# lyuchenyang/Macaw-LLM

Measured on NVIDIA H100. Metric: multimodal prefill tokens/sec (img+audio+text->LLaMA), higher is better.
Workload: dtype fp16

## Files before the change

include/macaw_b200.h:

```cpp
#ifndef MACAW_B200_H_
#define MACAW_B200_H_

#include <stdint.h>

#ifdef __cplusplus
extern "C" {
#endif

const char* mm_last_error(void);
int32_t mm_abi_version(void);
const char* mm_build_hash(void);
int64_t mm_launch_count(void);
void mm_launch_count_reset(void);
void mm_set_act_format(int32_t f16);
int32_t mm_get_act_format(void);

enum {
  MM_ACT_NONE = 0,
  MM_ACT_GELU = 1,
  MM_ACT_QUICK_GELU = 2,
  MM_ACT_SILU = 3
};
enum {
  MM_EPI_STD = 0,
  MM_EPI_SWIGLU = 1,
  MM_EPI_ROPE = 2
};

typedef struct mm_gemm_args {
  int32_t M, N, K, batch, batch2;
  const void* A;
  int64_t lda, a_bs, a_bs2;
  const void* B;
  int64_t ldb, b_bs, b_bs2;
  int32_t b_mn_major;
  void* C;
  int64_t ldc, c_bs, c_bs2;
  int32_t c_fp32;
  int32_t epi;
  int32_t act;
  float alpha;
  const void* bias;
  int64_t bias_bs;
  const float* row_scale;
  const void* residual;
  int64_t ldr, r_bs, r_bs2;
  int32_t res_row_mod;
  const float* rope_cos;
  const float* rope_sin;
  int32_t rope_T, rope_cols;
  const int32_t* rope_pos;
  int32_t c_trans;
  int32_t a_fp16, b_fp16;
  int32_t c_fp16;
  const float* bias_rs;
  const void* bias2;
  const float* bias2_rs;
  int32_t a_mn_major;
  float* sumsq_out;
  const float* rs_sumsq;
  int32_t rs_parts;
  float rs_eps;
  void* sk_workspace;
  int64_t sk_workspace_bytes;
} mm_gemm_args;

int32_t mm_gemm_fwd(const mm_gemm_args* args, void* stream);
enum {
  MM_GEMM_KERNEL_CONSUMER_EPILOGUE = 0,
  MM_GEMM_KERNEL_EPILOGUE_WARPGROUP = 1,
  MM_GEMM_KERNEL_TILE_PAIRS = 2
};
typedef struct mm_gemm_schedule {
  int32_t block_n;
  int32_t kernel;
  int32_t m_tiles, n_tiles, k_blocks;
  int64_t units;
  int32_t workers;
  int32_t grid;
  int32_t threads;
  int32_t waves;
  int32_t group_m;
  int32_t streamk_tiles;
  int32_t smem_bytes;
  int32_t vectorised_epilogue;
} mm_gemm_schedule;
int32_t mm_gemm_plan(const mm_gemm_args* args, mm_gemm_schedule* plan);
int32_t mm_gemm_streamk_mode(int32_t mode);
int32_t mm_gemm_overlap_mode(int32_t mode);
int64_t mm_gemm_streamk_workspace_bytes(void);

int32_t mm_splitk_reduce(const float* partial, int32_t splits, int32_t M, int32_t N, const void* bias, void* out,
                         int64_t ldo, int32_t out_fp16, void* stream);

typedef struct mm_attn_args {
  const void *q, *k, *v;
  void* out;
  int32_t B, H, Tq, Tk, head_dim;
  int64_t q_bs, q_ts, q_hs;
  int64_t k_bs, k_ts, k_hs;
  int64_t v_bs, v_ts, v_hs;
  int64_t o_bs, o_ts, o_hs;
  const int32_t* key_mask;
  int32_t causal;
  float scale;
  const int32_t* tk_dev;
} mm_attn_args;
int32_t mm_attn_fwd(const mm_attn_args* args, void* stream);

int32_t mm_rmsnorm_fwd(const void* x, const void* w, void* y, int32_t rows, int32_t cols, float eps, void* stream);
int32_t mm_rms_rstd(const void* x, float* rstd, int32_t rows, int32_t cols, float eps, void* stream);
int32_t mm_layernorm_fwd(const void* x, int64_t ldx, const void* w, const void* b, void* y, int64_t ldy, int32_t rows,
                         int32_t cols, float eps, void* stream);

int32_t mm_embed_gather(const void* table, int32_t vocab, int32_t dim, const int64_t* ids, int64_t n_ids, void* out,
                        int64_t ldo, void* stream);
int32_t mm_splice_prefix(const void* text, const void* prefix, void* dst, int32_t B, int32_t L, int32_t n_prefix,
                         int32_t E, const int64_t* mask_in, int64_t* mask_out, const int64_t* labels_in,
                         int64_t* labels_out, void* stream);
int32_t mm_patchify(const void* images, int32_t B, int32_t C, int32_t H, int32_t W, int32_t patch, void* out,
                    int64_t ldo, void* stream);
int32_t mm_transpose_pad(const void* x, int32_t B, int32_t C, int32_t T, int32_t pad, void* out, void* stream);
int32_t mm_add_rows(const void* x, int64_t ldx, const void* add, int64_t lda, int32_t add_rows, void* y, int64_t ldy,
                    int32_t rows, int32_t cols, void* stream);
int32_t mm_cast_bf16_f16(const void* x, int64_t ldx, void* y, int64_t ldy, int32_t rows, int32_t cols, void* stream);
int32_t mm_copy_rows(const void* x, int64_t ldx, void* y, int64_t ldy, int32_t rows, int32_t cols, void* stream);

typedef struct mm_align_args {
  const void* table;
  int32_t V, E;
  int64_t ldt;
  const void* qt;
  int32_t R;
  int64_t ldq;
  const float* row_bias;
  const float* extra;
  int64_t stat_stride;
  void* out;
  int64_t ldo;
  float* p_sum_real;
  float* p_extra;
  void* P;
  int64_t ldp;
  void* workspace;
  int32_t mode;
  float* inv_l;
} mm_align_args;
int32_t mm_align_fwd(const mm_align_args* args, void* stream);
int64_t mm_align_workspace_bytes(int32_t R, int32_t V);

int32_t mm_kv_append(const void* qkv, int64_t ld_qkv, int32_t B, int32_t T_new, int32_t E, void* cache, int32_t Tmax,
                     int32_t t0, const int32_t* t0_dev, void* stream);
int32_t mm_argmax_rows(const void* logits, int64_t ld, int32_t rows, int32_t V, int64_t* out, void* stream);
int32_t mm_sample_rows(const void* logits, int64_t ld, int32_t rows, int32_t V, uint32_t* seen, float repetition_penalty,
                       float temperature, int32_t top_k, float top_p, int32_t do_sample, const uint64_t* seed_dev,
                       const int32_t* step_dev, int64_t* out, void* stream);
enum { MM_THIN_RES = 0, MM_THIN_SWIGLU = 1, MM_THIN_QKV = 2 };
typedef struct mm_thin_args {
  const float* part;
  int32_t splits, N, M, ldp, mode;
  const float* row_scale;
  const float* rs_sumsq;
  int32_t rs_parts, rs_K;
  float rs_eps;
  const void* residual;
  int64_t ldr;
  void* out;
  int64_t ldo;
  float* sumsq_out;
  const float* rope_cos;
  const float* rope_sin;
  const int32_t* pos_dev;
  int32_t E;
  void* cache;
  int32_t Tmax, t0;
  const int32_t* t0_dev;
} mm_thin_args;
int32_t mm_thin_fused(const mm_thin_args* args, void* stream);
int32_t mm_rope_rows(void* x, int64_t ld, int32_t rows, int32_t rot_cols, const float* cos_t, const float* sin_t,
                     int32_t rope_T, const int32_t* pos_dev, void* stream);

int32_t mm_ce_loss(const void* logits, const int64_t* labels, int32_t B, int32_t T, int32_t V, float* loss_sum,
                   int32_t* n_valid, void* stream);

int32_t mm_rmsnorm_bwd_parts(int32_t rows);
int32_t mm_rmsnorm_bwd(const void* dy, const void* x, const float* rstd, const void* g, const void* dres, void* dx,
                       float* dg, float* dg_partials, int32_t rows, int32_t cols, void* stream);
int32_t mm_swiglu_fwd(const void* gate, const void* up, void* h, int64_t n, void* stream);
int32_t mm_swiglu_bwd(const void* dh, const void* gate, const void* up, void* dgate, void* dup, int64_t n, void* stream);
int32_t mm_attn_softmax_bwd(const float* S, const float* dP, void* P, void* dS, int32_t B, int32_t H, int32_t Tq,
                            int32_t Tk, int64_t ld, float scale, int32_t causal, const int32_t* key_mask, float p_drop,
                            const uint64_t* seed_dev, uint32_t sid, void* stream);
int32_t mm_attn_softmax_fwd(const float* S, void* P, int32_t B, int32_t H, int32_t Tq, int32_t Tk, int64_t ld, float scale,
                            int32_t causal, const int32_t* key_mask, float p_drop, const uint64_t* seed_dev, uint32_t sid,
                            void* stream);
int32_t mm_align_dropout_fwd(const void* P_unnorm_f16, void* Pm_f16, int64_t ldp, const float* inv_l, const float* p_extra,
                             float* rs, float* p_sum_real_d, float* p_extra_d, int32_t R, int32_t V, float p_drop,
                             const uint64_t* seed_dev, uint32_t sid, void* stream);
int32_t mm_dropout_mask(float* out, int64_t ld, int32_t rows, int32_t cols, float p_drop, const uint64_t* seed_dev,
                        uint32_t sid, void* stream);
int32_t mm_ce_bwd(const void* logits, const int64_t* labels, void* dlogits, int32_t B, int32_t T, int32_t V,
                  const int32_t* n_valid, float grad_scale, const float* grad_scale_dev, void* stream);
int32_t mm_embed_scatter_add(const void* dx, int64_t ldx, const int64_t* ids, int64_t n, int32_t dim, int32_t vocab,
                             void* dtable, void* stream);
int32_t mm_colsum(const void* x, int64_t ldx, int32_t rows, int32_t cols, float* out, void* stream);
int32_t mm_adamw(void* p, const void* g, float* master, float* m, float* v, int64_t n, float lr, float beta1, float beta2,
                 float eps, float weight_decay, int32_t step, const int32_t* step_dev, float grad_scale,
                 const float* grad_mult_dev, const int32_t* skip_dev, const float* lr_dev, void* stream);
int32_t mm_adamw_host(void* p, const void* g, float* master, float* m, float* v, int64_t n, float lr, float beta1,
                      float beta2, float eps, float weight_decay, int32_t step, const int32_t* step_dev, float grad_scale,
                      const float* grad_mult_dev, const int32_t* skip_dev, const float* lr_dev, void* stream);
int32_t mm_host_alloc(int64_t bytes, void** host_ptr, void** dev_ptr);
int32_t mm_host_free(void* host_ptr);

int32_t mm_grad_sumsq_parts(int64_t n);
int32_t mm_grad_sumsq(const void* g, int64_t n, int32_t fp16, float* out, float* partials, void* stream);
typedef struct mm_loss_scale_state {
  float scale;
  float inv_scale;
  int32_t cur_iter;
  int32_t last_overflow_iter;
  int32_t cur_hysteresis;
  int32_t skip;
  float grad_mult;
  int32_t skipped;
  int32_t step;
  float grad_norm;
  int32_t reserved[2];
} mm_loss_scale_state;
int32_t mm_loss_scale_update(mm_loss_scale_state* state, float* sumsq, float max_norm, int32_t dynamic, int32_t window,
                             int32_t hysteresis, float min_scale, void* stream);

int32_t mm_lr_schedule(const int32_t* step_dev, double base_lr, int32_t kind, int32_t warmup_steps, int32_t training_steps,
                       float* lr_out, void* stream);

int32_t mm_align_softmax_bwd(const float* G, int64_t ldg, const void* P_unnorm_f16, int64_t ldp, const float* inv_l,
                             const float* d_p_sum_real, const float* p_extra, const float* d_p_extra, float gscale,
                             void* P_bf16, void* dS_bf16, int64_t ldo, float* dstats, int32_t R, int32_t V, float p_drop,
                             const uint64_t* seed_dev, uint32_t sid, void* stream);
int32_t mm_head_weighted_colsum(const void* x, int64_t ldx, int32_t x_fp16, const float* w, int64_t w_stride, int32_t Nq,
                                int32_t E, int32_t head_dim, float* out, void* stream);
int32_t mm_window_gather_add(const void* dwin, int32_t B, int32_t N, int32_t C, int32_t Lq, int32_t kk, int32_t ss,
                             void* dfeats, void* stream);
int32_t mm_cast_f16_bf16(const void* x, int64_t ldx, void* y, int64_t ldy, int32_t rows, int32_t cols, void* stream);

#define MM_LORA_MAX 3
typedef struct mm_lora_args {
  int32_t n, M, K, N, r;
  float scaling, p_drop;
  const uint64_t* seed_dev;
  uint32_t sid[MM_LORA_MAX];
  const void* x;
  int64_t ldx;
  const void* A[MM_LORA_MAX];
  const void* B[MM_LORA_MAX];
  float* u[MM_LORA_MAX];
  void* y[MM_LORA_MAX];
  int64_t ldy;
  const float* rope_cos;
  const float* rope_sin;
  int32_t rope_T;
  float* g[MM_LORA_MAX];
  void* dA[MM_LORA_MAX];
  void* dB[MM_LORA_MAX];
  int32_t accumulate[MM_LORA_MAX];
  void* dx;
  int64_t lddx;
  float* workspace;
  int64_t workspace_bytes;
} mm_lora_args;
int32_t mm_lora_down(const mm_lora_args* args, void* stream);
int32_t mm_lora_up(const mm_lora_args* args, void* stream);
int32_t mm_lora_bwd_dy(const mm_lora_args* args, void* stream);
int32_t mm_lora_bwd_x(const mm_lora_args* args, void* stream);
int64_t mm_lora_workspace_bytes(const mm_lora_args* args, int32_t entry);

#define MM_W8_MAX_SRC 3
#define MM_W8_XS_BYTES 49152
typedef struct mm_w8_matrix {
  const int8_t* q[MM_W8_MAX_SRC];
  const float* scale[MM_W8_MAX_SRC];
  int32_t rows[MM_W8_MAX_SRC];
  const int32_t* chunks;
  int32_t N, K;
  const void* gain;
} mm_w8_matrix;
int32_t mm_quantize_rows_int8(const void* w, int64_t ldw, int32_t w_format, int32_t rows, int32_t K, int8_t* q, float* scale,
                              void* stream);
int32_t mm_dequant_rows(const mm_w8_matrix* w, void* out, int64_t ldo, void* stream);
int32_t mm_gemm_w8_thin(const mm_w8_matrix* w, const void* x, int64_t ldx, int32_t M, float* part, int32_t splits,
                        int32_t ldp, void* xs_work, void* stream);

typedef struct mm_gemm_e4m3_args {
  const float* a_scale;
  mm_w8_matrix w;
  int32_t unpromoted;
} mm_gemm_e4m3_args;
int32_t mm_quantize_rows_e4m3(const void* x, int64_t ldx, int32_t x_format, int32_t rows, int32_t K, const void* gain,
                              uint8_t* q, int64_t ldq, float* scale, void* stream);
int32_t mm_gemm_e4m3_fwd(const mm_gemm_args* args, const mm_gemm_e4m3_args* e, void* stream);
int32_t mm_gemm_e4m3_plan(const mm_gemm_args* args, const mm_gemm_e4m3_args* e, mm_gemm_schedule* plan);
int32_t mm_gemm_e4m3_thin(const mm_w8_matrix* w, const void* x, int64_t ldx, int32_t M, float* part, int32_t splits,
                          int32_t ldp, void* xs_work, void* stream);

int32_t mm_nccl_unique_id(void* out128);
int32_t mm_nccl_init(const void* id128, int32_t world, int32_t rank);
int32_t mm_nccl_allreduce(void* buf, int64_t count, int32_t dtype, int32_t average, void* stream);
int32_t mm_nccl_destroy(void);

typedef struct mm_image_args {
  const void* src;
  int64_t ld;
  int32_t row0, n_rows;
  int32_t out_h, out_w;
  const int32_t* bounds_h;
  const int32_t* kk_h;
  int32_t ksize_h;
  const int32_t* bounds_v;
  const int32_t* kk_v;
  int32_t ksize_v;
  float mean[3], std[3];
  void* tmp;
  void* out;
  int32_t out_fp32;
  void* out_u8;
} mm_image_args;
int32_t mm_image_preprocess(const mm_image_args* args, void* stream);
int32_t mm_log_mel(const float* pcm, int32_t n_samples, const float* basisT, const float* mel, float* logspec,
                   void* max_scratch, void* out, int32_t out_fp32, void* stream);

typedef struct mm_jpeg_image {
  int32_t width, height;
  int32_t n_comp;
  int32_t hmax, vmax;
  int32_t mcus_x, mcus_y;
  int32_t seg0, n_seg;
  int32_t bw[3], bh[3];
  int32_t huff_dc[3], huff_ac[3];
  int32_t quant[3];
  int64_t coef_off[3];
  int64_t plane_off[3];
  int64_t out_off, out_ld;
} mm_jpeg_image;
typedef struct mm_jpeg_segment {
  int64_t offset;
  int32_t n_bytes;
  int32_t image;
  int32_t mcu0, n_mcu;
} mm_jpeg_segment;
typedef struct mm_jpeg_huff {
  int32_t maxcode[18];
  int32_t valoffset[18];
  uint16_t look[256];
  uint8_t huffval[256];
} mm_jpeg_huff;
typedef struct mm_jpeg_args {
  int32_t n_images, n_segments, n_huff, n_quant;
  const uint8_t* data;
  int64_t data_bytes;
  const mm_jpeg_image* images;
  const mm_jpeg_segment* segments;
  const mm_jpeg_huff* huff;
  const uint16_t* quant;
  int16_t* coef;
  int64_t coef_elems;
  uint8_t* planes;
  int64_t plane_bytes;
  uint8_t* out;
  int64_t out_bytes;
  int32_t* status;
  int32_t max_blocks, max_pixels;
} mm_jpeg_args;
int32_t mm_jpeg_decode(const mm_jpeg_args* args, void* stream);

#ifdef __cplusplus
}
#endif
#endif
```

macaw-llm_b200/_lib.py:

```python
from __future__ import annotations

import ctypes as C
import os

HERE = os.path.dirname(os.path.abspath(__file__))
LIB_PATH = os.path.join(HERE, "libmacaw_b200.so")

c_i32, c_i64, c_f32, c_vp, c_u32 = C.c_int32, C.c_int64, C.c_float, C.c_void_p, C.c_uint32


class GemmArgs(C.Structure):

    _fields_ = [
        ("M", c_i32), ("N", c_i32), ("K", c_i32), ("batch", c_i32), ("batch2", c_i32),
        ("A", c_vp), ("lda", c_i64), ("a_bs", c_i64), ("a_bs2", c_i64),
        ("B", c_vp), ("ldb", c_i64), ("b_bs", c_i64), ("b_bs2", c_i64), ("b_mn_major", c_i32),
        ("C", c_vp), ("ldc", c_i64), ("c_bs", c_i64), ("c_bs2", c_i64), ("c_fp32", c_i32),
        ("epi", c_i32), ("act", c_i32), ("alpha", c_f32),
        ("bias", c_vp), ("bias_bs", c_i64),
        ("row_scale", c_vp),
        ("residual", c_vp), ("ldr", c_i64), ("r_bs", c_i64), ("r_bs2", c_i64), ("res_row_mod", c_i32),
        ("rope_cos", c_vp), ("rope_sin", c_vp), ("rope_T", c_i32), ("rope_cols", c_i32), ("rope_pos", c_vp), ("c_trans", c_i32),
        ("a_fp16", c_i32), ("b_fp16", c_i32), ("c_fp16", c_i32),
        ("bias_rs", c_vp), ("bias2", c_vp), ("bias2_rs", c_vp), ("a_mn_major", c_i32),
        ("sumsq_out", c_vp), ("rs_sumsq", c_vp), ("rs_parts", c_i32), ("rs_eps", c_f32),
        ("sk_workspace", c_vp), ("sk_workspace_bytes", c_i64),
    ]


class GemmPlan(C.Structure):

    _fields_ = [("block_n", c_i32), ("kernel", c_i32), ("m_tiles", c_i32), ("n_tiles", c_i32), ("k_blocks", c_i32),
                ("units", c_i64), ("workers", c_i32), ("grid", c_i32), ("threads", c_i32), ("waves", c_i32),
                ("group_m", c_i32), ("streamk_tiles", c_i32), ("smem_bytes", c_i32), ("vectorised_epilogue", c_i32)]


class ThinArgs(C.Structure):
    _fields_ = [("part", c_vp), ("splits", c_i32), ("N", c_i32), ("M", c_i32), ("ldp", c_i32), ("mode", c_i32),
                ("row_scale", c_vp), ("rs_sumsq", c_vp), ("rs_parts", c_i32), ("rs_K", c_i32), ("rs_eps", c_f32),
                ("residual", c_vp), ("ldr", c_i64), ("out", c_vp), ("ldo", c_i64), ("sumsq_out", c_vp),
                ("rope_cos", c_vp), ("rope_sin", c_vp), ("pos_dev", c_vp), ("E", c_i32), ("cache", c_vp),
                ("Tmax", c_i32), ("t0", c_i32), ("t0_dev", c_vp)]


class AttnArgs(C.Structure):

    _fields_ = [
        ("q", c_vp), ("k", c_vp), ("v", c_vp), ("out", c_vp),
        ("B", c_i32), ("H", c_i32), ("Tq", c_i32), ("Tk", c_i32), ("head_dim", c_i32),
        ("q_bs", c_i64), ("q_ts", c_i64), ("q_hs", c_i64),
        ("k_bs", c_i64), ("k_ts", c_i64), ("k_hs", c_i64),
        ("v_bs", c_i64), ("v_ts", c_i64), ("v_hs", c_i64),
        ("o_bs", c_i64), ("o_ts", c_i64), ("o_hs", c_i64),
        ("key_mask", c_vp), ("causal", c_i32), ("scale", c_f32), ("tk_dev", c_vp),
    ]


class AlignArgs(C.Structure):

    _fields_ = [
        ("table", c_vp), ("V", c_i32), ("E", c_i32), ("ldt", c_i64),
        ("qt", c_vp), ("R", c_i32), ("ldq", c_i64),
        ("row_bias", c_vp), ("extra", c_vp), ("stat_stride", c_i64),
        ("out", c_vp), ("ldo", c_i64), ("p_sum_real", c_vp), ("p_extra", c_vp),
        ("P", c_vp), ("ldp", c_i64), ("workspace", c_vp), ("mode", c_i32), ("inv_l", c_vp),
    ]


LORA_MAX = 3


class LoraArgs(C.Structure):

    _fields_ = [
        ("n", c_i32), ("M", c_i32), ("K", c_i32), ("N", c_i32), ("r", c_i32), ("scaling", c_f32), ("p_drop", c_f32),
        ("seed_dev", c_vp), ("sid", c_u32 * LORA_MAX), ("x", c_vp), ("ldx", c_i64), ("A", c_vp * LORA_MAX),
        ("B", c_vp * LORA_MAX), ("u", c_vp * LORA_MAX), ("y", c_vp * LORA_MAX), ("ldy", c_i64), ("rope_cos", c_vp),
        ("rope_sin", c_vp), ("rope_T", c_i32), ("g", c_vp * LORA_MAX), ("dA", c_vp * LORA_MAX), ("dB", c_vp * LORA_MAX),
        ("accumulate", c_i32 * LORA_MAX), ("dx", c_vp), ("lddx", c_i64), ("workspace", c_vp), ("workspace_bytes", c_i64),
    ]


W8_MAX_SRC = 3
W8_XS_BYTES = 49152


class W8Matrix(C.Structure):

    _fields_ = [("q", c_vp * W8_MAX_SRC), ("scale", c_vp * W8_MAX_SRC), ("rows", c_i32 * W8_MAX_SRC), ("chunks", c_vp), ("N", c_i32), ("K", c_i32),
                ("gain", c_vp)]


class GemmE4m3Args(C.Structure):

    _fields_ = [("a_scale", c_vp), ("w", W8Matrix), ("unpromoted", c_i32)]


class LossScaleState(C.Structure):

    _fields_ = [("scale", c_f32), ("inv_scale", c_f32), ("cur_iter", c_i32), ("last_overflow_iter", c_i32),
                ("cur_hysteresis", c_i32), ("skip", c_i32), ("grad_mult", c_f32), ("skipped", c_i32), ("step", c_i32),
                ("grad_norm", c_f32), ("reserved", c_i32 * 2)]


class ImageArgs(C.Structure):

    _fields_ = [
        ("src", c_vp), ("ld", c_i64), ("row0", c_i32), ("n_rows", c_i32), ("out_h", c_i32), ("out_w", c_i32),
        ("bounds_h", c_vp), ("kk_h", c_vp), ("ksize_h", c_i32), ("bounds_v", c_vp), ("kk_v", c_vp), ("ksize_v", c_i32),
        ("mean", c_f32 * 3), ("std", c_f32 * 3), ("tmp", c_vp), ("out", c_vp), ("out_fp32", c_i32), ("out_u8", c_vp),
    ]


class JpegImage(C.Structure):

    _fields_ = [
        ("width", c_i32), ("height", c_i32), ("n_comp", c_i32), ("hmax", c_i32), ("vmax", c_i32),
        ("mcus_x", c_i32), ("mcus_y", c_i32), ("seg0", c_i32), ("n_seg", c_i32),
        ("bw", c_i32 * 3), ("bh", c_i32 * 3), ("huff_dc", c_i32 * 3), ("huff_ac", c_i32 * 3), ("quant", c_i32 * 3),
        ("coef_off", c_i64 * 3), ("plane_off", c_i64 * 3), ("out_off", c_i64), ("out_ld", c_i64),
    ]


class JpegSegment(C.Structure):

    _fields_ = [("offset", c_i64), ("n_bytes", c_i32), ("image", c_i32), ("mcu0", c_i32), ("n_mcu", c_i32)]


class JpegHuff(C.Structure):

    _fields_ = [("maxcode", c_i32 * 18), ("valoffset", c_i32 * 18), ("look", C.c_uint16 * 256), ("huffval", C.c_uint8 * 256)]


class JpegArgs(C.Structure):

    _fields_ = [
        ("n_images", c_i32), ("n_segments", c_i32), ("n_huff", c_i32), ("n_quant", c_i32),
        ("data", c_vp), ("data_bytes", c_i64), ("images", c_vp), ("segments", c_vp), ("huff", c_vp), ("quant", c_vp),
        ("coef", c_vp), ("coef_elems", c_i64), ("planes", c_vp), ("plane_bytes", c_i64), ("out", c_vp),
        ("out_bytes", c_i64), ("status", c_vp), ("max_blocks", c_i32), ("max_pixels", c_i32),
    ]


SIGNATURES = {
    "mm_last_error": (C.c_char_p, []),
    "mm_abi_version": (c_i32, []),
    "mm_build_hash": (C.c_char_p, []),
    "mm_launch_count": (c_i64, []),
    "mm_launch_count_reset": (None, []),
    "mm_set_act_format": (None, [c_i32]),
    "mm_get_act_format": (c_i32, []),
    "mm_gemm_fwd": (c_i32, [C.POINTER(GemmArgs), c_vp]),
    "mm_gemm_plan": (c_i32, [C.POINTER(GemmArgs), C.POINTER(GemmPlan)]),
    "mm_splitk_reduce": (c_i32, [c_vp, c_i32, c_i32, c_i32, c_vp, c_vp, c_i64, c_i32, c_vp]),
    "mm_attn_fwd": (c_i32, [C.POINTER(AttnArgs), c_vp]),
    "mm_rmsnorm_fwd": (c_i32, [c_vp, c_vp, c_vp, c_i32, c_i32, c_f32, c_vp]),
    "mm_rms_rstd": (c_i32, [c_vp, c_vp, c_i32, c_i32, c_f32, c_vp]),
    "mm_layernorm_fwd": (c_i32, [c_vp, c_i64, c_vp, c_vp, c_vp, c_i64, c_i32, c_i32, c_f32, c_vp]),
    "mm_embed_gather": (c_i32, [c_vp, c_i32, c_i32, c_vp, c_i64, c_vp, c_i64, c_vp]),
    "mm_splice_prefix": (c_i32, [c_vp, c_vp, c_vp, c_i32, c_i32, c_i32, c_i32, c_vp, c_vp, c_vp, c_vp, c_vp]),
    "mm_patchify": (c_i32, [c_vp, c_i32, c_i32, c_i32, c_i32, c_i32, c_vp, c_i64, c_vp]),
    "mm_transpose_pad": (c_i32, [c_vp, c_i32, c_i32, c_i32, c_i32, c_vp, c_vp]),
    "mm_add_rows": (c_i32, [c_vp, c_i64, c_vp, c_i64, c_i32, c_vp, c_i64, c_i32, c_i32, c_vp]),
    "mm_cast_bf16_f16": (c_i32, [c_vp, c_i64, c_vp, c_i64, c_i32, c_i32, c_vp]),
    "mm_copy_rows": (c_i32, [c_vp, c_i64, c_vp, c_i64, c_i32, c_i32, c_vp]),
    "mm_align_fwd": (c_i32, [C.POINTER(AlignArgs), c_vp]),
    "mm_align_workspace_bytes": (c_i64, [c_i32, c_i32]),
    "mm_kv_append": (c_i32, [c_vp, c_i64, c_i32, c_i32, c_i32, c_vp, c_i32, c_i32, c_vp, c_vp]),
    "mm_gemm_streamk_workspace_bytes": (c_i64, []),
    "mm_gemm_streamk_mode": (c_i32, [c_i32]),
    "mm_gemm_overlap_mode": (c_i32, [c_i32]),
    "mm_thin_fused": (c_i32, [C.POINTER(ThinArgs), c_vp]),
    "mm_argmax_rows": (c_i32, [c_vp, c_i64, c_i32, c_i32, c_vp, c_vp]),
    "mm_sample_rows": (c_i32, [c_vp, c_i64, c_i32, c_i32, c_vp, c_f32, c_f32, c_i32, c_f32, c_i32, c_vp, c_vp, c_vp, c_vp]),
    "mm_rope_rows": (c_i32, [c_vp, c_i64, c_i32, c_i32, c_vp, c_vp, c_i32, c_vp, c_vp]),
    "mm_rmsnorm_bwd": (c_i32, [c_vp, c_vp, c_vp, c_vp, c_vp, c_vp, c_vp, c_vp, c_i32, c_i32, c_vp]),
    "mm_rmsnorm_bwd_parts": (c_i32, [c_i32]),
    "mm_swiglu_fwd": (c_i32, [c_vp, c_vp, c_vp, c_i64, c_vp]),
    "mm_swiglu_bwd": (c_i32, [c_vp, c_vp, c_vp, c_vp, c_vp, c_i64, c_vp]),
    "mm_attn_softmax_bwd": (c_i32, [c_vp, c_vp, c_vp, c_vp, c_i32, c_i32, c_i32, c_i32, c_i64, c_f32, c_i32, c_vp, c_f32, c_vp,
                                    c_u32, c_vp]),
    "mm_attn_softmax_fwd": (c_i32, [c_vp, c_vp, c_i32, c_i32, c_i32, c_i32, c_i64, c_f32, c_i32, c_vp, c_f32, c_vp, c_u32, c_vp]),
    "mm_align_dropout_fwd": (c_i32, [c_vp, c_vp, c_i64, c_vp, c_vp, c_vp, c_vp, c_vp, c_i32, c_i32, c_f32, c_vp, c_u32, c_vp]),
    "mm_dropout_mask": (c_i32, [c_vp, c_i64, c_i32, c_i32, c_f32, c_vp, c_u32, c_vp]),
    "mm_ce_bwd": (c_i32, [c_vp, c_vp, c_vp, c_i32, c_i32, c_i32, c_vp, c_f32, c_vp, c_vp]),
    "mm_embed_scatter_add": (c_i32, [c_vp, c_i64, c_vp, c_i64, c_i32, c_i32, c_vp, c_vp]),
    "mm_colsum": (c_i32, [c_vp, c_i64, c_i32, c_i32, c_vp, c_vp]),
    "mm_adamw": (c_i32, [c_vp, c_vp, c_vp, c_vp, c_vp, c_i64, c_f32, c_f32, c_f32, c_f32, c_f32, c_i32, c_vp, c_f32, c_vp,
                         c_vp, c_vp, c_vp]),
    "mm_adamw_host": (c_i32, [c_vp, c_vp, c_vp, c_vp, c_vp, c_i64, c_f32, c_f32, c_f32, c_f32, c_f32, c_i32, c_vp, c_f32,
                              c_vp, c_vp, c_vp, c_vp]),
    "mm_lr_schedule": (c_i32, [c_vp, C.c_double, c_i32, c_i32, c_i32, c_vp, c_vp]),
    "mm_host_alloc": (c_i32, [c_i64, C.POINTER(c_vp), C.POINTER(c_vp)]),
    "mm_host_free": (c_i32, [c_vp]),
    "mm_grad_sumsq_parts": (c_i32, [c_i64]),
    "mm_grad_sumsq": (c_i32, [c_vp, c_i64, c_i32, c_vp, c_vp, c_vp]),
    "mm_loss_scale_update": (c_i32, [c_vp, c_vp, c_f32, c_i32, c_i32, c_i32, c_f32, c_vp]),
    "mm_image_preprocess": (c_i32, [C.POINTER(ImageArgs), c_vp]),
    "mm_log_mel": (c_i32, [c_vp, c_i32, c_vp, c_vp, c_vp, c_vp, c_vp, c_i32, c_vp]),
    "mm_align_softmax_bwd": (c_i32, [c_vp, c_i64, c_vp, c_i64, c_vp, c_vp, c_vp, c_vp, c_f32, c_vp, c_vp, c_i64, c_vp, c_i32,
                                     c_i32, c_f32, c_vp, c_u32, c_vp]),
    "mm_head_weighted_colsum": (c_i32, [c_vp, c_i64, c_i32, c_vp, c_i64, c_i32, c_i32, c_i32, c_vp, c_vp]),
    "mm_window_gather_add": (c_i32, [c_vp, c_i32, c_i32, c_i32, c_i32, c_i32, c_i32, c_vp, c_vp]),
    "mm_cast_f16_bf16": (c_i32, [c_vp, c_i64, c_vp, c_i64, c_i32, c_i32, c_vp]),
    "mm_nccl_unique_id": (c_i32, [c_vp]),
    "mm_nccl_init": (c_i32, [c_vp, c_i32, c_i32]),
    "mm_nccl_allreduce": (c_i32, [c_vp, c_i64, c_i32, c_i32, c_vp]),
    "mm_nccl_destroy": (c_i32, []),
    "mm_ce_loss": (c_i32, [c_vp, c_vp, c_i32, c_i32, c_i32, c_vp, c_vp, c_vp]),
    "mm_lora_down": (c_i32, [C.POINTER(LoraArgs), c_vp]),
    "mm_lora_up": (c_i32, [C.POINTER(LoraArgs), c_vp]),
    "mm_lora_bwd_dy": (c_i32, [C.POINTER(LoraArgs), c_vp]),
    "mm_lora_bwd_x": (c_i32, [C.POINTER(LoraArgs), c_vp]),
    "mm_lora_workspace_bytes": (c_i64, [C.POINTER(LoraArgs), c_i32]),
    "mm_jpeg_decode": (c_i32, [C.POINTER(JpegArgs), c_vp]),
    "mm_quantize_rows_int8": (c_i32, [c_vp, c_i64, c_i32, c_i32, c_i32, c_vp, c_vp, c_vp]),
    "mm_dequant_rows": (c_i32, [C.POINTER(W8Matrix), c_vp, c_i64, c_vp]),
    "mm_gemm_w8_thin": (c_i32, [C.POINTER(W8Matrix), c_vp, c_i64, c_i32, c_vp, c_i32, c_i32, c_vp, c_vp]),
    "mm_quantize_rows_e4m3": (c_i32, [c_vp, c_i64, c_i32, c_i32, c_i32, c_vp, c_vp, c_i64, c_vp, c_vp]),
    "mm_gemm_e4m3_fwd": (c_i32, [C.POINTER(GemmArgs), C.POINTER(GemmE4m3Args), c_vp]),
    "mm_gemm_e4m3_plan": (c_i32, [C.POINTER(GemmArgs), C.POINTER(GemmE4m3Args), C.POINTER(GemmPlan)]),
    "mm_gemm_e4m3_thin": (c_i32, [C.POINTER(W8Matrix), c_vp, c_i64, c_i32, c_vp, c_i32, c_i32, c_vp, c_vp]),
}

NULLABLE_BEFORE_STREAM = {"mm_adamw": 1, "mm_adamw_host": 1}

_lib = None
ABI_VERSION = 8


class _NullableBeforeStream:

    def __init__(self, fn, n_opt: int):
        self._fn, self._n_opt = fn, n_opt

    def __call__(self, *args):
        n = len(self._fn.argtypes)
        if n - self._n_opt <= len(args) < n:
            args = args[:-1] + (None,) * (n - len(args)) + args[-1:]
        return self._fn(*args)

    def __getattr__(self, name):
        return getattr(self._fn, name)


def load(build_if_missing: bool = True) -> C.CDLL:
    global _lib
    if _lib is not None:
        return _lib
    import importlib.util

    spec = importlib.util.spec_from_file_location("_macaw_b200_build", os.path.join(HERE, "build.py"))
    mod = importlib.util.module_from_spec(spec)
    spec.loader.exec_module(mod)
    want = mod.source_hash()
    if not os.path.exists(LIB_PATH) or mod.built_hash() != want:
        if not build_if_missing:
            raise RuntimeError(f"{LIB_PATH} is missing or older than csrc/; run `python macaw-llm_b200/build.py`")
        mod.build()
    lib = C.CDLL(LIB_PATH)
    for name, (res, args) in SIGNATURES.items():
        fn = getattr(lib, name)
        fn.restype = res
        fn.argtypes = args
        if name in NULLABLE_BEFORE_STREAM:
            setattr(lib, name, _NullableBeforeStream(fn, NULLABLE_BEFORE_STREAM[name]))
    got = lib.mm_build_hash().decode()
    if got != want or lib.mm_abi_version() != ABI_VERSION:
        raise RuntimeError(f"libmacaw_b200.so was built from other sources (library {got}, csrc {want}; ABI "
                           f"{lib.mm_abi_version()} vs {ABI_VERSION}): rebuild with `python macaw-llm_b200/build.py --force`")
    _lib = lib
    return lib


def last_error() -> str:
    return load().mm_last_error().decode("utf-8", "replace")
```

macaw-llm_b200/csrc/gemm_wgmma.cu:

```cuda
#include "common.cuh"
#include "ptx.cuh"
#include "../../include/macaw_b200.h"
#include <stdlib.h>

namespace mm {

struct GemmKParams {
  int M, N, K, batch, batch2;
  int m_tiles, n_tiles, num_k;
  int b_shared, b2_shared;
  void* C;
  long long ldc, c_bs, c_bs2;
  int c_fp32;
  int act;
  float alpha;
  const bf16* bias;
  long long bias_bs;
  const float* row_scale;
  const bf16* residual;
  long long ldr, r_bs, r_bs2;
  int res_row_mod;
  const float* rope_cos;
  const float* rope_sin;
  int rope_T, rope_cols;
  const int* rope_pos;
  int c_trans;
  int c_fp16;
  int aux_f16;
  const float* bias_rs;
  const bf16* bias2;
  const float* bias2_rs;
  float* sumsq_out;
  const float* rs_sumsq;
  int sumsq_parts, rs_parts;
  float rs_eps;
  int vec_ok;
  int group_m;
  int sk_tiles, sk_first;
  float* sk_ws;
  int* sk_flags;
};

constexpr int kBlockM = 128;
constexpr int kBlockK = 64;
constexpr uint32_t kABytes = kBlockM * kBlockK * 2;
constexpr int kMaxBN = 128;
constexpr int kGemmThreads = 288;
constexpr int kProducerWarp = 8;
constexpr int kGemmThreadsEwg = 512;
constexpr int kProducerWarpEwg = 12;
constexpr int kEwgMinKBlocks = 32;

__host__ __device__ constexpr int gemm_stages(int BN) {
  return BN >= 128 ? 4 : (BN >= 64 ? 6 : 8);
}
__host__ __device__ constexpr int gemm_stage_ld(int BN) { return BN + 4; }
__host__ __device__ constexpr size_t gemm_smem_bytes(int stages, uint32_t b_bytes, int BN) {
  return 1024  + (size_t)stages * (kABytes + b_bytes) + (size_t)kBlockM * gemm_stage_ld(BN) * 4 +
         256 ;
}

struct GemmSmem {
  uint8_t *sA, *sB;
  float* sC;
  uint64_t *full_bar, *empty_bar, *staging_full, *staging_empty;
};
template <int STAGES, uint32_t B_BYTES, int BN>
__device__ __forceinline__ GemmSmem gemm_smem(uint8_t* smem_raw) {
  uint8_t* smem = reinterpret_cast<uint8_t*>((reinterpret_cast<uintptr_t>(smem_raw) + 1023) & ~uintptr_t(1023));
  uint8_t* sB = smem + STAGES * kABytes;
  float* sC = reinterpret_cast<float*>(sB + STAGES * B_BYTES);
  uint64_t* bar = reinterpret_cast<uint64_t*>(sC + kBlockM * gemm_stage_ld(BN));
  return {smem, sB, sC, bar, bar + STAGES, bar + 2 * STAGES, bar + 2 * STAGES + 1};
}
template <int STAGES, bool STAGING>
__device__ __forceinline__ void gemm_prologue(const GemmSmem& s, const CUtensorMap* tmA, const CUtensorMap* tmB) {
  tma_prefetch_desc(tmA);
  tma_prefetch_desc(tmB);
  for (int i = 0; i < STAGES; ++i) {
    mbar_init(&s.full_bar[i], 1);
    mbar_init(&s.empty_bar[i], 8);
  }
  if constexpr (STAGING) {
    mbar_init(s.staging_full, 256);
    mbar_init(s.staging_empty, 128);
  }
  fence_mbar_init();
}

struct TileCoord {
  int b, b_lo, b_hi, m_blk, n_blk;
};
__device__ __forceinline__ TileCoord tile_coord(int idx, const GemmKParams& p, int m_units) {
  const int per_batch = m_units * p.n_tiles;
  TileCoord t;
  t.b = idx / per_batch;
  t.b_hi = t.b / p.batch;
  t.b_lo = t.b - t.b_hi * p.batch;
  int r = idx - t.b * per_batch;
  const int in_group = p.group_m * p.n_tiles;
  const int g = r / in_group;
  const int first_m = g * p.group_m;
  const int gsz = min(m_units - first_m, p.group_m);
  const int rr = r - g * in_group;
  t.m_blk = first_m + rr % gsz;
  t.n_blk = rr / gsz;
  return t;
}

struct GemmWork {
  int tile, kb0, kb1, role, c0, nc;
};
__device__ __forceinline__ bool gemm_work(const GemmKParams& p, int worker, int n_workers, int total_tiles, int it,
                                          GemmWork& w) {
  const int first = p.sk_tiles > 0 ? p.sk_first : total_tiles;
  const int n_full = first > worker ? (first - worker + n_workers - 1) / n_workers : 0;
  w.c0 = 0;
  w.nc = 0;
  int n_sk = 0;
  unsigned nk = 1, U = 0, u0 = 0, u1 = 0, ta = 0, end_a = 0;
  bool has_b = false;
  if (p.sk_tiles > 0) {
    nk = p.num_k;
    U = static_cast<unsigned>(p.sk_tiles) * nk;
    u0 = static_cast<unsigned>(worker) * U / n_workers;
    u1 = static_cast<unsigned>(worker + 1) * U / n_workers;
    if (u0 < u1) {
      ta = u0 / nk;
      end_a = u1 < (ta + 1) * nk ? u1 : (ta + 1) * nk;
      has_b = u1 > end_a;
      n_sk = has_b ? 2 : 1;
    }
  }
  if (it >= n_sk) {
    const int f = it - n_sk;
    if (f >= n_full) return false;
    w.tile = worker + f * n_workers;
    w.kb0 = 0;
    w.kb1 = p.num_k;
    w.role = 0;
    return true;
  }
  if (has_b && it == 0) {
    w.tile = first + static_cast<int>(ta) + 1;
    w.kb0 = 0;
    w.kb1 = static_cast<int>(u1 - end_a);
    w.role = 1;
    return true;
  }
  w.tile = first + static_cast<int>(ta);
  w.kb0 = static_cast<int>(u0 - ta * nk);
  w.kb1 = static_cast<int>(end_a - ta * nk);
  w.role = (w.kb1 == p.num_k) ? 2 : 1;
  if (w.role == 2) {
    int c0 = worker;
    while (c0 > 0 && static_cast<unsigned>(c0) * U / n_workers > ta * nk) --c0;
    w.c0 = c0;
    w.nc = worker - c0;
  }
  return true;
}

__device__ __forceinline__ void st_release_gpu(int* p, int v) {
  asm volatile("st.release.gpu.global.s32 [%0], %1;" ::"l"(p), "r"(v) : "memory");
}
__device__ __forceinline__ int ld_acquire_gpu(const int* p) {
  int v;
  asm volatile("ld.acquire.gpu.global.s32 %0, [%1];" : "=r"(v) : "l"(p) : "memory");
  return v;
}

__device__ __forceinline__ float rcp_approx(float x) {
  float y;
  asm("rcp.approx.ftz.f32 %0, %1;" : "=f"(y) : "f"(x));
  return y;
}
__device__ __forceinline__ float sigmoid_fast(float x) { return rcp_approx(1.0f + __expf(-x)); }
__device__ __forceinline__ float gelu_erf(float x) {
  const float z = fabsf(x) * 0.70710678118654752f;
  const float t = __frcp_rn(fmaf(0.5f, z, 1.0f));
  float p = fmaf(0.17087277f, t, -0.82215223f);
  p = fmaf(p, t, 1.48851587f);
  p = fmaf(p, t, -1.13520398f);
  p = fmaf(p, t, 0.27886807f);
  p = fmaf(p, t, -0.18628806f);
  p = fmaf(p, t, 0.09678418f);
  p = fmaf(p, t, 0.37409196f);
  p = fmaf(p, t, 1.00002368f);
  p = fmaf(p, t, -1.26551223f);
  const float q = t * exp2f(1.4426950408889634f * fmaf(-z, z, p));
  return 0.5f * x * (x >= 0.0f ? 2.0f - q : q);
}

__device__ __forceinline__ float aux_ld(const bf16* p, long long i, int f16) {
  const uint16_t raw = reinterpret_cast<const uint16_t*>(p)[i];
  return f16 ? __half2float(__ushort_as_half(raw)) : __uint_as_float(static_cast<uint32_t>(raw) << 16);
}
__device__ __forceinline__ void aux_add8(float* v, const uint4& u, int f16) {
  if (f16) {
    const __half2* h = reinterpret_cast<const __half2*>(&u);
#pragma unroll
    for (int k = 0; k < 4; ++k) {
      const float2 f = __half22float2(h[k]);
      v[2 * k] += f.x;
      v[2 * k + 1] += f.y;
    }
  } else {
    v[0] += bf16lo(u.x); v[1] += bf16hi(u.x); v[2] += bf16lo(u.y); v[3] += bf16hi(u.y);
    v[4] += bf16lo(u.z); v[5] += bf16hi(u.z); v[6] += bf16lo(u.w); v[7] += bf16hi(u.w);
  }
}

__device__ __forceinline__ void apply_act32(float (&v)[32], int act) {
  if (act == MM_ACT_QUICK_GELU) {
#pragma unroll
    for (int i = 0; i < 32; ++i) v[i] *= sigmoid_fast(1.702f * v[i]);
  } else if (act == MM_ACT_GELU) {
#pragma unroll
    for (int i = 0; i < 32; ++i) v[i] = gelu_erf(v[i]);
  } else if (act == MM_ACT_SILU) {
#pragma unroll
    for (int i = 0; i < 32; ++i) v[i] *= sigmoid_fast(v[i]);
  }
}

__device__ __forceinline__ void store_row32(const GemmKParams& p, void* crow, int col0, int ncols_total,
                                            const float (&v)[32]) {
  if (p.c_fp32) {
    float* c = reinterpret_cast<float*>(crow) + col0;
    if (p.vec_ok && col0 + 32 <= ncols_total) {
#pragma unroll
      for (int i = 0; i < 8; ++i)
        reinterpret_cast<float4*>(c)[i] = make_float4(v[4 * i], v[4 * i + 1], v[4 * i + 2], v[4 * i + 3]);
    } else {
#pragma unroll
      for (int i = 0; i < 32; ++i)
        if (col0 + i < ncols_total) c[i] = v[i];
    }
  } else {
    bf16* c = reinterpret_cast<bf16*>(crow) + col0;
    if (p.vec_ok && col0 + 32 <= ncols_total) {
      if (p.c_fp16) {
#pragma unroll
        for (int i = 0; i < 4; ++i) {
          uint4 u;
          u.x = pack_f16x2(v[8 * i + 0], v[8 * i + 1]);
          u.y = pack_f16x2(v[8 * i + 2], v[8 * i + 3]);
          u.z = pack_f16x2(v[8 * i + 4], v[8 * i + 5]);
          u.w = pack_f16x2(v[8 * i + 6], v[8 * i + 7]);
          reinterpret_cast<uint4*>(c)[i] = u;
        }
      } else {
#pragma unroll
        for (int i = 0; i < 4; ++i) {
          uint4 u;
          u.x = pack_bf16x2(v[8 * i + 0], v[8 * i + 1]);
          u.y = pack_bf16x2(v[8 * i + 2], v[8 * i + 3]);
          u.z = pack_bf16x2(v[8 * i + 4], v[8 * i + 5]);
          u.w = pack_bf16x2(v[8 * i + 6], v[8 * i + 7]);
          reinterpret_cast<uint4*>(c)[i] = u;
        }
      }
    } else if (p.c_fp16) {
      __half* ch = reinterpret_cast<__half*>(c);
#pragma unroll
      for (int i = 0; i < 32; ++i)
        if (col0 + i < ncols_total) ch[i] = __float2half_rn(v[i]);
    } else {
#pragma unroll
      for (int i = 0; i < 32; ++i)
        if (col0 + i < ncols_total) c[i] = __float2bfloat16(v[i]);
    }
  }
}

template <int BN, bool F16, int TA, int TB>
__device__ __forceinline__ void wgmma_tile(float (&d)[BN / 2], uint64_t a, uint64_t b) {
  if constexpr (BN == 128) wgmma_ss_n128<F16, TA, TB>(d, a, b, 1u);
  else if constexpr (BN == 64) wgmma_ss_n64<F16, TA, TB>(d, a, b, 1u);
  else wgmma_ss_n32<F16, TA, TB>(d, a, b, 1u);
}

template <int BN, int EPI>
__host__ __device__ constexpr int epi_chunk_count() {
  return EPI == MM_EPI_STD ? (BN >= 64 ? BN / 64 : 1) : 2 * (BN / 128);
}
template <int BN, int EPI>
__host__ __device__ constexpr int epi_chunk(int half, int j) {
  if constexpr (EPI == MM_EPI_STD) {
    const int c = half * epi_chunk_count<BN, EPI>() + j;
    return c < BN / 32 ? c : -1;
  } else {
    const int u = half * (BN / 128) + j / 2;
    if constexpr (EPI == MM_EPI_SWIGLU) return 2 * u + (j & 1);
    else return 4 * (u >> 1) + (u & 1) + 2 * (j & 1);
  }
}
template <int BN, int EPI>
constexpr bool epi_chunks_partition_tile() {
  int seen[BN / 32] = {};
  for (int half = 0; half < 2; ++half)
    for (int j = 0; j < epi_chunk_count<BN, EPI>(); ++j) {
      const int c = epi_chunk<BN, EPI>(half, j);
      if (c >= BN / 32) return false;
      if (c >= 0) ++seen[c];
    }
  for (int c = 0; c < BN / 32; ++c)
    if (seen[c] != 1) return false;
  return true;
}

__device__ __forceinline__ void consumer_sync() { asm volatile("bar.sync 1, 256;" ::: "memory"); }

__device__ __forceinline__ float epi_row_scale(const GemmKParams& p, const TileCoord& t, int row) {
  const bool row_ok = row < p.M;
  float rs = 1.0f;
  if (p.row_scale != nullptr && row_ok && !p.c_trans) rs = p.row_scale[static_cast<long long>(t.b) * p.M + row];
  if (p.rs_sumsq != nullptr && row_ok) {
    const float4* sp = reinterpret_cast<const float4*>(p.rs_sumsq + static_cast<long long>(row) * p.rs_parts);
    float ssum = 0.f;
    for (int j = 0; j < p.rs_parts / 4; ++j) {
      const float4 f = __ldg(sp + j);
      ssum += (f.x + f.y) + (f.z + f.w);
    }
    rs = rsqrtf(ssum / static_cast<float>(p.K) + p.rs_eps);
  }
  return rs * p.alpha;
}

template <int BN, int EPI>
__device__ __forceinline__ void gemm_epilogue(const GemmKParams& p, const TileCoord& t, const GemmWork& wk, const float* srow,
                                              float rs, int q, int lane, int half, int wi, int worker, int n_workers) {
  const int n_out_total = (EPI == MM_EPI_SWIGLU) ? p.N / 2 : p.N;
  const int row = t.m_blk * kBlockM + q * 32 + lane;
  const bool row_ok = row < p.M;
  if (wk.role == 1) {
    float* slot = p.sk_ws + static_cast<long long>(worker) * (kBlockM * BN);
#pragma unroll 1
    for (int j = 0; j < epi_chunk_count<BN, EPI>(); ++j) {
      const int c = epi_chunk<BN, EPI>(half, j);
      if (c < 0) continue;
      uint32_t r[32];
      stage_ld32(srow + c * 32, r);
      float4* dst = reinterpret_cast<float4*>(slot) + static_cast<long long>(c) * 8 * kBlockM + q * 32 + lane;
#pragma unroll
      for (int i = 0; i < 8; ++i)
        dst[i * kBlockM] = make_float4(__uint_as_float(r[4 * i]), __uint_as_float(r[4 * i + 1]), __uint_as_float(r[4 * i + 2]),
                             __uint_as_float(r[4 * i + 3]));
    }
    __threadfence();
    __syncwarp();
    if (lane == 0) st_release_gpu(p.sk_flags + worker * 8 + wi, 1);
    return;
  }
  const unsigned sk_units = static_cast<unsigned>(p.sk_tiles) * p.num_k;
  auto sk_has = [&](int sidx) {
    return static_cast<unsigned>(sidx) * sk_units / n_workers < static_cast<unsigned>(sidx + 1) * sk_units / n_workers;
  };
  auto sk_add = [&](uint32_t (&r)[32], int col_off) {
    if (wk.nc == 0) return;
    const int c = col_off >> 5;
    for (int sidx = wk.c0; sidx < wk.c0 + wk.nc; ++sidx) {
      if (!sk_has(sidx)) continue;
      const float4* src = reinterpret_cast<const float4*>(p.sk_ws + static_cast<long long>(sidx) * (kBlockM * BN)) +
                          static_cast<long long>(c) * 8 * kBlockM + q * 32 + lane;
      float4 fv[8];
#pragma unroll
      for (int i = 0; i < 8; ++i) fv[i] = __ldcg(src + i * kBlockM);
#pragma unroll
      for (int i = 0; i < 8; ++i) {
        const float4 f = fv[i];
        r[4 * i] = __float_as_uint(__uint_as_float(r[4 * i]) + f.x);
        r[4 * i + 1] = __float_as_uint(__uint_as_float(r[4 * i + 1]) + f.y);
        r[4 * i + 2] = __float_as_uint(__uint_as_float(r[4 * i + 2]) + f.z);
        r[4 * i + 3] = __float_as_uint(__uint_as_float(r[4 * i + 3]) + f.w);
      }
    }
  };
  if (wk.nc > 0) {
    if (lane == 0)
      for (int sidx = wk.c0; sidx < wk.c0 + wk.nc; ++sidx)
        if (sk_has(sidx)) {
          unsigned spins = 0;
          while (ld_acquire_gpu(p.sk_flags + sidx * 8 + wi) == 0) {
            __nanosleep(64);
            if (++spins > (1u << 25)) asm volatile("trap;");
          }
        }
    __syncwarp();
  }
  char* crow = reinterpret_cast<char*>(p.C) +
               (static_cast<long long>(t.b_lo) * p.c_bs + static_cast<long long>(t.b_hi) * p.c_bs2 +
                static_cast<long long>(row) * p.ldc) * (p.c_fp32 ? 4 : 2);
  if constexpr (EPI == MM_EPI_STD) {
    if (p.c_trans) {
      const float bias_r = (p.bias != nullptr && row_ok) ? aux_ld(p.bias, row, p.aux_f16) : 0.f;
#pragma unroll 1
      for (int j = 0; j < epi_chunk_count<BN, EPI>(); ++j) {
        const int c = epi_chunk<BN, EPI>(half, j);
        if (c < 0) continue;
        uint32_t r[32];
        stage_ld32(srow + c * 32, r);
        sk_add(r, c * 32);
        const int col0 = t.n_blk * BN + c * 32;
        if (col0 >= p.N || !row_ok) continue;
        float v[32];
#pragma unroll
        for (int i = 0; i < 32; ++i) {
          const int col = col0 + i;
          float cs = p.alpha;
          if (p.row_scale != nullptr && col < p.N) cs *= p.row_scale[col];
          v[i] = __uint_as_float(r[i]) * cs + bias_r;
        }
        if (p.act != MM_ACT_NONE) apply_act32(v, p.act);
#pragma unroll
        for (int i = 0; i < 32; ++i) {
          const int col = col0 + i;
          if (col < p.N) {
            float o = v[i];
            if (p.residual != nullptr) o += aux_ld(p.residual, static_cast<long long>(col) * p.ldr + row, p.aux_f16);
            if (p.c_fp32)
              reinterpret_cast<float*>(p.C)[static_cast<long long>(col) * p.ldc + row] = o;
            else if (p.c_fp16)
              reinterpret_cast<__half*>(p.C)[static_cast<long long>(col) * p.ldc + row] = __float2half_rn(o);
            else
              reinterpret_cast<bf16*>(p.C)[static_cast<long long>(col) * p.ldc + row] = __float2bfloat16(o);
          }
        }
      }
    } else {
    const bf16* bias = p.bias ? p.bias + static_cast<long long>(t.b_lo) * p.bias_bs : nullptr;
    const bf16* rrow = nullptr;
    if (p.residual != nullptr && row_ok) {
      const int rr = p.res_row_mod > 0 ? row % p.res_row_mod : row;
      rrow = p.residual + static_cast<long long>(t.b_lo) * p.r_bs + static_cast<long long>(t.b_hi) * p.r_bs2 +
             static_cast<long long>(rr) * p.ldr;
    }
#pragma unroll 1
    for (int j = 0; j < epi_chunk_count<BN, EPI>(); ++j) {
      const int c = epi_chunk<BN, EPI>(half, j);
      if (c < 0) continue;
      uint32_t r[32];
      stage_ld32(srow + c * 32, r);
      sk_add(r, c * 32);
      const int col0 = t.n_blk * BN + c * 32;
      if (col0 >= p.N) continue;
      float v[32];
#pragma unroll
      for (int i = 0; i < 32; ++i) v[i] = __uint_as_float(r[i]) * rs;
      const bool full = p.vec_ok && (col0 + 32 <= p.N);
      if (p.bias_rs != nullptr || p.bias2 != nullptr) {
        const long long ri = static_cast<long long>(t.b) * p.M + row;
        const float s1 = (p.bias_rs != nullptr && row_ok) ? p.bias_rs[ri] : 1.0f;
        const float s2 = (p.bias2_rs != nullptr && row_ok) ? p.bias2_rs[ri] : 1.0f;
        const bf16* b2 = p.bias2 ? p.bias2 + static_cast<long long>(t.b_lo) * p.bias_bs : nullptr;
#pragma unroll
        for (int i = 0; i < 32; ++i)
          if (col0 + i < p.N) {
            if (bias != nullptr) v[i] = fmaf(s1, aux_ld(bias, col0 + i, p.aux_f16), v[i]);
            if (b2 != nullptr) v[i] = fmaf(s2, aux_ld(b2, col0 + i, p.aux_f16), v[i]);
          }
      } else if (bias != nullptr) {
        if (full) {
#pragma unroll
          for (int i = 0; i < 4; ++i)
            aux_add8(v + 8 * i, __ldg(reinterpret_cast<const uint4*>(bias + col0) + i), p.aux_f16);
        } else {
#pragma unroll
          for (int i = 0; i < 32; ++i)
            if (col0 + i < p.N) v[i] += aux_ld(bias, col0 + i, p.aux_f16);
        }
      }
      if (p.act != MM_ACT_NONE) apply_act32(v, p.act);
      if (rrow != nullptr) {
        if (full) {
#pragma unroll
          for (int i = 0; i < 4; ++i) aux_add8(v + 8 * i, *(reinterpret_cast<const uint4*>(rrow + col0) + i), p.aux_f16);
        } else {
#pragma unroll
          for (int i = 0; i < 32; ++i)
            if (col0 + i < p.N) v[i] += aux_ld(rrow, col0 + i, p.aux_f16);
        }
      }
      if (row_ok) store_row32(p, crow, col0, n_out_total, v);
      if (p.sumsq_out != nullptr && row_ok) {
        float ss = 0.f;
#pragma unroll
        for (int i = 0; i < 32; ++i) {
          const float r = p.c_fp16 ? __half2float(__float2half_rn(v[i])) : __bfloat162float(__float2bfloat16(v[i]));
          ss = fmaf(r, r, ss);
        }
        p.sumsq_out[static_cast<long long>(row) * p.sumsq_parts + (col0 >> 5)] = ss;
      }
    }
    }
  } else if constexpr (EPI == MM_EPI_SWIGLU) {
#pragma unroll 1
    for (int j = 0; j < epi_chunk_count<BN, EPI>(); j += 2) {
      const int cg = epi_chunk<BN, EPI>(half, j), cu = epi_chunk<BN, EPI>(half, j + 1);
      uint32_t g[32], u[32];
      stage_ld32(srow + cg * 32, g);
      stage_ld32(srow + cu * 32, u);
      sk_add(g, cg * 32);
      sk_add(u, cu * 32);
      const int col_in = t.n_blk * BN + cg * 32;
      if (col_in >= p.N) continue;
      float v[32];
#pragma unroll
      for (int i = 0; i < 32; ++i) {
        const float gg = __uint_as_float(g[i]) * rs;
        const float uu = __uint_as_float(u[i]) * rs;
        v[i] = gg * sigmoid_fast(gg) * uu;
      }
      if (row_ok) store_row32(p, crow, col_in / 2, n_out_total, v);
    }
  } else {
    const int pos = (row_ok ? (row % p.rope_T) : 0) + (p.rope_pos != nullptr ? __ldg(p.rope_pos) : 0);
    const float* cs = p.rope_cos + static_cast<long long>(pos) * 64;
    const float* sn = p.rope_sin + static_cast<long long>(pos) * 64;
#pragma unroll 1
    for (int j = 0; j < epi_chunk_count<BN, EPI>(); j += 2) {
      {
        const int c1 = epi_chunk<BN, EPI>(half, j), c2 = epi_chunk<BN, EPI>(half, j + 1);
        const int hc = c1 & 1;
        uint32_t x1[32], x2[32];
        stage_ld32(srow + c1 * 32, x1);
        stage_ld32(srow + c2 * 32, x2);
        sk_add(x1, c1 * 32);
        sk_add(x2, c2 * 32);
        const int col1 = t.n_blk * BN + c1 * 32;
        if (col1 >= p.N) continue;
        float o1[32], o2[32];
        if (col1 < p.rope_cols) {
#pragma unroll
          for (int i = 0; i < 8; ++i) {
            const float4 c4 = __ldg(reinterpret_cast<const float4*>(cs + hc * 32) + i);
            const float4 s4 = __ldg(reinterpret_cast<const float4*>(sn + hc * 32) + i);
            const float cc[4] = {c4.x, c4.y, c4.z, c4.w};
            const float ss[4] = {s4.x, s4.y, s4.z, s4.w};
#pragma unroll
            for (int j = 0; j < 4; ++j) {
              const float a = __uint_as_float(x1[4 * i + j]) * rs;
              const float b = __uint_as_float(x2[4 * i + j]) * rs;
              o1[4 * i + j] = a * cc[j] - b * ss[j];
              o2[4 * i + j] = b * cc[j] + a * ss[j];
            }
          }
        } else {
#pragma unroll
          for (int i = 0; i < 32; ++i) {
            o1[i] = __uint_as_float(x1[i]) * rs;
            o2[i] = __uint_as_float(x2[i]) * rs;
          }
        }
        if (row_ok) {
          store_row32(p, crow, col1, n_out_total, o1);
          store_row32(p, crow, col1 + 64, n_out_total, o2);
        }
      }
    }
  }
  if (wk.nc > 0) {
    __syncwarp();
    if (lane == 0)
      for (int sidx = wk.c0; sidx < wk.c0 + wk.nc; ++sidx)
        if (sk_has(sidx)) p.sk_flags[sidx * 8 + wi] = 0;
  }
}

template <int BN, int N>
__device__ __forceinline__ void stage_acc(float* sC, const float (&acc)[N], int off, int wg, int q, int lane) {
  constexpr int LDS = gemm_stage_ld(BN);
  const int r0 = wg * 64 + q * 16 + (lane >> 2);
  const int c0 = 2 * (lane & 3);
#pragma unroll
  for (int j = 0; j < BN / 8; ++j) {
    const int i = off + 4 * j;
    *reinterpret_cast<float2*>(sC + r0 * LDS + 8 * j + c0) = make_float2(acc[i], acc[i + 1]);
    *reinterpret_cast<float2*>(sC + (r0 + 8) * LDS + 8 * j + c0) = make_float2(acc[i + 2], acc[i + 3]);
  }
}

template <int BN, int EPI>
__device__ __forceinline__ void ewg_tile(const GemmKParams& p, const GemmSmem& s, const TileCoord& t, const GemmWork& wk,
                                         const float* srow, float rs, uint32_t parity, int q, int lane, int worker,
                                         int n_workers) {
  mbar_wait(s.staging_full, parity);
  for (int half = 0; half < 2; ++half)
    gemm_epilogue<BN, EPI>(p, t, wk, srow, rs, q, lane, half, q + 4 * half, worker, n_workers);
  mbar_arrive(s.staging_empty);
}

template <int BN, int EPI, bool B_MN, bool A_MN, bool F16, bool EWG>
__global__ void __launch_bounds__(EWG ? kGemmThreadsEwg : kGemmThreads, 1)
gemm_bf16_kernel(const __grid_constant__ CUtensorMap tmA, const __grid_constant__ CUtensorMap tmB,
                 const GemmKParams p) {
  static_assert(BN == 32 || BN == 64 || BN == 128, "wgmma tile width");
  static_assert(epi_chunks_partition_tile<BN, EPI>(), "epilogue chunk ownership must partition the tile");
  constexpr int STAGES = gemm_stages(BN);
  constexpr uint32_t B_BYTES = BN * kBlockK * 2;
  constexpr int LDS = gemm_stage_ld(BN);

  extern __shared__ uint8_t smem_raw[];
  const GemmSmem sm = gemm_smem<STAGES, B_BYTES, BN>(smem_raw);

  constexpr int kProducer = EWG ? kProducerWarpEwg : kProducerWarp;
  const int warp = threadIdx.x >> 5;
  const int lane = threadIdx.x & 31;
  const int worker = static_cast<int>(blockIdx.x);
  const int n_workers = static_cast<int>(gridDim.x);
  const int m_units = p.m_tiles;
  const int total_tiles = p.batch * p.batch2 * m_units * p.n_tiles;

  if (warp == kProducer && elect_one()) gemm_prologue<STAGES, EWG>(sm, &tmA, &tmB);
  __syncthreads();
  griddep_launch();
  griddep_wait();

  if (warp >= kProducer) {
    if constexpr (EWG) setmaxnreg_dec<40>();
    if (warp == kProducer && elect_one()) {
      int stage = 0;
      uint32_t phase = 0;
      GemmWork wk;
      for (int it = 0; gemm_work(p, worker, n_workers, total_tiles, it, wk); ++it) {
        const TileCoord t = tile_coord(wk.tile, p, m_units);
        const int bb = p.b_shared ? 0 : t.b_lo;
        const int bh = p.b2_shared ? 0 : t.b_hi;
        for (int kb = wk.kb0; kb < wk.kb1; ++kb) {
          mbar_wait(&sm.empty_bar[stage], phase ^ 1);
          mbar_arrive_expect_tx(&sm.full_bar[stage], kABytes + B_BYTES);
          if constexpr (A_MN) {
#pragma unroll
            for (int j = 0; j < kBlockM / 64; ++j)
              tma_load_4d(&tmA, &sm.full_bar[stage], sm.sA + stage * kABytes + j * 8192, t.m_blk * kBlockM + j * 64,
                          kb * kBlockK, t.b_lo, t.b_hi);
          } else {
            tma_load_4d(&tmA, &sm.full_bar[stage], sm.sA + stage * kABytes, kb * kBlockK, t.m_blk * kBlockM, t.b_lo,
                        t.b_hi);
          }
          if constexpr (!B_MN) {
            tma_load_4d(&tmB, &sm.full_bar[stage], sm.sB + stage * B_BYTES, kb * kBlockK, t.n_blk * BN, bb, bh);
          } else {
#pragma unroll
            for (int j = 0; j < BN / 64; ++j)
              tma_load_4d(&tmB, &sm.full_bar[stage], sm.sB + stage * B_BYTES + j * 8192, t.n_blk * BN + j * 64,
                          kb * kBlockK, bb, bh);
          }
          if (++stage == STAGES) {
            stage = 0;
            phase ^= 1;
          }
        }
      }
    }
    return;
  }

  const int q = warp & 3;
  const float* srow = sm.sC + (q * 32 + lane) * LDS;
  if (EWG && warp >= 8) {
    if constexpr (EWG) setmaxnreg_inc<168>();
    GemmWork wk;
    for (int it = 0; gemm_work(p, worker, n_workers, total_tiles, it, wk); ++it) {
      const TileCoord t = tile_coord(wk.tile, p, m_units);
      const float rs = epi_row_scale(p, t, t.m_blk * kBlockM + q * 32 + lane);
      ewg_tile<BN, EPI>(p, sm, t, wk, srow, rs, it & 1, q, lane, worker, n_workers);
    }
    return;
  }

  if constexpr (EWG) setmaxnreg_inc<152>();
  const int wg = warp >> 2;
  int stage = 0;
  uint32_t phase = 0;
  GemmWork wk;
  for (int it = 0; gemm_work(p, worker, n_workers, total_tiles, it, wk); ++it) {
    const TileCoord t = tile_coord(wk.tile, p, m_units);
    {
      float acc[BN / 2];
#pragma unroll
      for (int i = 0; i < BN / 2; ++i) acc[i] = 0.f;
      int prev = -1;
      for (int kb = wk.kb0; kb < wk.kb1; ++kb) {
        mbar_wait(&sm.full_bar[stage], phase);
        const uint32_t a_addr = smem_u32(sm.sA + stage * kABytes) + wg * 8192;
        const uint32_t b_addr = smem_u32(sm.sB + stage * B_BYTES);
        const uint64_t a_desc = make_sdesc_sw128(a_addr, A_MN ? 8192 : 16, 1024);
        const uint64_t b_desc = make_sdesc_sw128(b_addr, B_MN ? 8192 : 16, 1024);
        wgmma_fence();
#pragma unroll
        for (int kk = 0; kk < kBlockK / 16; ++kk)
          wgmma_tile<BN, F16, A_MN ? 1 : 0, B_MN ? 1 : 0>(acc, a_desc + static_cast<uint64_t>(A_MN ? kk * 128 : kk * 2),
                                                         b_desc + static_cast<uint64_t>(B_MN ? kk * 128 : kk * 2));
        wgmma_commit();
        wgmma_wait<1>();
        if (prev >= 0) {
          __syncwarp();
          if (lane == 0) mbar_arrive(&sm.empty_bar[prev]);
        }
        prev = stage;
        if (++stage == STAGES) {
          stage = 0;
          phase ^= 1;
        }
      }
      wgmma_wait<0>();
      fence_regs(acc);
      __syncwarp();
      if (lane == 0) mbar_arrive(&sm.empty_bar[prev]);
      if constexpr (EWG) mbar_wait(sm.staging_empty, (it & 1) ^ 1);
      else consumer_sync();
      stage_acc<BN>(sm.sC, acc, 0, wg, q, lane);
      if constexpr (EWG) {
        mbar_arrive(sm.staging_full);
        continue;
      }
      consumer_sync();
    }
    const int half = warp >> 2;
    const float rs = wk.role == 1 ? 1.0f : epi_row_scale(p, t, t.m_blk * kBlockM + q * 32 + lane);
    gemm_epilogue<BN, EPI>(p, t, wk, srow, rs, q, lane, half, warp, worker, n_workers);
  }
}

constexpr int kWideThreads = 384;
constexpr int kWideStages = 3;
constexpr uint32_t kWideBBytes = 2 * kMaxBN * kBlockK * 2;
constexpr size_t kWideSmemBytes = gemm_smem_bytes(kWideStages, kWideBBytes, kMaxBN);
static_assert(kWideSmemBytes <= 227 * 1024, "wide GEMM: ring + staging tile exceed an sm_90 block's shared memory");
constexpr int kWideRegsConsumer = 184, kWideRegsEpilogue = 136;
static_assert(2 * kWideRegsConsumer + kWideRegsEpilogue <= 3 * 168, "wide GEMM: register budget");

__device__ __forceinline__ TileCoord pair_coord(int idx, const GemmKParams& p) {
  const int n_pairs = p.n_tiles / 2;
  const int in_group = p.group_m * n_pairs;
  const int g = idx / in_group;
  const int first_m = g * p.group_m;
  const int gsz = min(p.m_tiles - first_m, p.group_m);
  const int rr = idx - g * in_group;
  TileCoord t;
  t.b = t.b_lo = t.b_hi = 0;
  t.m_blk = first_m + rr % gsz;
  t.n_blk = 2 * (rr / gsz);
  return t;
}

template <int EPI, bool F16>
__global__ void __launch_bounds__(kWideThreads, 1)
gemm_wide_kernel(const __grid_constant__ CUtensorMap tmA, const __grid_constant__ CUtensorMap tmB, const GemmKParams p) {
  constexpr int BN = kMaxBN;
  extern __shared__ uint8_t smem_raw[];
  const GemmSmem sm = gemm_smem<kWideStages, kWideBBytes, BN>(smem_raw);

  const int warp = threadIdx.x >> 5;
  const int lane = threadIdx.x & 31;
  const int worker = static_cast<int>(blockIdx.x);
  const int n_workers = static_cast<int>(gridDim.x);
  const int total_pairs = p.m_tiles * (p.n_tiles / 2);

  if (warp == 0 && elect_one()) gemm_prologue<kWideStages, true>(sm, &tmA, &tmB);
  __syncthreads();
  griddep_launch();
  griddep_wait();

  const int q = warp & 3;
  if (warp >= 8) {
    setmaxnreg_dec<kWideRegsEpilogue>();
    const float* srow = sm.sC + (q * 32 + lane) * gemm_stage_ld(BN);
    GemmWork wk;
    wk.tile = 0; wk.kb0 = 0; wk.kb1 = p.num_k; wk.role = 0; wk.c0 = 0; wk.nc = 0;
    for (int u = worker; u < total_pairs; u += n_workers) {
      TileCoord t = pair_coord(u, p);
      const float rs = epi_row_scale(p, t, t.m_blk * kBlockM + q * 32 + lane);
#pragma unroll 1
      for (int side = 0; side < 2; ++side) {
        ewg_tile<BN, EPI>(p, sm, t, wk, srow, rs, side, q, lane, worker, n_workers);
        ++t.n_blk;
      }
    }
    return;
  }

  setmaxnreg_inc<kWideRegsConsumer>();
  const int wg = warp >> 2;
  int stage = 0;
  uint32_t phase = 0;
  const bool loader = threadIdx.x == 0;
  int ld_u = worker, ld_kb = 0, ld_stage = 0;
  uint32_t ld_phase = 0;
  TileCoord ld_t = pair_coord(worker, p);
  auto load_next = [&]() {
    if (ld_u >= total_pairs) return;
    mbar_wait(&sm.empty_bar[ld_stage], ld_phase ^ 1);
    mbar_arrive_expect_tx(&sm.full_bar[ld_stage], kABytes + kWideBBytes);
    tma_load_4d(&tmA, &sm.full_bar[ld_stage], sm.sA + ld_stage * kABytes, ld_kb * kBlockK, ld_t.m_blk * kBlockM, 0, 0);
    uint8_t* b = sm.sB + ld_stage * kWideBBytes;
    tma_load_4d(&tmB, &sm.full_bar[ld_stage], b, ld_kb * kBlockK, ld_t.n_blk * BN, 0, 0);
    tma_load_4d(&tmB, &sm.full_bar[ld_stage], b + kWideBBytes / 2, ld_kb * kBlockK, (ld_t.n_blk + 1) * BN, 0, 0);
    if (++ld_stage == kWideStages) {
      ld_stage = 0;
      ld_phase ^= 1;
    }
    if (++ld_kb == p.num_k) {
      ld_kb = 0;
      ld_u += n_workers;
      if (ld_u < total_pairs) ld_t = pair_coord(ld_u, p);
    }
  };
  if (loader)
    for (int s = 0; s < kWideStages; ++s) load_next();
  __syncwarp();
  for (int u = worker; u < total_pairs; u += n_workers) {
    float acc[2 * BN / 2];
#pragma unroll
    for (int i = 0; i < BN; ++i) acc[i] = 0.f;
    int prev = -1;
    for (int kb = 0; kb < p.num_k; ++kb) {
      mbar_wait(&sm.full_bar[stage], phase);
      const uint64_t a_desc = make_sdesc_sw128(smem_u32(sm.sA + stage * kABytes) + wg * 8192, 16, 1024);
      const uint64_t b_desc = make_sdesc_sw128(smem_u32(sm.sB + stage * kWideBBytes), 16, 1024);
      wgmma_fence();
#pragma unroll
      for (int kk = 0; kk < kBlockK / 16; ++kk)
        wgmma_ss_n256<F16, 0, 0>(acc, a_desc + static_cast<uint64_t>(kk * 2), b_desc + static_cast<uint64_t>(kk * 2), 1u);
      wgmma_commit();
      wgmma_wait<1>();
      if (prev >= 0) {
        __syncwarp();
        if (lane == 0) mbar_arrive(&sm.empty_bar[prev]);
        if (loader) load_next();
        __syncwarp();
      }
      prev = stage;
      if (++stage == kWideStages) {
        stage = 0;
        phase ^= 1;
      }
    }
    wgmma_wait<0>();
    fence_regs(acc);
    __syncwarp();
    if (lane == 0) mbar_arrive(&sm.empty_bar[prev]);
    if (loader) load_next();
    __syncwarp();
#pragma unroll
    for (int side = 0; side < 2; ++side) {
      mbar_wait(sm.staging_empty, side ^ 1);
      stage_acc<BN>(sm.sC, acc, side * (BN / 2), wg, q, lane);
      mbar_arrive(sm.staging_full);
    }
  }
}

struct E4m3P {
  const float* a_scale;
  const float* w_scale[MM_W8_MAX_SRC];
  int w_rows[MM_W8_MAX_SRC];
  const int32_t* chunks;
};

__device__ __forceinline__ void tma_load_2d(const CUtensorMap* m, uint64_t* bar, void* dst, int c0, int c1) {
  asm volatile("cp.async.bulk.tensor.2d.shared::cluster.global.mbarrier::complete_tx::bytes [%0], [%1, {%3, %4}], [%2];"
               ::"r"(smem_u32(dst)), "l"(reinterpret_cast<uint64_t>(m)), "r"(smem_u32(bar)), "r"(c0), "r"(c1)
               : "memory");
}

__device__ __forceinline__ float e4m3_w_scale(const E4m3P& e, int n) {
  const int2 c = reinterpret_cast<const int2*>(e.chunks)[n >> 5];
  const int rows = c.x == 0 ? e.w_rows[0] : c.x == 1 ? e.w_rows[1] : e.w_rows[2];
  const float* s = c.x == 0 ? e.w_scale[0] : c.x == 1 ? e.w_scale[1] : e.w_scale[2];
  if (c.x < 0 || c.x >= MM_W8_MAX_SRC || s == nullptr || c.y < 0 || c.y + 32 > rows) return 0.f;
  return __ldg(s + c.y + (n & 31));
}

constexpr int kE4m3BlockK = 128;

template <int EPI, bool PROMOTE>
__global__ void __launch_bounds__(kGemmThreads, 1)
gemm_e4m3_kernel(const __grid_constant__ CUtensorMap tmA, const __grid_constant__ CUtensorMap tmB0,
                 const __grid_constant__ CUtensorMap tmB1, const __grid_constant__ CUtensorMap tmB2, const GemmKParams p,
                 const E4m3P e) {
  constexpr int BN = kMaxBN;
  constexpr int STAGES = gemm_stages(BN);
  constexpr uint32_t B_BYTES = BN * kE4m3BlockK;
  static_assert(B_BYTES == BN * kBlockK * 2 && kABytes == kBlockM * kE4m3BlockK, "e4m3 stage = the 16-bit stage");
  constexpr int LDS = gemm_stage_ld(BN);
  extern __shared__ uint8_t smem_raw[];
  const GemmSmem sm = gemm_smem<STAGES, B_BYTES, BN>(smem_raw);

  const int warp = threadIdx.x >> 5;
  const int lane = threadIdx.x & 31;
  const int worker = static_cast<int>(blockIdx.x);
  const int n_workers = static_cast<int>(gridDim.x);
  const int m_units = p.m_tiles;
  const int total_tiles = m_units * p.n_tiles;

  if (warp == kProducerWarp && elect_one()) {
    gemm_prologue<STAGES, false>(sm, &tmA, &tmB0);
    tma_prefetch_desc(&tmB1);
    tma_prefetch_desc(&tmB2);
  }
  __syncthreads();
  griddep_launch();
  griddep_wait();

  if (warp == kProducerWarp) {
    if (elect_one()) {
      int stage = 0;
      uint32_t phase = 0;
      GemmWork wk;
      for (int it = 0; gemm_work(p, worker, n_workers, total_tiles, it, wk); ++it) {
        const TileCoord t = tile_coord(wk.tile, p, m_units);
        const CUtensorMap* bm[4];
        int brow[4];
#pragma unroll
        for (int c = 0; c < 4; ++c) {
          const int2 ch = reinterpret_cast<const int2*>(e.chunks)[t.n_blk * 4 + c];
          bm[c] = ch.x == 0 ? &tmB0 : ch.x == 1 ? &tmB1 : &tmB2;
          brow[c] = ch.y;
        }
        for (int kb = wk.kb0; kb < wk.kb1; ++kb) {
          mbar_wait(&sm.empty_bar[stage], phase ^ 1);
          mbar_arrive_expect_tx(&sm.full_bar[stage], kABytes + B_BYTES);
          tma_load_2d(&tmA, &sm.full_bar[stage], sm.sA + stage * kABytes, kb * kE4m3BlockK, t.m_blk * kBlockM);
#pragma unroll
          for (int c = 0; c < 4; ++c)
            tma_load_2d(bm[c], &sm.full_bar[stage], sm.sB + stage * B_BYTES + c * (32 * kE4m3BlockK), kb * kE4m3BlockK,
                        brow[c]);
          if (++stage == STAGES) {
            stage = 0;
            phase ^= 1;
          }
        }
      }
    }
    return;
  }

  const int q = warp & 3;
  const float* srow = sm.sC + (q * 32 + lane) * LDS;
  const int wg = warp >> 2;
  int stage = 0;
  uint32_t phase = 0;
  GemmWork wk;
  for (int it = 0; gemm_work(p, worker, n_workers, total_tiles, it, wk); ++it) {
    const TileCoord t = tile_coord(wk.tile, p, m_units);
    {
      float acc[BN / 2];
#pragma unroll
      for (int i = 0; i < BN / 2; ++i) acc[i] = 0.f;
      int prev = -1;
      for (int kb = wk.kb0; kb < wk.kb1; ++kb) {
        mbar_wait(&sm.full_bar[stage], phase);
        const uint64_t a_desc = make_sdesc_sw128(smem_u32(sm.sA + stage * kABytes) + wg * 8192, 16, 1024);
        const uint64_t b_desc = make_sdesc_sw128(smem_u32(sm.sB + stage * B_BYTES), 16, 1024);
        if constexpr (PROMOTE) {
          float part[BN / 2];
          wgmma_fence();
#pragma unroll
          for (int kk = 0; kk < kE4m3BlockK / 32; ++kk)
            wgmma_e4m3_n128(part, a_desc + static_cast<uint64_t>(kk * 2), b_desc + static_cast<uint64_t>(kk * 2),
                            kk > 0 ? 1u : 0u);
          wgmma_commit();
          wgmma_wait<0>();
          fence_regs(part);
          __syncwarp();
          if (lane == 0) mbar_arrive(&sm.empty_bar[stage]);
#pragma unroll
          for (int i = 0; i < BN / 2; ++i) acc[i] += part[i];
        } else {
          wgmma_fence();
#pragma unroll
          for (int kk = 0; kk < kE4m3BlockK / 32; ++kk)
            wgmma_e4m3_n128(acc, a_desc + static_cast<uint64_t>(kk * 2), b_desc + static_cast<uint64_t>(kk * 2), 1u);
          wgmma_commit();
          wgmma_wait<1>();
          if (prev >= 0) {
            __syncwarp();
            if (lane == 0) mbar_arrive(&sm.empty_bar[prev]);
          }
          prev = stage;
        }
        if (++stage == STAGES) {
          stage = 0;
          phase ^= 1;
        }
      }
      if constexpr (!PROMOTE) {
        wgmma_wait<0>();
        fence_regs(acc);
        __syncwarp();
        if (lane == 0 && prev >= 0) mbar_arrive(&sm.empty_bar[prev]);
      }
      const int r0 = t.m_blk * kBlockM + wg * 64 + q * 16 + (lane >> 2);
      const float sx0 = r0 < p.M ? __ldg(e.a_scale + r0) : 0.f;
      const float sx1 = r0 + 8 < p.M ? __ldg(e.a_scale + r0 + 8) : 0.f;
      const int n0 = t.n_blk * BN + 2 * (lane & 3);
#pragma unroll
      for (int j = 0; j < BN / 8; ++j) {
        const float sw0 = e4m3_w_scale(e, n0 + 8 * j), sw1 = e4m3_w_scale(e, n0 + 8 * j + 1);
        acc[4 * j] = acc[4 * j] * sx0 * sw0;
        acc[4 * j + 1] = acc[4 * j + 1] * sx0 * sw1;
        acc[4 * j + 2] = acc[4 * j + 2] * sx1 * sw0;
        acc[4 * j + 3] = acc[4 * j + 3] * sx1 * sw1;
      }
      consumer_sync();
      stage_acc<BN>(sm.sC, acc, 0, wg, q, lane);
      consumer_sync();
    }
    const int half = warp >> 2;
    const float rs = epi_row_scale(p, t, t.m_blk * kBlockM + q * 32 + lane);
    gemm_epilogue<BN, EPI>(p, t, wk, srow, rs, q, lane, half, warp, worker, n_workers);
  }
}

typedef CUresult (*EncodeTiledFn)(CUtensorMap*, CUtensorMapDataType, cuuint32_t, void*, const cuuint64_t*,
                                  const cuuint64_t*, const cuuint32_t*, const cuuint32_t*, CUtensorMapInterleave,
                                  CUtensorMapSwizzle, CUtensorMapL2promotion, CUtensorMapFloatOOBfill);

static EncodeTiledFn get_encode_fn() {
  static EncodeTiledFn fn = nullptr;
  if (fn == nullptr) {
    void* p = nullptr;
    cudaDriverEntryPointQueryResult q;
    if (cudaGetDriverEntryPoint("cuTensorMapEncodeTiled", &p, cudaEnableDefault, &q) == cudaSuccess &&
        q == cudaDriverEntryPointSuccess)
      fn = reinterpret_cast<EncodeTiledFn>(p);
  }
  return fn;
}

int make_map(CUtensorMap* m, const void* ptr, uint64_t inner, uint64_t rows, uint64_t batch, uint64_t batch2,
             int64_t ld, int64_t bs, int64_t bs2, uint32_t box_rows) {
  EncodeTiledFn fn = get_encode_fn();
  if (fn == nullptr) {
    set_error("cuTensorMapEncodeTiled entry point unavailable (no CUDA driver?)");
    return 1;
  }
  cuuint64_t dims[4] = {inner, rows, batch, batch2};
  if (bs <= 0) bs = static_cast<int64_t>(rows) * ld;
  if (bs2 <= 0) bs2 = static_cast<int64_t>(batch) * bs;
  cuuint64_t strides[3] = {static_cast<cuuint64_t>(ld) * 2, static_cast<cuuint64_t>(bs) * 2,
                           static_cast<cuuint64_t>(bs2) * 2};
  cuuint32_t box[4] = {64, box_rows, 1, 1};
  cuuint32_t estr[4] = {1, 1, 1, 1};
  CUresult r = fn(m, CU_TENSOR_MAP_DATA_TYPE_BFLOAT16, 4, const_cast<void*>(ptr), dims, strides, box, estr,
                  CU_TENSOR_MAP_INTERLEAVE_NONE, CU_TENSOR_MAP_SWIZZLE_128B, CU_TENSOR_MAP_L2_PROMOTION_L2_256B,
                  CU_TENSOR_MAP_FLOAT_OOB_FILL_NONE);
  if (r != CUDA_SUCCESS) {
    set_error("cuTensorMapEncodeTiled failed (%d): ptr=%p dims={%llu,%llu,%llu,%llu} ld=%lld bs=%lld bs2=%lld box_rows=%u",
              static_cast<int>(r), ptr, (unsigned long long)inner, (unsigned long long)rows,
              (unsigned long long)batch, (unsigned long long)batch2, (long long)ld, (long long)bs, (long long)bs2,
              box_rows);
    return 1;
  }
  return 0;
}


static int& streamk_mode() {
  static int mode = []() { const char* e = getenv("MACAW_B200_GEMM_STREAMK"); const int v = e ? atoi(e) : 1; return v < 0 || v > 2 ? 1 : v; }();
  return mode;
}

static int& overlap_mode() {
  static int mode = []() { const char* e = getenv("MACAW_B200_GEMM_OVERLAP"); const int v = e ? atoi(e) : 2; return v < 0 || v > 2 ? 2 : v; }();
  return mode;
}

struct GemmLaunch {
  GemmKParams p;
  mm_gemm_schedule s;
  bool f16;
};

static int plan_gemm(const mm_gemm_args* a, GemmLaunch& L) {
  MM_REQUIRE(a != nullptr, "mm_gemm_fwd: null args");
  MM_REQUIRE(a->M > 0 && a->N > 0 && a->K > 0 && a->batch > 0 && a->batch2 >= 0,
             "mm_gemm_fwd: bad shape M=%d N=%d K=%d batch=%d batch2=%d", a->M, a->N, a->K, a->batch, a->batch2);
  const int batch2 = a->batch2 > 0 ? a->batch2 : 1;
  MM_REQUIRE(a->A && a->B && a->C, "mm_gemm_fwd: null operand");
  MM_REQUIRE((reinterpret_cast<uintptr_t>(a->A) & 15) == 0 && (reinterpret_cast<uintptr_t>(a->B) & 15) == 0,
             "mm_gemm_fwd: A/B must be 16-byte aligned");
  MM_REQUIRE(a->lda % 8 == 0 && a->ldb % 8 == 0, "mm_gemm_fwd: lda/ldb must be multiples of 8 elements (lda=%lld ldb=%lld)",
             (long long)a->lda, (long long)a->ldb);
  MM_REQUIRE(a->batch == 1 || (a->a_bs % 8 == 0 && a->b_bs % 8 == 0), "mm_gemm_fwd: batch strides must be multiples of 8");
  MM_REQUIRE(batch2 == 1 || (a->a_bs2 % 8 == 0 && a->b_bs2 % 8 == 0), "mm_gemm_fwd: batch2 strides must be multiples of 8");
  MM_REQUIRE(a->epi >= MM_EPI_STD && a->epi <= MM_EPI_ROPE, "mm_gemm_fwd: bad epilogue %d", a->epi);
  MM_REQUIRE(a->sumsq_out == nullptr || (a->epi == MM_EPI_STD && !a->c_trans && !a->c_fp32 && a->batch == 1 && batch2 == 1 &&
                                         a->N % 32 == 0),
             "mm_gemm_fwd: sumsq_out needs the standard epilogue, 16-bit output, no batching and N %% 32 == 0");
  MM_REQUIRE(a->rs_sumsq == nullptr || (a->rs_parts > 0 && a->rs_parts % 4 == 0 && !a->c_trans && a->batch == 1 && batch2 == 1 &&
                                        (reinterpret_cast<uintptr_t>(a->rs_sumsq) & 15) == 0),
             "mm_gemm_fwd: rs_sumsq needs rs_parts %% 4 == 0, a 16-byte aligned buffer and no batching");
  MM_REQUIRE(!(a->c_fp16 && a->c_fp32), "mm_gemm_fwd: c_fp16 and c_fp32 are exclusive");
  MM_REQUIRE((a->a_fp16 != 0) == (a->b_fp16 != 0),
             "mm_gemm_fwd: A and B must share one 16-bit format (wgmma takes no mixed f16 x bf16 operands)");
  MM_REQUIRE((!a->bias_rs && !a->bias2 && !a->bias2_rs) || (a->epi == MM_EPI_STD && !a->c_trans),
             "mm_gemm_fwd: row-scaled bias terms need the standard, non-transposed epilogue");
  MM_REQUIRE(!a->c_trans || (a->epi == MM_EPI_STD && a->batch == 1 && batch2 == 1),
             "mm_gemm_fwd: c_trans needs the standard epilogue and no batching");
  MM_REQUIRE(!a->a_mn_major || (a->b_mn_major && a->epi == MM_EPI_STD && !a->c_trans),
             "mm_gemm_fwd: MN-major A needs MN-major B and the standard epilogue");
  MM_REQUIRE(!a->b_mn_major || a->epi == MM_EPI_STD, "mm_gemm_fwd: MN-major B only with the standard epilogue");
  const int esz = a->c_fp32 ? 4 : 2;
  bool vec = (reinterpret_cast<uintptr_t>(a->C) % 16 == 0) && ((a->ldc * esz) % 16 == 0) &&
             ((a->c_bs * esz) % 16 == 0) && ((a->c_bs2 * esz) % 16 == 0);
  if (a->bias) vec = vec && (reinterpret_cast<uintptr_t>(a->bias) % 16 == 0) && (a->bias_bs % 8 == 0);
  if (a->residual)
    vec = vec && (reinterpret_cast<uintptr_t>(a->residual) % 16 == 0) && (a->ldr % 8 == 0) && (a->r_bs % 8 == 0) &&
          (a->r_bs2 % 8 == 0);
  MM_REQUIRE(a->epi != MM_EPI_ROPE || (a->N % 128 == 0 && a->rope_cos && a->rope_sin && a->rope_T > 0 && vec &&
                                       a->rope_cols % 128 == 0),
             "mm_gemm_fwd: RoPE epilogue needs N %% 128 == 0, cos/sin tables and vector-aligned C");
  MM_REQUIRE(a->epi != MM_EPI_SWIGLU || a->N % 64 == 0, "mm_gemm_fwd: SwiGLU epilogue needs N %% 64 == 0");
  GemmKParams& p = L.p;
  p.M = a->M; p.N = a->N; p.K = a->K; p.batch = a->batch; p.batch2 = batch2;
  p.num_k = (a->K + kBlockK - 1) / kBlockK;
  p.m_tiles = (a->M + kBlockM - 1) / kBlockM;
  p.b_shared = (a->batch > 1 && a->b_bs == 0) ? 1 : 0;
  p.b2_shared = (batch2 > 1 && a->b_bs2 == 0) ? 1 : 0;
  p.C = a->C; p.ldc = a->ldc; p.c_bs = a->c_bs; p.c_bs2 = a->c_bs2; p.c_fp32 = a->c_fp32;
  p.act = a->act; p.alpha = a->alpha;
  p.bias = reinterpret_cast<const bf16*>(a->bias); p.bias_bs = a->bias_bs;
  p.row_scale = a->row_scale;
  p.residual = reinterpret_cast<const bf16*>(a->residual); p.ldr = a->ldr; p.r_bs = a->r_bs; p.r_bs2 = a->r_bs2;
  p.res_row_mod = a->res_row_mod;
  p.rope_cos = a->rope_cos; p.rope_sin = a->rope_sin; p.rope_T = a->rope_T; p.rope_cols = a->rope_cols;
  p.rope_pos = a->rope_pos;
  p.c_trans = a->c_trans;
  p.c_fp16 = a->c_fp16;
  p.aux_f16 = act_f16() ? 1 : 0;
  p.bias_rs = a->bias_rs; p.bias2 = reinterpret_cast<const bf16*>(a->bias2); p.bias2_rs = a->bias2_rs;
  p.sumsq_out = a->sumsq_out; p.sumsq_parts = (a->N + 31) / 32;
  p.rs_sumsq = a->rs_sumsq; p.rs_parts = a->rs_parts; p.rs_eps = a->rs_eps;
  p.vec_ok = vec ? 1 : 0;

  const int sms = num_sms();
  int BN = kMaxBN;
  if (a->epi == MM_EPI_STD) {
    const int cands[3] = {128, 64, 32};
    const long long kcost[3] = {512, 282, 192};
    long long best = -1;
    BN = 32;
    for (int i = 0; i < 3; ++i) {
      const int bn = cands[i];
      if (a->b_mn_major && bn < 64) continue;
      if (bn > 32 && a->N <= bn / 2) continue;
      const long long tiles = (long long)a->batch * batch2 * p.m_tiles * ((a->N + bn - 1) / bn);
      const long long waves = (tiles + sms - 1) / sms;
      const long long cost = waves * ((long long)p.num_k * kcost[i] + 2 * kcost[i]);
      if (best < 0 || cost < best) {
        best = cost;
        BN = bn;
      }
    }
    if (a->b_mn_major && BN < 64) BN = 64;
  }
  p.n_tiles = (a->N + BN - 1) / BN;
  const long long tiles = (long long)a->batch * batch2 * p.m_tiles * p.n_tiles;
  {
    const long long unit_bytes = (long long)kBlockM * a->K * 2;
    long long g = ((16LL << 20) + unit_bytes / 2) / unit_bytes;
    g = g < 2 ? 2 : (g > 32 ? 32 : g);
    p.group_m = static_cast<int>(g);
  }
  p.sk_tiles = 0; p.sk_first = 0; p.sk_ws = nullptr; p.sk_flags = nullptr;
  const int sk_env = streamk_mode();
  if (sk_env != 0 && a->sk_workspace != nullptr && p.num_k >= 8 && tiles > sms &&
      static_cast<long long>(sms) * p.num_k * (sms + 1) < (1LL << 31)) {
    const int rem = static_cast<int>(tiles % sms);
    const long long need = 8192 + static_cast<long long>(sms) * kBlockM * BN * 4;
    const bool pays = sk_env == 2 || static_cast<long long>(sms - rem) * p.num_k * BN >= 3400LL * 256;
    if (rem > 0 && pays && a->sk_workspace_bytes >= need &&
        (reinterpret_cast<uintptr_t>(a->sk_workspace) & 15) == 0) {
      p.sk_tiles = rem;
      p.sk_first = static_cast<int>(tiles - rem);
      p.sk_flags = reinterpret_cast<int*>(a->sk_workspace);
      p.sk_ws = reinterpret_cast<float*>(reinterpret_cast<char*>(a->sk_workspace) + 8192);
    }
  }
  const int overlap = overlap_mode();
  const bool ewg = overlap >= 1 && p.num_k >= kEwgMinKBlocks && p.sk_tiles == 0;
  const bool wide = overlap == 2 && ewg && BN == kMaxBN && !a->a_mn_major && !a->b_mn_major && !a->c_trans &&
                    a->batch == 1 && batch2 == 1 && p.n_tiles % 2 == 0 && tiles / 2 >= sms;
  L.f16 = a->a_fp16 != 0;
  mm_gemm_schedule& s = L.s;
  s.block_n = BN; s.m_tiles = p.m_tiles; s.n_tiles = p.n_tiles; s.k_blocks = p.num_k; s.group_m = p.group_m;
  s.units = tiles; s.workers = sms; s.waves = static_cast<int>((tiles + sms - 1) / sms);
  s.streamk_tiles = p.sk_tiles; s.vectorised_epilogue = p.vec_ok;
  s.kernel = wide ? MM_GEMM_KERNEL_TILE_PAIRS : ewg ? MM_GEMM_KERNEL_EPILOGUE_WARPGROUP : MM_GEMM_KERNEL_CONSUMER_EPILOGUE;
  s.threads = wide ? kWideThreads : ewg ? kGemmThreadsEwg : kGemmThreads;
  s.smem_bytes = static_cast<int32_t>(wide ? kWideSmemBytes : gemm_smem_bytes(gemm_stages(BN), BN * kBlockK * 2, BN));
  const long long units = wide ? tiles / 2 : tiles;
  s.grid = static_cast<int>((units < sms && p.sk_tiles == 0) ? units : sms);
  MM_REQUIRE(s.kernel == MM_GEMM_KERNEL_CONSUMER_EPILOGUE || p.sk_tiles == 0,
             "mm_gemm_fwd: only the consumer-epilogue kernel takes a stream-K tail");
  return 0;
}

template <auto kern>
static int launch_gemm(const GemmLaunch& L, const CUtensorMap& ta, const CUtensorMap& tb, cudaStream_t st) {
  static bool attr_set[kMaxDevices] = {};
  if (int rc = ensure_smem_attr(kern, L.s.smem_bytes, attr_set, "mm_gemm_fwd")) return rc;
  cudaError_t e = launch_kernel(kern, dim3(L.s.grid), dim3(L.s.threads), L.s.smem_bytes, st, 1, ta, tb, L.p);
  if (e != cudaSuccess) {
    set_error("mm_gemm_fwd: launch failed: %s", cudaGetErrorString(e));
    return 2;
  }
  return check_launch("mm_gemm_fwd");
}

template <int BN, int EPI, bool B_MN = false, bool A_MN = false>
static int launch_variant(const GemmLaunch& L, const CUtensorMap& ta, const CUtensorMap& tb, cudaStream_t st) {
  if constexpr (BN == kMaxBN && !B_MN && !A_MN)
    if (L.s.kernel == MM_GEMM_KERNEL_TILE_PAIRS)
      return L.f16 ? launch_gemm<&gemm_wide_kernel<EPI, true>>(L, ta, tb, st)
                   : launch_gemm<&gemm_wide_kernel<EPI, false>>(L, ta, tb, st);
  if (L.s.kernel == MM_GEMM_KERNEL_EPILOGUE_WARPGROUP)
    return L.f16 ? launch_gemm<&gemm_bf16_kernel<BN, EPI, B_MN, A_MN, true, true>>(L, ta, tb, st)
                 : launch_gemm<&gemm_bf16_kernel<BN, EPI, B_MN, A_MN, false, true>>(L, ta, tb, st);
  return L.f16 ? launch_gemm<&gemm_bf16_kernel<BN, EPI, B_MN, A_MN, true, false>>(L, ta, tb, st)
               : launch_gemm<&gemm_bf16_kernel<BN, EPI, B_MN, A_MN, false, false>>(L, ta, tb, st);
}

}

using namespace mm;

extern "C" int32_t mm_gemm_fwd(const mm_gemm_args* a, void* stream) {
  GemmLaunch L;
  if (int rc = plan_gemm(a, L)) return rc;
  const int BN = L.s.block_n;
  const int batch2 = L.p.batch2;
  CUtensorMap ta, tb;
  if (a->a_mn_major) {
    if (make_map(&ta, a->A, a->M, a->K, a->batch, batch2, a->lda, a->a_bs, a->a_bs2, 64)) return 1;
  } else if (make_map(&ta, a->A, a->K, a->M, a->batch, batch2, a->lda, a->a_bs, a->a_bs2, kBlockM)) {
    return 1;
  }
  const uint64_t b_batch = L.p.b_shared ? 1 : a->batch;
  const uint64_t b_batch2 = L.p.b2_shared ? 1 : batch2;
  if (!a->b_mn_major) {
    if (make_map(&tb, a->B, a->K, a->N, b_batch, b_batch2, a->ldb, a->b_bs, a->b_bs2, BN)) return 1;
  } else {
    if (make_map(&tb, a->B, a->N, a->K, b_batch, b_batch2, a->ldb, a->b_bs, a->b_bs2, 64)) return 1;
  }
  cudaStream_t st = reinterpret_cast<cudaStream_t>(stream);
#define MM_LAUNCH(...) return launch_variant<__VA_ARGS__>(L, ta, tb, st)
  if (a->epi == MM_EPI_ROPE) MM_LAUNCH(128, MM_EPI_ROPE);
  if (a->epi == MM_EPI_SWIGLU) MM_LAUNCH(128, MM_EPI_SWIGLU);
  if (a->a_mn_major) {
    if (BN == 128) MM_LAUNCH(128, MM_EPI_STD, true, true);
    MM_LAUNCH(64, MM_EPI_STD, true, true);
  }
  if (a->b_mn_major) {
    if (BN == 128) MM_LAUNCH(128, MM_EPI_STD, true);
    MM_LAUNCH(64, MM_EPI_STD, true);
  }
  if (BN == 128) MM_LAUNCH(128, MM_EPI_STD);
  if (BN == 64) MM_LAUNCH(64, MM_EPI_STD);
  MM_LAUNCH(32, MM_EPI_STD);
#undef MM_LAUNCH
}

extern "C" int32_t mm_gemm_plan(const mm_gemm_args* a, mm_gemm_schedule* plan) {
  MM_REQUIRE(plan != nullptr, "mm_gemm_plan: null plan");
  GemmLaunch L;
  if (int rc = plan_gemm(a, L)) return rc;
  *plan = L.s;
  return 0;
}

extern "C" int32_t mm_gemm_streamk_mode(int32_t mode) {
  const int prev = streamk_mode();
  if (mode >= 0 && mode <= 2) streamk_mode() = mode;
  return prev;
}

extern "C" int32_t mm_gemm_overlap_mode(int32_t mode) {
  const int prev = overlap_mode();
  if (mode >= 0 && mode <= 2) overlap_mode() = mode;
  return prev;
}

extern "C" int64_t mm_gemm_streamk_workspace_bytes(void) {
  return 8192 + static_cast<int64_t>(num_sms()) * kBlockM * kMaxBN * 4;
}

namespace mm {
static int make_map_e4m3(CUtensorMap* m, const void* ptr, uint64_t inner, uint64_t rows, uint64_t ld, uint32_t box_rows) {
  EncodeTiledFn fn = get_encode_fn();
  if (fn == nullptr) {
    set_error("cuTensorMapEncodeTiled entry point unavailable (no CUDA driver?)");
    return 1;
  }
  cuuint64_t dims[2] = {inner, rows};
  cuuint64_t strides[1] = {ld};
  cuuint32_t box[2] = {static_cast<cuuint32_t>(kE4m3BlockK), box_rows}, estr[2] = {1, 1};
  const CUresult r = fn(m, CU_TENSOR_MAP_DATA_TYPE_UINT8, 2, const_cast<void*>(ptr), dims, strides, box, estr,
                        CU_TENSOR_MAP_INTERLEAVE_NONE, CU_TENSOR_MAP_SWIZZLE_128B, CU_TENSOR_MAP_L2_PROMOTION_L2_256B,
                        CU_TENSOR_MAP_FLOAT_OOB_FILL_NONE);
  if (r != CUDA_SUCCESS) {
    set_error("mm_gemm_e4m3_fwd: cuTensorMapEncodeTiled failed (%d): ptr=%p %llu x %llu ld=%llu", static_cast<int>(r), ptr,
              (unsigned long long)rows, (unsigned long long)inner, (unsigned long long)ld);
    return 1;
  }
  return 0;
}

static int plan_gemm_e4m3(const mm_gemm_args* a, const mm_gemm_e4m3_args* e, GemmLaunch& L) {
  MM_REQUIRE(a != nullptr && e != nullptr, "mm_gemm_e4m3_fwd: null args");
  MM_REQUIRE(a->M > 0 && a->N > 0 && a->K > 0, "mm_gemm_e4m3_fwd: bad shape M=%d N=%d K=%d", a->M, a->N, a->K);
  MM_REQUIRE(a->K % kE4m3BlockK == 0, "mm_gemm_e4m3_fwd: K %% 128 == 0 required (K=%d)", a->K);
  MM_REQUIRE(a->N % kMaxBN == 0, "mm_gemm_e4m3_fwd: N %% 128 == 0 required (N=%d)", a->N);
  MM_REQUIRE(a->batch == 1 && a->batch2 <= 1 && !a->c_trans && !a->a_mn_major && !a->b_mn_major,
             "mm_gemm_e4m3_fwd: no batching, c_trans or MN-major operands");
  MM_REQUIRE(a->A != nullptr && (reinterpret_cast<uintptr_t>(a->A) & 15) == 0 && a->lda >= a->K && a->lda % 16 == 0,
             "mm_gemm_e4m3_fwd: A must be 16-byte aligned with lda >= K and lda %% 16 == 0 (lda=%lld)", (long long)a->lda);
  MM_REQUIRE(e->a_scale != nullptr, "mm_gemm_e4m3_fwd: null A scales");
  MM_REQUIRE(!e->unpromoted || a->epi == MM_EPI_STD,
             "mm_gemm_e4m3_fwd: the unpromoted comparison instance has the standard epilogue only");
  const mm_w8_matrix& w = e->w;
  MM_REQUIRE(w.N == a->N && w.K == a->K, "mm_gemm_e4m3_fwd: weight is %d x %d, the problem needs %d x %d", w.N, w.K, a->N,
             a->K);
  MM_REQUIRE(w.chunks != nullptr && (reinterpret_cast<uintptr_t>(w.chunks) & 15) == 0,
             "mm_gemm_e4m3_fwd: chunk table (16-byte aligned)");
  MM_REQUIRE(w.gain == nullptr, "mm_gemm_e4m3_fwd: the weight's gain must be null (apply it when quantizing A)");
  MM_REQUIRE(w.q[0] != nullptr, "mm_gemm_e4m3_fwd: weight source 0");
  for (int j = 0; j < MM_W8_MAX_SRC; ++j) {
    MM_REQUIRE(w.q[j] == nullptr || (reinterpret_cast<uintptr_t>(w.q[j]) & 15) == 0,
               "mm_gemm_e4m3_fwd: weight source %d must be 16-byte aligned", j);
    MM_REQUIRE(w.q[j] == nullptr || (w.scale[j] != nullptr && w.rows[j] > 0 && w.rows[j] % 32 == 0),
               "mm_gemm_e4m3_fwd: weight source %d needs non-null scales and a positive multiple of 32 rows", j);
  }
  mm_gemm_args v = *a;
  v.B = w.q[0];
  v.lda = v.ldb = a->K;
  v.a_fp16 = v.b_fp16 = 0;
  v.sk_workspace = nullptr;
  v.sk_workspace_bytes = 0;
  if (int rc = plan_gemm(&v, L)) return rc;
  GemmKParams& p = L.p;
  const int sms = num_sms();
  p.n_tiles = a->N / kMaxBN;
  p.num_k = a->K / kE4m3BlockK;
  {
    const long long unit_bytes = (long long)kBlockM * a->K;
    long long g = ((16LL << 20) + unit_bytes / 2) / unit_bytes;
    p.group_m = static_cast<int>(g < 2 ? 2 : (g > 32 ? 32 : g));
  }
  p.sk_tiles = 0; p.sk_first = 0; p.sk_ws = nullptr; p.sk_flags = nullptr;
  const long long tiles = (long long)p.m_tiles * p.n_tiles;
  mm_gemm_schedule& s = L.s;
  s.block_n = kMaxBN; s.m_tiles = p.m_tiles; s.n_tiles = p.n_tiles; s.k_blocks = p.num_k; s.group_m = p.group_m;
  s.units = tiles; s.workers = sms; s.waves = static_cast<int>((tiles + sms - 1) / sms);
  s.streamk_tiles = 0; s.vectorised_epilogue = p.vec_ok;
  s.kernel = MM_GEMM_KERNEL_CONSUMER_EPILOGUE;
  s.threads = kGemmThreads;
  s.smem_bytes = static_cast<int32_t>(gemm_smem_bytes(gemm_stages(kMaxBN), kMaxBN * kE4m3BlockK, kMaxBN));
  s.grid = static_cast<int>(tiles < sms ? tiles : sms);
  return 0;
}

template <int EPI, bool PROMOTE>
static int launch_e4m3(const GemmLaunch& L, const CUtensorMap (&tm)[4], const E4m3P& e, cudaStream_t st) {
  auto kern = &gemm_e4m3_kernel<EPI, PROMOTE>;
  static bool attr_set[kMaxDevices] = {};
  if (int rc = ensure_smem_attr(kern, L.s.smem_bytes, attr_set, "mm_gemm_e4m3_fwd")) return rc;
  cudaError_t err = launch_kernel(kern, dim3(L.s.grid), dim3(L.s.threads), L.s.smem_bytes, st, 1, tm[0], tm[1], tm[2], tm[3],
                                  L.p, e);
  if (err != cudaSuccess) {
    set_error("mm_gemm_e4m3_fwd: launch failed: %s", cudaGetErrorString(err));
    return 2;
  }
  return check_launch("mm_gemm_e4m3_fwd");
}
}

extern "C" int32_t mm_gemm_e4m3_plan(const mm_gemm_args* a, const mm_gemm_e4m3_args* e, mm_gemm_schedule* plan) {
  MM_REQUIRE(plan != nullptr, "mm_gemm_e4m3_plan: null plan");
  GemmLaunch L;
  if (int rc = plan_gemm_e4m3(a, e, L)) return rc;
  *plan = L.s;
  return 0;
}

extern "C" int32_t mm_gemm_e4m3_fwd(const mm_gemm_args* a, const mm_gemm_e4m3_args* e, void* stream) {
  GemmLaunch L;
  if (int rc = plan_gemm_e4m3(a, e, L)) return rc;
  CUtensorMap tm[4];
  if (make_map_e4m3(&tm[0], a->A, a->K, a->M, a->lda, kBlockM)) return 1;
  const mm_w8_matrix& w = e->w;
  for (int j = 0; j < MM_W8_MAX_SRC; ++j) {
    const int src = w.q[j] != nullptr ? j : 0;
    if (make_map_e4m3(&tm[1 + j], w.q[src], w.K, w.rows[src], w.K, 32)) return 1;
  }
  E4m3P ep = {};
  ep.a_scale = e->a_scale;
  for (int j = 0; j < MM_W8_MAX_SRC; ++j) {
    ep.w_scale[j] = w.q[j] != nullptr ? w.scale[j] : nullptr;
    ep.w_rows[j] = w.q[j] != nullptr ? w.rows[j] : 0;
  }
  ep.chunks = w.chunks;
  cudaStream_t st = reinterpret_cast<cudaStream_t>(stream);
  if (e->unpromoted) return launch_e4m3<MM_EPI_STD, false>(L, tm, ep, st);
  if (a->epi == MM_EPI_ROPE) return launch_e4m3<MM_EPI_ROPE, true>(L, tm, ep, st);
  if (a->epi == MM_EPI_SWIGLU) return launch_e4m3<MM_EPI_SWIGLU, true>(L, tm, ep, st);
  return launch_e4m3<MM_EPI_STD, true>(L, tm, ep, st);
}


namespace mm {
__global__ void splitk_reduce_kernel(const float* __restrict__ part, int splits, int M, int N,
                                     const bf16* __restrict__ bias, bf16* __restrict__ out, long long ldo, int out_fp16,
                                     int bias_f16) {
  const long long total = static_cast<long long>(M) * N;
  for (long long i = blockIdx.x * static_cast<long long>(blockDim.x) + threadIdx.x; i < total;
       i += static_cast<long long>(gridDim.x) * blockDim.x) {
    const int m = static_cast<int>(i / N), n = static_cast<int>(i % N);
    float acc = bias ? aux_ld(bias, n, bias_f16) : 0.0f;
    for (int s = 0; s < splits; ++s) acc += part[static_cast<long long>(s) * total + i];
    if (out_fp16)
      reinterpret_cast<__half*>(out)[static_cast<long long>(m) * ldo + n] = __float2half_rn(acc);
    else
      out[static_cast<long long>(m) * ldo + n] = __float2bfloat16(acc);
  }
}
}

extern "C" int32_t mm_splitk_reduce(const float* partial, int32_t splits, int32_t M, int32_t N, const void* bias,
                                    void* out, int64_t ldo, int32_t out_fp16, void* stream) {
  MM_REQUIRE(partial && out && splits > 0 && M > 0 && N > 0, "mm_splitk_reduce: bad arguments");
  const long long total = static_cast<long long>(M) * N;
  int blocks = static_cast<int>((total + 255) / 256);
  if (blocks > num_sms() * 8) blocks = num_sms() * 8;
  splitk_reduce_kernel<<<blocks, 256, 0, reinterpret_cast<cudaStream_t>(stream)>>>(
      partial, splits, M, N, reinterpret_cast<const bf16*>(bias), reinterpret_cast<bf16*>(out), ldo, out_fp16,
      act_f16() ? 1 : 0);
  return check_launch("mm_splitk_reduce");
}
```

macaw-llm_b200/ops.py:

```python
from __future__ import annotations

import ctypes as C
from typing import Optional

import torch

from . import _lib
from ._lib import AlignArgs, AttnArgs, GemmArgs

ACT_NONE, ACT_GELU, ACT_QUICK_GELU, ACT_SILU = 0, 1, 2, 3
EPI_STD, EPI_SWIGLU, EPI_ROPE = 0, 1, 2
GEMM_CONSUMER_EPILOGUE, GEMM_EPILOGUE_WARPGROUP, GEMM_TILE_PAIRS = 0, 1, 2

_BF16 = torch.bfloat16
_F16 = torch.float16
_ACT_DTYPE = torch.bfloat16


def ACT():
    return _ACT_DTYPE


def set_act_format(dtype) -> None:
    global _ACT_DTYPE
    if dtype not in _16BIT:
        raise TypeError(f"macaw_b200: activation format must be bf16 or fp16, got {dtype}")
    if dtype != _ACT_DTYPE or int(_lib.load().mm_get_act_format()) != int(dtype == _F16):
        _lib.load().mm_set_act_format(int(dtype == _F16))
        _ACT_DTYPE = dtype
_16BIT = (torch.bfloat16, torch.float16)


def _stream() -> int:
    return torch.cuda.current_stream().cuda_stream


def _check(rc: int, what: str) -> None:
    if rc != 0:
        raise RuntimeError(f"{what} failed (rc={rc}): {_lib.last_error()}")


def _cuda(t: torch.Tensor, dtype=None, name: str = "tensor") -> torch.Tensor:
    if not isinstance(t, torch.Tensor) or not t.is_cuda:
        raise RuntimeError(f"macaw_b200: {name} must be a CUDA tensor (no CPU fallback exists)")
    if dtype is not None and t.dtype != dtype:
        raise TypeError(f"macaw_b200: {name} must be {dtype}, got {t.dtype}")
    if t.device.index != torch.cuda.current_device():
        raise RuntimeError(f"macaw_b200: {name} lives on {t.device} but the current CUDA device is "
                           f"cuda:{torch.cuda.current_device()}; wrap the call in torch.cuda.device(...)")
    return t


def _ptr(t: Optional[torch.Tensor]) -> Optional[int]:
    return None if t is None else t.data_ptr()


PROFILE = None
TAG = "gemm"


def launch_count() -> int:
    return int(_lib.load().mm_launch_count())


def launch_count_reset() -> None:
    _lib.load().mm_launch_count_reset()


def gemm_raw(*, M, N, K, A, lda, B, ldb, Cout, ldc, batch=1, a_bs=0, b_bs=0, c_bs=0, batch2=1, a_bs2=0, b_bs2=0,
             c_bs2=0, b_mn_major=False, c_fp32=False, epi=EPI_STD, act=ACT_NONE, alpha=1.0, bias=None, bias_bs=0,
             row_scale=None, residual=None, ldr=0, r_bs=0, r_bs2=0, res_row_mod=0, rope_cos=None, rope_sin=None,
             rope_T=0, rope_cols=0, rope_pos=None, c_trans=False, a_fp16=None, b_fp16=None, c_fp16=None,
             bias_rs=None, bias2=None, bias2_rs=None, a_mn_major=False, sumsq_out=None, rs_sumsq=None, rs_parts=0,
             rs_eps=0.0, streamk=None, plan_only: bool = False, e4m3: Optional[_lib.GemmE4m3Args] = None):
    f16 = ACT() == _F16
    a_fp16 = f16 if a_fp16 is None else a_fp16
    b_fp16 = f16 if b_fp16 is None else b_fp16
    c_fp16 = (f16 and not c_fp32) if c_fp16 is None else c_fp16
    if isinstance(streamk, torch.Tensor):
        streamk = (streamk.data_ptr(), streamk.numel() * streamk.element_size())
    a = GemmArgs(M, N, K, batch, batch2, A, lda, a_bs, a_bs2, B, ldb, b_bs, b_bs2, int(b_mn_major), Cout, ldc, c_bs,
                 c_bs2, int(c_fp32), epi, act, float(alpha), bias, bias_bs, row_scale, residual, ldr, r_bs, r_bs2,
                 res_row_mod, rope_cos, rope_sin, rope_T, rope_cols, rope_pos, int(c_trans), int(a_fp16), int(b_fp16), int(c_fp16),
                 bias_rs, bias2, bias2_rs, int(a_mn_major), sumsq_out, rs_sumsq, int(rs_parts), float(rs_eps),
                 None if streamk is None else streamk[0], 0 if streamk is None else streamk[1])
    if plan_only or PLANS is not None:
        plan = _plan_of(a, e4m3)
        if plan_only:
            return plan
        PLANS.append(plan)
    if e4m3 is None:
        fwd, args, what = _lib.load().mm_gemm_fwd, (C.byref(a),), "mm_gemm_fwd"
    else:
        fwd, args, what = _lib.load().mm_gemm_e4m3_fwd, (C.byref(a), C.byref(e4m3)), "mm_gemm_e4m3_fwd"
    if PROFILE is None:
        _check(fwd(*args, _stream()), what)
        return
    e0, e1 = torch.cuda.Event(enable_timing=True), torch.cuda.Event(enable_timing=True)
    e0.record()
    _check(fwd(*args, _stream()), what)
    e1.record()
    PROFILE.append((TAG, 2.0 * M * N * K * batch * max(1, batch2), e0, e1))


def gemm_plan(*, M: int, N: int, K: int, batch: int = 1, batch2: int = 1, epi: int = EPI_STD, b_mn_major: bool = False,
              a_mn_major: bool = False, c_fp32: bool = False, c_trans: bool = False, fp16: bool = False,
              streamk: bool = False) -> dict:
    lib = _lib.load()
    fake = 1 << 20
    lda = M if a_mn_major else K
    ldb = N if b_mn_major else K
    n_out = N // 2 if epi == EPI_SWIGLU else N
    ldc = M if c_trans else n_out
    ws = int(lib.mm_gemm_streamk_workspace_bytes()) if streamk else 0
    rope = dict(rope_cos=fake, rope_sin=fake, rope_T=max(1, M), rope_cols=(N // 128) * 128) if epi == EPI_ROPE else {}
    kw = dict(M=M, N=N, K=K, batch=batch, batch2=batch2, A=fake, lda=lda, a_bs=M * K, a_bs2=M * K * batch, B=fake, ldb=ldb,
              b_bs=N * K, b_bs2=N * K * batch, b_mn_major=int(b_mn_major), C=fake, ldc=ldc, c_bs=M * n_out,
              c_bs2=M * n_out * batch, c_fp32=int(c_fp32), epi=epi, act=ACT_NONE, alpha=1.0, c_trans=int(c_trans),
              a_fp16=int(fp16), b_fp16=int(fp16), c_fp16=int(fp16 and not c_fp32), a_mn_major=int(a_mn_major),
              sk_workspace=fake if streamk else None, sk_workspace_bytes=ws, **rope)
    return _plan_of(GemmArgs(**kw))


PLANS = None


def _plan_of(a: GemmArgs, e4m3=None) -> dict:
    plan = _lib.GemmPlan()
    if e4m3 is None:
        _check(_lib.load().mm_gemm_plan(C.byref(a), C.byref(plan)), "mm_gemm_plan")
    else:
        _check(_lib.load().mm_gemm_e4m3_plan(C.byref(a), C.byref(e4m3), C.byref(plan)), "mm_gemm_e4m3_plan")
    d = {name: int(getattr(plan, name)) for name, _ in _lib.GemmPlan._fields_}
    d["fill"] = d["units"] / float(d["waves"] * d["workers"])
    return d


def linear(x: torch.Tensor, w: torch.Tensor, bias: Optional[torch.Tensor] = None, *, act: int = ACT_NONE,
           residual: Optional[torch.Tensor] = None, res_row_mod: int = 0, out: Optional[torch.Tensor] = None,
           out_fp32: bool = False, alpha: float = 1.0, row_scale: Optional[torch.Tensor] = None, epi: int = EPI_STD,
           rope=None, out_dtype=None, sumsq_out: Optional[torch.Tensor] = None, rms_from=None) -> torch.Tensor:
    _cuda(x, None, "x"); _cuda(w, None, "w")
    assert x.dtype in _16BIT and w.dtype in _16BIT, (x.dtype, w.dtype)
    assert x.dim() == 2 and w.dim() == 2 and x.shape[1] == w.shape[1], (x.shape, w.shape)
    assert x.stride(1) == 1 and w.stride(1) == 1
    M, K = x.shape
    N = w.shape[0]
    n_out = N // 2 if epi == EPI_SWIGLU else N
    if out is None:
        out = torch.empty((M, n_out), device=x.device,
                          dtype=out_dtype if out_dtype is not None else (torch.float32 if out_fp32 else ACT()))
    assert out.shape[0] == M and out.shape[1] == n_out and out.stride(1) == 1
    kw = {}
    if residual is not None:
        _cuda(residual, ACT(), "residual")
        assert residual.stride(-1) == 1
        kw.update(residual=residual.data_ptr(), ldr=residual.stride(0), res_row_mod=res_row_mod)
    if rope is not None:
        cos, sin, T, cols = rope[:4]
        kw.update(rope_cos=cos.data_ptr(), rope_sin=sin.data_ptr(), rope_T=T, rope_cols=cols)
        if len(rope) > 4 and rope[4] is not None:
            kw.update(rope_pos=rope[4].data_ptr())
    if sumsq_out is not None:
        assert sumsq_out.dtype == torch.float32 and sumsq_out.is_contiguous() and sumsq_out.shape == (M, (N + 31) // 32)
        kw.update(sumsq_out=sumsq_out.data_ptr())
    if rms_from is not None:
        parts, eps = rms_from
        assert parts.dtype == torch.float32 and parts.is_contiguous() and parts.shape[0] == M and row_scale is None
        kw.update(rs_sumsq=parts.data_ptr(), rs_parts=parts.shape[1], rs_eps=eps)
    if STREAMK is not None and STREAMK.device == x.device:
        kw.update(streamk=STREAMK)
    gemm_raw(M=M, N=N, K=K, A=x.data_ptr(), lda=x.stride(0), B=w.data_ptr(), ldb=w.stride(0), Cout=out.data_ptr(),
             ldc=out.stride(0), c_fp32=out.dtype == torch.float32, c_fp16=out.dtype == _F16, a_fp16=x.dtype == _F16,
             b_fp16=w.dtype == _F16, epi=epi, act=act, alpha=alpha, bias=_ptr(bias), row_scale=_ptr(row_scale), **kw)
    return out


STREAMK: Optional[torch.Tensor] = None


def streamk_workspace(device) -> torch.Tensor:
    _lib.load()
    with torch.cuda.device(device):
        n = int(_lib.load().mm_gemm_streamk_workspace_bytes())
    return torch.zeros((n + 15) // 16 * 4, device=device, dtype=torch.int32)


def linear_thin(x: torch.Tensor, w: torch.Tensor, bias: Optional[torch.Tensor] = None, *, act: int = ACT_NONE,
                residual: Optional[torch.Tensor] = None, out: Optional[torch.Tensor] = None,
                row_scale: Optional[torch.Tensor] = None) -> torch.Tensor:
    _cuda(x, ACT(), "x"); _cuda(w, ACT(), "w")
    M, K = x.shape
    N = w.shape[0]
    assert x.stride(1) == 1 and w.stride(1) == 1 and w.shape[1] == K
    if out is None:
        out = torch.empty((M, N), device=x.device, dtype=ACT())
    assert out.shape == (M, N) and out.stride(1) == 1
    kw = {}
    if residual is not None:
        assert residual.stride(1) == 1
        kw.update(residual=residual.data_ptr(), ldr=residual.stride(0))
    if STREAMK is not None and STREAMK.device == x.device:
        kw.update(streamk=STREAMK)
    gemm_raw(M=N, N=M, K=K, A=w.data_ptr(), lda=w.stride(0), B=x.data_ptr(), ldb=x.stride(0), Cout=out.data_ptr(),
             ldc=out.stride(0), c_fp32=out.dtype == torch.float32, act=act, bias=_ptr(bias), row_scale=_ptr(row_scale),
             c_trans=True, **kw)
    return out


THIN_SPLITS = 4


THIN_RES, THIN_SWIGLU, THIN_QKV = 0, 1, 2


def linear_thin_fused(x: torch.Tensor, w: torch.Tensor, mode: int, *, row_scale: Optional[torch.Tensor] = None,
                      rms_from=None, residual: Optional[torch.Tensor] = None, out: Optional[torch.Tensor] = None,
                      sumsq_out: Optional[torch.Tensor] = None, rope=None, cache: Optional[torch.Tensor] = None, t0: int = 0,
                      t0_dev: Optional[torch.Tensor] = None, splits: Optional[int] = None) -> torch.Tensor:
    _cuda(x, ACT(), "x"); _cuda(w, ACT(), "w")
    M, K = x.shape
    N = w.shape[0]
    assert x.stride(1) == 1 and w.stride(1) == 1 and w.shape[1] == K and M <= 64
    sk = None
    S = THIN_SPLITS if splits is None else int(splits)
    if S < 1 or K % (S * 64) != 0:
        S = 1
    Kc = K // S
    Mp = (M + 3) // 4 * 4
    dev = x.device
    part = torch.empty((S, N, Mp), device=dev, dtype=torch.float32)
    gemm_raw(M=N, N=M, K=Kc, batch=S, A=w.data_ptr(), lda=w.stride(0), a_bs=Kc, B=x.data_ptr(), ldb=x.stride(0), b_bs=Kc,
             Cout=part.data_ptr(), ldc=Mp, c_bs=N * Mp, c_fp32=True, streamk=sk)
    return _thin_tail(part, M, K, mode, row_scale=row_scale, rms_from=rms_from, residual=residual, out=out,
                      sumsq_out=sumsq_out, rope=rope, cache=cache, t0=t0, t0_dev=t0_dev)


def _thin_tail(part: torch.Tensor, M: int, K: int, mode: int, *, row_scale=None, rms_from=None, residual=None, out=None,
               sumsq_out=None, rope=None, cache=None, t0: int = 0, t0_dev=None) -> torch.Tensor:
    S, N, Mp = part.shape
    dev = part.device
    n_out = N // 2 if mode == THIN_SWIGLU else N
    if out is None:
        out = torch.empty((M, n_out), device=dev, dtype=ACT())
    assert out.shape == (M, n_out) and out.stride(1) == 1
    a = _lib.ThinArgs()
    a.part, a.splits, a.N, a.M, a.ldp, a.mode = part.data_ptr(), S, N, M, Mp, int(mode)
    a.row_scale = _ptr(row_scale)
    if rms_from is not None:
        parts, eps = rms_from
        assert row_scale is None and parts.dtype == torch.float32 and parts.is_contiguous() and parts.shape[0] == M
        a.rs_sumsq, a.rs_parts, a.rs_K, a.rs_eps = parts.data_ptr(), parts.shape[1], K, float(eps)
    if residual is not None:
        _cuda(residual, ACT(), "residual")
        assert mode == THIN_RES and residual.stride(1) == 1
        a.residual, a.ldr = residual.data_ptr(), residual.stride(0)
    a.out, a.ldo = out.data_ptr(), out.stride(0)
    if sumsq_out is not None:
        assert mode == THIN_RES and sumsq_out.dtype == torch.float32 and sumsq_out.is_contiguous() and sumsq_out.shape == (M, N // 32)
        a.sumsq_out = sumsq_out.data_ptr()
    if mode == THIN_QKV:
        cos, sin, pos_dev = rope
        _cuda(cache, ACT(), "cache")
        E = N // 3
        assert cache.is_contiguous() and cache.dim() == 4 and cache.shape[0] == M and cache.shape[2] == 2 and cache.shape[3] == E
        a.rope_cos, a.rope_sin, a.pos_dev, a.E = cos.data_ptr(), sin.data_ptr(), _ptr(pos_dev), E
        a.cache, a.Tmax, a.t0, a.t0_dev = cache.data_ptr(), cache.shape[1], int(t0), _ptr(t0_dev)
    _check(_lib.load().mm_thin_fused(C.byref(a), _stream()), "mm_thin_fused")
    return out


_W8_FORMAT = {torch.bfloat16: 0, torch.float16: 1, torch.float32: 2}


def quantize_rows_int8(w: torch.Tensor):
    if not isinstance(w, torch.Tensor) or w.dim() != 2 or w.dtype not in _W8_FORMAT or w.stride(1) != 1:
        raise TypeError("macaw_b200: quantize_rows_int8 takes a 2-D bf16 / fp16 / fp32 tensor with unit column stride")
    _cuda(w, None, "w")
    rows, K = w.shape
    q = torch.empty((rows, K), device=w.device, dtype=torch.int8)
    s = torch.empty((rows,), device=w.device, dtype=torch.float32)
    _check(_lib.load().mm_quantize_rows_int8(w.data_ptr(), w.stride(0), _W8_FORMAT[w.dtype], rows, K, q.data_ptr(),
                                             s.data_ptr(), _stream()), "mm_quantize_rows_int8")
    return q, s


def w8_chunk_map(rows, interleave: bool = False) -> torch.Tensor:
    rows = [int(r) for r in rows]
    if any(r <= 0 or r % 32 for r in rows):
        raise ValueError(f"macaw_b200: fused sources need a positive multiple of 32 rows, got {rows}")
    if interleave:
        if len(rows) != 2 or rows[0] != rows[1]:
            raise ValueError(f"macaw_b200: an interleaved fused matrix has two sources of equal height, got {rows}")
        c = torch.arange(2 * rows[0] // 32)
        return torch.stack([c % 2, 32 * (c // 2)], 1).to(torch.int32)
    return torch.cat([torch.stack([torch.full((r // 32,), j), 32 * torch.arange(r // 32)], 1)
                      for j, r in enumerate(rows)]).to(torch.int32)


_W8_CHUNKS = {}


class W8Matrix:

    def __init__(self, qs, scales, interleave: bool = False, gain: Optional[torch.Tensor] = None):
        qs, scales = list(qs), list(scales)
        if not 1 <= len(qs) <= _lib.W8_MAX_SRC or len(scales) != len(qs):
            raise ValueError(f"macaw_b200: a fused int8 weight has 1..{_lib.W8_MAX_SRC} sources, each with its scales")
        K = qs[0].shape[1]
        self.fp8 = qs[0].dtype == _E4M3
        for q, s in zip(qs, scales):
            if self.fp8 and (q.dtype != _E4M3 or q.dim() != 2 or not q.is_contiguous() or q.shape[1] != K):
                raise TypeError("macaw_b200: e4m3 sources must be contiguous (rows, K) float8_e4m3fn tensors with one K")
            if not self.fp8 and (q.dtype != torch.int8 or q.dim() != 2 or not q.is_contiguous() or q.shape[1] != K):
                raise TypeError("macaw_b200: int8 sources must be contiguous (rows, K) int8 tensors with one K")
            if s.dtype != torch.float32 or tuple(s.shape) != (q.shape[0],) or not s.is_contiguous():
                raise TypeError("macaw_b200: each source needs a contiguous fp32 scale per row")
        chunks = w8_chunk_map([q.shape[0] for q in qs], interleave)
        N = 32 * chunks.shape[0]
        if N % 64 or K % 16:
            raise ValueError(f"macaw_b200: int8 weights need N % 64 == 0 and K % 16 == 0, got N={N}, K={K}")
        if gain is not None and (gain.dtype != ACT() or tuple(gain.shape) != (K,) or not gain.is_contiguous()):
            raise TypeError(f"macaw_b200: the gain must be a contiguous ({K},) {ACT()} tensor")
        for i, t in enumerate(qs + scales + ([gain] if gain is not None else [])):
            _cuda(t, None, f"int8 weight operand {i}")
        dev = qs[0].device
        key = (tuple(q.shape[0] for q in qs), bool(interleave), str(dev))
        dchunks = _W8_CHUNKS.get(key)
        if dchunks is None:
            dchunks = _W8_CHUNKS[key] = chunks.to(dev)
        self.N, self.K, self.gain = N, K, gain
        self._keep = (qs, scales, dchunks, gain)
        self.args = _lib.W8Matrix()
        for j, (q, s) in enumerate(zip(qs, scales)):
            self.args.q[j], self.args.scale[j], self.args.rows[j] = q.data_ptr(), s.data_ptr(), q.shape[0]
        self.args.chunks, self.args.N, self.args.K, self.args.gain = dchunks.data_ptr(), N, K, _ptr(gain)


def dequant_rows(w: W8Matrix, out: Optional[torch.Tensor] = None) -> torch.Tensor:
    dev = w._keep[0][0].device
    if out is None:
        out = torch.empty((w.N, w.K), device=dev, dtype=ACT())
    _cuda(out, ACT(), "out")
    assert out.shape == (w.N, w.K) and out.stride(1) == 1
    _check(_lib.load().mm_dequant_rows(C.byref(w.args), out.data_ptr(), out.stride(0), _stream()), "mm_dequant_rows")
    return out


def w8_thin_splits(N: int, K: int, n_sms: int) -> int:
    return min((K + 127) // 128, max(2, -(-2 * n_sms // (N // 64))))


def linear_w8_thin_fused(x: torch.Tensor, w: W8Matrix, mode: int, *, splits: Optional[int] = None, **tail) -> torch.Tensor:
    _cuda(x, ACT(), "x")
    M, K = x.shape
    assert x.stride(1) == 1 and K == w.K and 1 <= M <= 64
    dev = x.device
    S = w8_thin_splits(w.N, K, torch.cuda.get_device_properties(dev).multi_processor_count) if splits is None else int(splits)
    Mp = (M + 3) // 4 * 4
    part = torch.empty((S, w.N, Mp), device=dev, dtype=torch.float32)
    xs_work = torch.empty((M, (K + 127) // 128 * 128), device=dev, dtype=ACT())
    fn, what = (_lib.load().mm_gemm_e4m3_thin, "mm_gemm_e4m3_thin") if w.fp8 else (_lib.load().mm_gemm_w8_thin, "mm_gemm_w8_thin")
    _check(fn(C.byref(w.args), x.data_ptr(), x.stride(0), M, part.data_ptr(), S, Mp, xs_work.data_ptr(), _stream()), what)
    return _thin_tail(part, M, K, mode, **tail)


_E4M3 = torch.float8_e4m3fn


def quantize_rows_e4m3(x: torch.Tensor, gain: Optional[torch.Tensor] = None):
    if not isinstance(x, torch.Tensor) or x.dim() != 2 or x.dtype not in _W8_FORMAT or x.stride(1) != 1:
        raise TypeError("macaw_b200: quantize_rows_e4m3 takes a 2-D bf16 / fp16 / fp32 tensor with unit column stride")
    _cuda(x, None, "x")
    rows, K = x.shape
    if gain is not None:
        _cuda(gain, ACT(), "gain")
        assert tuple(gain.shape) == (K,) and gain.is_contiguous()
    q = torch.empty((rows, K), device=x.device, dtype=_E4M3)
    s = torch.empty((rows,), device=x.device, dtype=torch.float32)
    args = (x.data_ptr(), x.stride(0), _W8_FORMAT[x.dtype], rows, K, _ptr(gain), q.data_ptr(), K, s.data_ptr(), _stream())
    if PROFILE is None:
        _check(_lib.load().mm_quantize_rows_e4m3(*args), "mm_quantize_rows_e4m3")
        return q, s
    e0, e1 = torch.cuda.Event(enable_timing=True), torch.cuda.Event(enable_timing=True)
    e0.record()
    _check(_lib.load().mm_quantize_rows_e4m3(*args), "mm_quantize_rows_e4m3")
    e1.record()
    PROFILE.append((TAG + ".quantize", 0.0, e0, e1))
    return q, s


def _e4m3_args(a_scale: int, w: W8Matrix, unpromoted: bool) -> _lib.GemmE4m3Args:
    if not w.fp8:
        raise TypeError("macaw_b200: the e4m3 GEMM needs an e4m3 weight")
    e = _lib.GemmE4m3Args()
    e.a_scale, e.unpromoted = a_scale, int(unpromoted)
    C.memmove(C.byref(e.w), C.byref(w.args), C.sizeof(_lib.W8Matrix))
    e.w.gain = None
    return e


def linear_e4m3(xq: torch.Tensor, xs: torch.Tensor, w: W8Matrix, *, epi: int = EPI_STD, residual=None,
                out: Optional[torch.Tensor] = None, out_dtype=None, row_scale: Optional[torch.Tensor] = None, rope=None,
                sumsq_out: Optional[torch.Tensor] = None, rms_from=None, unpromoted: bool = False,
                plan_only: bool = False):
    _cuda(xq, _E4M3, "xq"); _cuda(xs, torch.float32, "xs")
    M, K = xq.shape
    assert xq.stride(1) == 1 and xs.shape == (M,) and xs.is_contiguous() and K == w.K
    N = w.N
    n_out = N // 2 if epi == EPI_SWIGLU else N
    if out is None:
        out = torch.empty((M, n_out), device=xq.device, dtype=out_dtype if out_dtype is not None else ACT())
    assert out.shape == (M, n_out) and out.stride(1) == 1
    kw = {}
    if residual is not None:
        _cuda(residual, ACT(), "residual")
        assert residual.stride(-1) == 1
        kw.update(residual=residual.data_ptr(), ldr=residual.stride(0))
    if rope is not None:
        cos, sin, T, cols = rope[:4]
        kw.update(rope_cos=cos.data_ptr(), rope_sin=sin.data_ptr(), rope_T=T, rope_cols=cols)
        if len(rope) > 4 and rope[4] is not None:
            kw.update(rope_pos=rope[4].data_ptr())
    if sumsq_out is not None:
        assert sumsq_out.dtype == torch.float32 and sumsq_out.is_contiguous() and sumsq_out.shape == (M, (N + 31) // 32)
        kw.update(sumsq_out=sumsq_out.data_ptr())
    if rms_from is not None:
        parts, eps = rms_from
        assert parts.dtype == torch.float32 and parts.is_contiguous() and parts.shape[0] == M and row_scale is None
        kw.update(rs_sumsq=parts.data_ptr(), rs_parts=parts.shape[1], rs_eps=eps)
    e = _e4m3_args(xs.data_ptr(), w, unpromoted)
    plan = gemm_raw(M=M, N=N, K=K, A=xq.data_ptr(), lda=xq.stride(0), B=0, ldb=K, Cout=out.data_ptr(), ldc=out.stride(0),
                    c_fp32=out.dtype == torch.float32, c_fp16=out.dtype == _F16, epi=epi, row_scale=_ptr(row_scale),
                    plan_only=plan_only, e4m3=e, **kw)
    return plan if plan_only else out


def gemm_e4m3_plan(*, M: int, N: int, K: int, epi: int = EPI_STD, rows=None, lda: Optional[int] = None,
                   a_scale: bool = True, w_scale: bool = True) -> dict:
    lib = _lib.load()
    fake = 1 << 20
    rows = [N] if rows is None else list(rows)
    n_out = N // 2 if epi == EPI_SWIGLU else N
    rope = dict(rope_cos=fake, rope_sin=fake, rope_T=max(1, M), rope_cols=(N // 128) * 128) if epi == EPI_ROPE else {}
    a = GemmArgs(M=M, N=N, K=K, batch=1, batch2=1, A=fake, lda=K if lda is None else lda, B=fake, ldb=K, C=fake,
                 ldc=n_out, epi=epi, alpha=1.0, c_fp16=int(ACT() == _F16), **rope)
    e = _lib.GemmE4m3Args()
    e.a_scale = fake if a_scale else None
    for j, r in enumerate(rows):
        e.w.q[j], e.w.scale[j], e.w.rows[j] = fake, fake if w_scale else None, r
    e.w.chunks, e.w.N, e.w.K = fake, N, K
    return _plan_of(a, e)


def splitk_reduce(partial: torch.Tensor, bias: Optional[torch.Tensor], out: torch.Tensor) -> torch.Tensor:
    _cuda(partial, torch.float32, "partial"); _cuda(out, None, "out")
    assert out.dtype in _16BIT
    S, M, N = partial.shape
    _check(_lib.load().mm_splitk_reduce(partial.data_ptr(), S, M, N, _ptr(bias), out.data_ptr(), out.stride(0),
                                        int(out.dtype == _F16), _stream()), "mm_splitk_reduce")
    return out


def attention(q: torch.Tensor, k: torch.Tensor, v: torch.Tensor, *, scale: float, causal: bool = False,
              key_mask: Optional[torch.Tensor] = None, out: Optional[torch.Tensor] = None,
              tk_dev: Optional[torch.Tensor] = None) -> torch.Tensor:
    for n, t in (("q", q), ("k", k), ("v", v)):
        _cuda(t, ACT(), n)
        assert t.dim() == 4 and t.stride(3) == 1
    B, Tq, H, hd = q.shape
    Tk = k.shape[1]
    if out is None:
        out = torch.empty((B, Tq, H, hd), device=q.device, dtype=ACT())
    if key_mask is not None:
        _cuda(key_mask, torch.int32, "key_mask")
        assert key_mask.shape == (B, Tk) and key_mask.is_contiguous()
    a = AttnArgs(q.data_ptr(), k.data_ptr(), v.data_ptr(), out.data_ptr(), B, H, Tq, Tk, hd,
                 q.stride(0), q.stride(1), q.stride(2), k.stride(0), k.stride(1), k.stride(2),
                 v.stride(0), v.stride(1), v.stride(2), out.stride(0), out.stride(1), out.stride(2),
                 _ptr(key_mask), int(causal), float(scale), _ptr(tk_dev))
    _check(_lib.load().mm_attn_fwd(C.byref(a), _stream()), "mm_attn_fwd")
    return out


def rmsnorm(x: torch.Tensor, w: torch.Tensor, eps: float, out: Optional[torch.Tensor] = None) -> torch.Tensor:
    _cuda(x, ACT(), "x"); _cuda(w, ACT(), "w")
    assert x.is_contiguous()
    cols = x.shape[-1]
    rows = x.numel() // cols
    if out is None:
        out = torch.empty_like(x)
    _check(_lib.load().mm_rmsnorm_fwd(x.data_ptr(), w.data_ptr(), out.data_ptr(), rows, cols, float(eps), _stream()),
           "mm_rmsnorm_fwd")
    return out


def rms_rstd(x: torch.Tensor, eps: float) -> torch.Tensor:
    _cuda(x, ACT(), "x")
    assert x.is_contiguous()
    cols = x.shape[-1]
    rows = x.numel() // cols
    out = torch.empty((rows,), device=x.device, dtype=torch.float32)
    _check(_lib.load().mm_rms_rstd(x.data_ptr(), out.data_ptr(), rows, cols, float(eps), _stream()), "mm_rms_rstd")
    return out


def layernorm(x: torch.Tensor, w: torch.Tensor, b: torch.Tensor, eps: float,
              out: Optional[torch.Tensor] = None) -> torch.Tensor:
    _cuda(x, ACT(), "x"); _cuda(w, ACT(), "w"); _cuda(b, ACT(), "b")
    assert x.dim() == 2 and x.stride(1) == 1
    rows, cols = x.shape
    if out is None:
        out = torch.empty((rows, cols), device=x.device, dtype=ACT())
    _check(_lib.load().mm_layernorm_fwd(x.data_ptr(), x.stride(0), w.data_ptr(), b.data_ptr(), out.data_ptr(),
                                        out.stride(0), rows, cols, float(eps), _stream()), "mm_layernorm_fwd")
    return out


def embed_gather(table: torch.Tensor, ids: torch.Tensor, out: Optional[torch.Tensor] = None) -> torch.Tensor:
    _cuda(table, ACT(), "table"); _cuda(ids, None, "ids")
    ids64 = ids.reshape(-1).to(torch.int64).contiguous()
    n, dim = ids64.numel(), table.shape[1]
    if out is None:
        out = torch.empty((n, dim), device=table.device, dtype=ACT())
    assert out.stride(-1) == 1
    _check(_lib.load().mm_embed_gather(table.data_ptr(), table.shape[0], dim, ids64.data_ptr(), n, out.data_ptr(),
                                       out.stride(0), _stream()), "mm_embed_gather")
    return out


def splice_prefix(text: torch.Tensor, prefix: Optional[torch.Tensor], mask_in: Optional[torch.Tensor],
                  labels_in: Optional[torch.Tensor]):
    _cuda(text, ACT(), "text")
    B, L, E = text.shape
    P = 0 if prefix is None else prefix.shape[1]
    assert text.is_contiguous() and (prefix is None or prefix.is_contiguous())
    dst = torch.empty((B, P + L, E), device=text.device, dtype=ACT())
    mask_out = labels_out = None
    if mask_in is not None:
        mask_in = _cuda(mask_in, None, "attention_mask").to(torch.int64).contiguous()
        mask_out = torch.empty((B, P + L), device=text.device, dtype=torch.int64)
    if labels_in is not None:
        labels_in = _cuda(labels_in, None, "labels").to(torch.int64).contiguous()
        labels_out = torch.empty((B, P + L), device=text.device, dtype=torch.int64)
    _check(_lib.load().mm_splice_prefix(text.data_ptr(), _ptr(prefix), dst.data_ptr(), B, L, P, E, _ptr(mask_in),
                                        _ptr(mask_out), _ptr(labels_in), _ptr(labels_out), _stream()),
           "mm_splice_prefix")
    return dst, mask_out, labels_out


def patchify(images: torch.Tensor, patch: int, ldo: int) -> torch.Tensor:
    _cuda(images, ACT(), "images")
    assert images.is_contiguous()
    B, Cc, H, W = images.shape
    out = torch.empty((B * (H // patch) * (W // patch), ldo), device=images.device, dtype=ACT())
    _check(_lib.load().mm_patchify(images.data_ptr(), B, Cc, H, W, patch, out.data_ptr(), ldo, _stream()),
           "mm_patchify")
    return out


def transpose_pad(x: torch.Tensor, pad: int) -> torch.Tensor:
    _cuda(x, ACT(), "x")
    assert x.is_contiguous()
    B, Cc, T = x.shape
    out = torch.empty((B, T + 2 * pad, Cc), device=x.device, dtype=ACT())
    _check(_lib.load().mm_transpose_pad(x.data_ptr(), B, Cc, T, pad, out.data_ptr(), _stream()), "mm_transpose_pad")
    return out


def cast_f16(x: torch.Tensor) -> torch.Tensor:
    _cuda(x, torch.bfloat16, "x")
    assert x.is_contiguous()
    cols = x.shape[-1]
    rows = x.numel() // cols
    y = torch.empty(x.shape, device=x.device, dtype=_F16)
    _check(_lib.load().mm_cast_bf16_f16(x.data_ptr(), cols, y.data_ptr(), cols, rows, cols, _stream()), "mm_cast_bf16_f16")
    return y


def add_rows(x: torch.Tensor, add: Optional[torch.Tensor], out: torch.Tensor) -> torch.Tensor:
    _cuda(x, ACT(), "x"); _cuda(out, ACT(), "out")
    rows, cols = x.shape
    assert x.stride(1) == 1 and out.stride(1) == 1 and out.shape == x.shape
    if add is None:
        _check(_lib.load().mm_copy_rows(x.data_ptr(), x.stride(0), out.data_ptr(), out.stride(0), rows, cols,
                                        _stream()), "mm_copy_rows")
    else:
        _cuda(add, ACT(), "add")
        assert add.stride(1) == 1 and add.shape[1] == cols
        _check(_lib.load().mm_add_rows(x.data_ptr(), x.stride(0), add.data_ptr(), add.stride(0), add.shape[0],
                                       out.data_ptr(), out.stride(0), rows, cols, _stream()), "mm_add_rows")
    return out


ALIGN_MODE = 0


def align_fused(table: torch.Tensor, qt: torch.Tensor, stats: torch.Tensor, out: Optional[torch.Tensor] = None,
                mode: Optional[int] = None, keep: Optional[dict] = None):
    _cuda(table, _F16, "table"); _cuda(qt, _F16, "qt"); _cuda(stats, torch.float32, "stats")
    R, E = qt.shape
    V = table.shape[0]
    assert table.shape[1] == E and table.stride(1) == 1 and qt.stride(1) == 1 and stats.shape == (R, 2) and stats.is_contiguous()
    dev = qt.device
    if out is None:
        out = torch.empty((R, E), device=dev, dtype=_F16)
    assert out.shape == (R, E) and out.stride(1) == 1 and out.dtype == _F16
    Vp = (V + 7) // 8 * 8
    P = torch.empty((R, Vp), device=dev, dtype=_F16)
    lib = _lib.load()
    ws = torch.empty((int(lib.mm_align_workspace_bytes(R, V)) + 15) // 16 * 4, device=dev, dtype=torch.int32)
    psum = torch.empty((R,), device=dev, dtype=torch.float32)
    pext = torch.empty((R,), device=dev, dtype=torch.float32)
    inv_l = torch.empty((R,), device=dev, dtype=torch.float32) if keep is not None else None
    a = AlignArgs(table.data_ptr(), V, E, table.stride(0), qt.data_ptr(), R, qt.stride(0), stats.data_ptr(),
                  stats.data_ptr() + 4, 2, out.data_ptr(), out.stride(0), psum.data_ptr(), pext.data_ptr(), P.data_ptr(), Vp,
                  ws.data_ptr(), ALIGN_MODE if mode is None else int(mode), _ptr(inv_l))
    if keep is not None:
        keep.update(P=P, inv_l=inv_l)
    if PROFILE is None:
        _check(lib.mm_align_fwd(C.byref(a), _stream()), "mm_align_fwd")
    else:
        e0, e1 = torch.cuda.Event(enable_timing=True), torch.cuda.Event(enable_timing=True)
        e0.record()
        _check(lib.mm_align_fwd(C.byref(a), _stream()), "mm_align_fwd")
        e1.record()
        PROFILE.append(("align.fused", 4.0 * R * V * E, e0, e1))
    return out, psum, pext


def kv_append(qkv: torch.Tensor, B: int, T_new: int, cache: torch.Tensor, t0: int,
              t0_dev: Optional[torch.Tensor] = None) -> None:
    _cuda(qkv, ACT(), "qkv"); _cuda(cache, ACT(), "cache")
    E = cache.shape[-1]
    assert qkv.shape == (B * T_new, 3 * E) and qkv.stride(1) == 1 and cache.is_contiguous() and cache.shape[2] == 2
    _check(_lib.load().mm_kv_append(qkv.data_ptr(), qkv.stride(0), B, T_new, E, cache.data_ptr(), cache.shape[1], t0,
                                    _ptr(t0_dev), _stream()), "mm_kv_append")


def rope_rows(x: torch.Tensor, rot_cols: int, cos: torch.Tensor, sin: torch.Tensor, rope_T: int,
              pos_dev: Optional[torch.Tensor] = None) -> torch.Tensor:
    _cuda(x, ACT(), "x")
    assert x.dim() == 2 and x.stride(1) == 1
    _check(_lib.load().mm_rope_rows(x.data_ptr(), x.stride(0), x.shape[0], rot_cols, cos.data_ptr(), sin.data_ptr(), rope_T,
                                    _ptr(pos_dev), _stream()), "mm_rope_rows")
    return x


def argmax_rows(logits: torch.Tensor) -> torch.Tensor:
    _cuda(logits, ACT(), "logits")
    assert logits.dim() == 2 and logits.stride(1) == 1
    out = torch.empty((logits.shape[0],), device=logits.device, dtype=torch.int64)
    _check(_lib.load().mm_argmax_rows(logits.data_ptr(), logits.stride(0), logits.shape[0], logits.shape[1],
                                      out.data_ptr(), _stream()), "mm_argmax_rows")
    return out


def sample_rows(logits: torch.Tensor, seen: torch.Tensor, *, do_sample: bool, repetition_penalty: float = 1.0,
                temperature: float = 1.0, top_k: int = 0, top_p: float = 1.0, seed_dev: Optional[torch.Tensor] = None,
                step_dev: Optional[torch.Tensor] = None) -> torch.Tensor:
    _cuda(logits, ACT(), "logits"); _cuda(seen, torch.int32, "seen")
    assert logits.dim() == 2 and logits.stride(1) == 1
    rows, V = logits.shape
    assert seen.is_contiguous() and tuple(seen.shape) == (rows, (V + 31) // 32)
    if do_sample:
        _cuda(seed_dev, torch.int64, "seed_dev"); _cuda(step_dev, torch.int32, "step_dev")
    out = torch.empty((rows,), device=logits.device, dtype=torch.int64)
    _check(_lib.load().mm_sample_rows(logits.data_ptr(), logits.stride(0), rows, V, seen.data_ptr(),
                                      float(repetition_penalty), float(temperature), int(top_k), float(top_p),
                                      int(bool(do_sample)), _ptr(seed_dev), _ptr(step_dev), out.data_ptr(), _stream()),
           "mm_sample_rows")
    return out


def ce_loss(logits: torch.Tensor, labels: torch.Tensor) -> torch.Tensor:
    return ce_loss_with_count(logits, labels)[0]


def gemm_dx(dy: torch.Tensor, w: torch.Tensor, out: Optional[torch.Tensor] = None, accumulate: bool = False) -> torch.Tensor:
    _cuda(dy, ACT(), "dy"); _cuda(w, ACT(), "w")
    M, N = dy.shape
    K = w.shape[1]
    assert w.shape[0] == N and dy.stride(1) == 1 and w.stride(1) == 1
    if out is None:
        assert not accumulate
        out = torch.empty((M, K), device=dy.device, dtype=ACT())
    kw = dict(residual=out.data_ptr(), ldr=out.stride(0)) if accumulate else {}
    gemm_raw(M=M, N=K, K=N, A=dy.data_ptr(), lda=dy.stride(0), B=w.data_ptr(), ldb=w.stride(0), b_mn_major=True,
             Cout=out.data_ptr(), ldc=out.stride(0), **kw)
    return out


def gemm_dw(dy: torch.Tensor, x: torch.Tensor, out: torch.Tensor, accumulate: bool) -> torch.Tensor:
    _cuda(dy, ACT(), "dy"); _cuda(x, ACT(), "x"); _cuda(out, ACT(), "dw")
    M, N = dy.shape
    K = x.shape[1]
    assert x.shape[0] == M and out.shape == (N, K) and dy.stride(1) == 1 and x.stride(1) == 1 and out.stride(1) == 1
    kw = dict(residual=out.data_ptr(), ldr=out.stride(0)) if accumulate else {}
    gemm_raw(M=N, N=K, K=M, A=dy.data_ptr(), lda=dy.stride(0), a_mn_major=True, B=x.data_ptr(), ldb=x.stride(0),
             b_mn_major=True, Cout=out.data_ptr(), ldc=out.stride(0), **kw)
    return out


def rmsnorm_bwd(dy: torch.Tensor, x: torch.Tensor, rstd: torch.Tensor, g: torch.Tensor, dres: Optional[torch.Tensor],
                dg: Optional[torch.Tensor]) -> torch.Tensor:
    _cuda(dy, ACT(), "dy"); _cuda(x, ACT(), "x"); _cuda(rstd, torch.float32, "rstd"); _cuda(g, ACT(), "g")
    assert dy.is_contiguous() and x.is_contiguous() and (dres is None or dres.is_contiguous())
    rows, cols = x.shape
    dx = torch.empty_like(x)
    lib = _lib.load()
    parts = None
    if dg is not None:
        with torch.cuda.device(x.device):
            parts = torch.empty((int(lib.mm_rmsnorm_bwd_parts(rows)), cols), device=x.device, dtype=torch.float32)
    _check(lib.mm_rmsnorm_bwd(dy.data_ptr(), x.data_ptr(), rstd.data_ptr(), g.data_ptr(), _ptr(dres), dx.data_ptr(),
                              _ptr(dg), _ptr(parts), rows, cols, _stream()), "mm_rmsnorm_bwd")
    return dx


def swiglu_fwd(gate: torch.Tensor, up: torch.Tensor) -> torch.Tensor:
    _cuda(gate, ACT(), "gate"); _cuda(up, ACT(), "up")
    assert gate.is_contiguous() and up.is_contiguous() and gate.shape == up.shape
    h = torch.empty_like(gate)
    _check(_lib.load().mm_swiglu_fwd(gate.data_ptr(), up.data_ptr(), h.data_ptr(), gate.numel(), _stream()), "mm_swiglu_fwd")
    return h


def swiglu_bwd(dh: torch.Tensor, gate: torch.Tensor, up: torch.Tensor):
    _cuda(dh, ACT(), "dh")
    assert dh.is_contiguous() and gate.is_contiguous() and up.is_contiguous()
    dg, du = torch.empty_like(gate), torch.empty_like(up)
    _check(_lib.load().mm_swiglu_bwd(dh.data_ptr(), gate.data_ptr(), up.data_ptr(), dg.data_ptr(), du.data_ptr(), dh.numel(),
                                     _stream()), "mm_swiglu_bwd")
    return dg, du


def _drop_args(dropout):
    if dropout is None:
        return 0.0, None, 0
    p, seed, sid = dropout
    if float(p) <= 0.0:
        return 0.0, None, 0
    assert seed.is_cuda and seed.dtype == torch.int64 and seed.numel() == 1
    return float(p), seed.data_ptr(), int(sid)


def dropout_mask(rows: int, cols: int, dropout, device) -> torch.Tensor:
    p, seed, sid = _drop_args(dropout)
    out = torch.empty((rows, cols), device=device, dtype=torch.float32)
    _check(_lib.load().mm_dropout_mask(out.data_ptr(), cols, rows, cols, p, seed, sid, _stream()), "mm_dropout_mask")
    return out


def attention_train_fwd(q: torch.Tensor, k: torch.Tensor, v: torch.Tensor, *, scale: float, causal: bool = False,
                        key_mask: Optional[torch.Tensor] = None, dropout=None) -> torch.Tensor:
    for n, t in (("q", q), ("k", k), ("v", v)):
        _cuda(t, ACT(), n)
        assert t.dim() == 4 and t.stride(3) == 1
    B, Tq, H, hd = q.shape
    Tk = k.shape[1]
    dev = q.device
    Tp = (Tk + 7) // 8 * 8
    S = torch.empty((B, H, Tq, Tp), device=dev, dtype=torch.float32)
    gemm_raw(M=Tq, N=Tk, K=hd, batch=H, batch2=B, A=q.data_ptr(), lda=q.stride(1), a_bs=q.stride(2), a_bs2=q.stride(0),
             B=k.data_ptr(), ldb=k.stride(1), b_bs=k.stride(2), b_bs2=k.stride(0), Cout=S.data_ptr(), ldc=Tp, c_bs=Tq * Tp,
             c_bs2=H * Tq * Tp, c_fp32=True)
    P = torch.empty((B, H, Tq, Tp), device=dev, dtype=ACT())
    if key_mask is not None:
        _cuda(key_mask, torch.int32, "key_mask")
    pd, seed, sid = _drop_args(dropout)
    _check(_lib.load().mm_attn_softmax_fwd(S.data_ptr(), P.data_ptr(), B, H, Tq, Tk, Tp, float(scale), int(causal),
                                           _ptr(key_mask), pd, seed, sid, _stream()), "mm_attn_softmax_fwd")
    del S
    o = torch.empty((B, Tq, H, hd), device=dev, dtype=ACT())
    gemm_raw(M=Tq, N=hd, K=Tk, batch=H, batch2=B, A=P.data_ptr(), lda=Tp, a_bs=Tq * Tp, a_bs2=H * Tq * Tp,
             B=v.data_ptr(), ldb=v.stride(1), b_bs=v.stride(2), b_bs2=v.stride(0), b_mn_major=True, Cout=o.data_ptr(),
             ldc=o.stride(1), c_bs=o.stride(2), c_bs2=o.stride(0))
    return o


def attention_bwd(q: torch.Tensor, k: torch.Tensor, v: torch.Tensor, do: torch.Tensor, *, scale: float, causal: bool,
                  key_mask: Optional[torch.Tensor] = None, dropout=None):
    for n, t in (("q", q), ("k", k), ("v", v), ("do", do)):
        _cuda(t, ACT(), n)
        assert t.dim() == 4 and t.stride(3) == 1
    B, Tq, H, hd = q.shape
    Tk = k.shape[1]
    dev = q.device
    Tp = (Tk + 7) // 8 * 8
    S = torch.empty((B, H, Tq, Tp), device=dev, dtype=torch.float32)
    dP = torch.empty((B, H, Tq, Tp), device=dev, dtype=torch.float32)

    def bat(t):
        return dict(ld=t.stride(1), bs=t.stride(2), bs2=t.stride(0))

    s_alpha, k_scale, g_alpha = (float(scale), 1.0, float(scale)) if ACT() == _F16 else (1.0, float(scale), 1.0)

    def scores(a, b, out, alpha=1.0):
        sa, sb = bat(a), bat(b)
        gemm_raw(M=Tq, N=Tk, K=hd, batch=H, batch2=B, A=a.data_ptr(), lda=sa["ld"], a_bs=sa["bs"], a_bs2=sa["bs2"],
                 B=b.data_ptr(), ldb=sb["ld"], b_bs=sb["bs"], b_bs2=sb["bs2"], Cout=out.data_ptr(), ldc=Tp, c_bs=Tq * Tp,
                 c_bs2=H * Tq * Tp, c_fp32=True, alpha=alpha)

    scores(q, k, S, s_alpha)
    scores(do, v, dP)
    P = torch.empty((B, H, Tq, Tp), device=dev, dtype=ACT())
    dS = torch.empty((B, H, Tq, Tp), device=dev, dtype=ACT())
    if key_mask is not None:
        _cuda(key_mask, torch.int32, "key_mask")
    pd, seed, sid = _drop_args(dropout)
    _check(_lib.load().mm_attn_softmax_bwd(S.data_ptr(), dP.data_ptr(), P.data_ptr(), dS.data_ptr(), B, H, Tq, Tk, Tp,
                                           k_scale, int(causal), _ptr(key_mask), pd, seed, sid, _stream()),
           "mm_attn_softmax_bwd")
    del S, dP
    dq = torch.empty((B, Tq, H, hd), device=dev, dtype=ACT())
    dk = torch.empty((B, Tk, H, hd), device=dev, dtype=ACT())
    dv = torch.empty((B, Tk, H, hd), device=dev, dtype=ACT())

    def pt_x(p_, x_, out, alpha=1.0):
        sx, so = bat(x_), bat(out)
        gemm_raw(M=Tk, N=hd, K=Tq, batch=H, batch2=B, A=p_.data_ptr(), lda=Tp, a_bs=Tq * Tp, a_bs2=H * Tq * Tp,
                 a_mn_major=True, B=x_.data_ptr(), ldb=sx["ld"], b_bs=sx["bs"], b_bs2=sx["bs2"], b_mn_major=True,
                 Cout=out.data_ptr(), ldc=so["ld"], c_bs=so["bs"], c_bs2=so["bs2"], alpha=alpha)

    pt_x(P, do, dv)
    pt_x(dS, q, dk, g_alpha)
    sk, so = bat(k), bat(dq)
    gemm_raw(M=Tq, N=hd, K=Tk, batch=H, batch2=B, A=dS.data_ptr(), lda=Tp, a_bs=Tq * Tp, a_bs2=H * Tq * Tp,
             B=k.data_ptr(), ldb=sk["ld"], b_bs=sk["bs"], b_bs2=sk["bs2"], b_mn_major=True, Cout=dq.data_ptr(),
             ldc=so["ld"], c_bs=so["bs"], c_bs2=so["bs2"], alpha=g_alpha)
    return dq, dk, dv


def ce_loss_with_count(logits: torch.Tensor, labels: torch.Tensor):
    _cuda(logits, ACT(), "logits"); _cuda(labels, torch.int64, "labels")
    assert logits.is_contiguous() and labels.is_contiguous()
    B, T, V = logits.shape
    acc = torch.zeros((2,), device=logits.device, dtype=torch.float32)
    cnt = acc[1:].view(torch.int32)
    _check(_lib.load().mm_ce_loss(logits.data_ptr(), labels.data_ptr(), B, T, V, acc.data_ptr(), cnt.data_ptr(),
                                  _stream()), "mm_ce_loss")
    return acc[0] / cnt[0].to(torch.float32), cnt


def ce_bwd(logits: torch.Tensor, labels: torch.Tensor, n_valid: torch.Tensor, grad_scale=1.0) -> torch.Tensor:
    B, T, V = logits.shape
    gs_dev = None
    if isinstance(grad_scale, torch.Tensor):
        gs_dev = _cuda(grad_scale.reshape(1).to(torch.float32), torch.float32, "grad_scale")
        grad_scale = 1.0
    _check(_lib.load().mm_ce_bwd(logits.data_ptr(), labels.data_ptr(), logits.data_ptr(), B, T, V, n_valid.data_ptr(),
                                 float(grad_scale), _ptr(gs_dev), _stream()), "mm_ce_bwd")
    return logits


def embed_scatter_add(dx: torch.Tensor, ids: torch.Tensor, dtable: torch.Tensor) -> None:
    _cuda(dx, ACT(), "dx"); _cuda(dtable, ACT(), "dtable")
    ids64 = ids.reshape(-1).to(torch.int64).contiguous()
    assert dx.dim() == 2 and dx.stride(1) == 1 and dx.shape[0] == ids64.numel() and dtable.is_contiguous()
    _check(_lib.load().mm_embed_scatter_add(dx.data_ptr(), dx.stride(0), ids64.data_ptr(), ids64.numel(), dx.shape[1],
                                            dtable.shape[0], dtable.data_ptr(), _stream()), "mm_embed_scatter_add")


def colsum(x: torch.Tensor, out: torch.Tensor) -> torch.Tensor:
    _cuda(x, ACT(), "x"); _cuda(out, torch.float32, "out")
    assert x.dim() == 2 and x.stride(1) == 1 and out.numel() == x.shape[1]
    _check(_lib.load().mm_colsum(x.data_ptr(), x.stride(0), x.shape[0], x.shape[1], out.data_ptr(), _stream()), "mm_colsum")
    return out


def adamw(p: torch.Tensor, g: torch.Tensor, master: torch.Tensor, m: torch.Tensor, v: torch.Tensor, *, lr: float,
          beta1: float, beta2: float, eps: float, weight_decay: float, step: int, grad_scale: float = 1.0,
          step_dev: Optional[torch.Tensor] = None, grad_mult_dev: Optional[torch.Tensor] = None,
          skip_dev: Optional[torch.Tensor] = None, lr_dev: Optional[torch.Tensor] = None) -> None:
    _cuda(p, ACT(), "p"); _cuda(g, ACT(), "g")
    assert p.is_contiguous() and g.is_contiguous() and master.numel() == p.numel()
    _check(_lib.load().mm_adamw(p.data_ptr(), g.data_ptr(), master.data_ptr(), m.data_ptr(), v.data_ptr(), p.numel(),
                                float(lr), float(beta1), float(beta2), float(eps), float(weight_decay), int(step),
                                _ptr(step_dev), float(grad_scale), _ptr(grad_mult_dev), _ptr(skip_dev), _ptr(lr_dev),
                                _stream()),
           "mm_adamw")


LR_SCHEDULE_KINDS = {"linear": 0, "cosine": 1, "constant_with_warmup": 2}


def lr_schedule(step_dev: torch.Tensor, lr_out: torch.Tensor, *, base_lr: float, kind: str, warmup_steps: int,
                training_steps: int) -> None:
    _cuda(step_dev, torch.int32, "step_dev"); _cuda(lr_out, torch.float32, "lr_out")
    assert step_dev.numel() == 1 and lr_out.numel() == 1
    if kind not in LR_SCHEDULE_KINDS:
        raise ValueError(f"lr_schedule: unknown kind {kind!r}; supported: {', '.join(LR_SCHEDULE_KINDS)}")
    _check(_lib.load().mm_lr_schedule(step_dev.data_ptr(), float(base_lr), LR_SCHEDULE_KINDS[kind], int(warmup_steps),
                                      int(training_steps), lr_out.data_ptr(), _stream()), "mm_lr_schedule")


class HostBlock:

    def __init__(self, nbytes: int):
        if nbytes <= 0:
            raise ValueError("HostBlock: nbytes must be > 0")
        h, d = C.c_void_p(), C.c_void_p()
        _check(_lib.load().mm_host_alloc(int(nbytes), C.byref(h), C.byref(d)), "mm_host_alloc")
        self.nbytes, self.host, self.dev = int(nbytes), int(h.value), int(d.value)
        self._flat = torch.frombuffer((C.c_char * self.nbytes).from_address(self.host), dtype=torch.uint8)

    def view(self, offset: int, numel: int) -> torch.Tensor:
        if offset % 16 or offset < 0 or offset + 4 * numel > self.nbytes:
            raise ValueError(f"HostBlock.view: [{offset}, {offset + 4 * numel}) is not a 16-byte aligned range of the block")
        return self._flat[offset:offset + 4 * numel].view(torch.float32)

    def dev_ptr(self, t: torch.Tensor) -> int:
        off = t.data_ptr() - self.host
        if t.device.type != "cpu" or t.dtype != torch.float32 or not t.is_contiguous() or off < 0 or \
                off + 4 * t.numel() > self.nbytes:
            raise ValueError("HostBlock.dev_ptr: not a contiguous float32 view of this block")
        return self.dev + off

    def free(self) -> None:
        if self.host:
            self._flat = None
            _check(_lib.load().mm_host_free(self.host), "mm_host_free")
            self.host = self.dev = 0


def host_alloc(nbytes: int) -> HostBlock:
    return HostBlock(nbytes)


def adamw_host(p: torch.Tensor, g: torch.Tensor, master: torch.Tensor, m: torch.Tensor, v: torch.Tensor, *,
               block: HostBlock, lr: float, beta1: float, beta2: float, eps: float, weight_decay: float, step: int,
               grad_scale: float = 1.0, step_dev: Optional[torch.Tensor] = None,
               grad_mult_dev: Optional[torch.Tensor] = None, skip_dev: Optional[torch.Tensor] = None,
               lr_dev: Optional[torch.Tensor] = None) -> None:
    _cuda(p, ACT(), "p"); _cuda(g, ACT(), "g")
    assert p.is_contiguous() and g.is_contiguous() and master.numel() == m.numel() == v.numel() == p.numel()
    _check(_lib.load().mm_adamw_host(p.data_ptr(), g.data_ptr(), block.dev_ptr(master), block.dev_ptr(m), block.dev_ptr(v),
                                     p.numel(), float(lr), float(beta1), float(beta2), float(eps), float(weight_decay),
                                     int(step), _ptr(step_dev), float(grad_scale), _ptr(grad_mult_dev), _ptr(skip_dev),
                                     _ptr(lr_dev), _stream()),
           "mm_adamw_host")


def grad_sumsq_parts(n: int) -> int:
    return int(_lib.load().mm_grad_sumsq_parts(int(n)))


def grad_sumsq(g: torch.Tensor, out: torch.Tensor, partials: Optional[torch.Tensor] = None) -> torch.Tensor:
    _cuda(g, None, "g"); _cuda(out, torch.float32, "out")
    assert g.dtype in _16BIT and g.is_contiguous() and out.numel() == 1
    n = g.numel()
    if partials is None:
        partials = torch.empty((grad_sumsq_parts(n),), device=g.device, dtype=torch.float32)
    assert partials.dtype == torch.float32 and partials.numel() >= grad_sumsq_parts(n)
    _check(_lib.load().mm_grad_sumsq(g.data_ptr(), n, int(g.dtype == _F16), out.data_ptr(), partials.data_ptr(), _stream()),
           "mm_grad_sumsq")
    return out


LOSS_SCALE_STATE_WORDS = 12


def loss_scale_update(state: torch.Tensor, sumsq: torch.Tensor, *, max_norm: Optional[float], dynamic: bool,
                      window: int, hysteresis: int, min_scale: float) -> None:
    _cuda(state, torch.int32, "state"); _cuda(sumsq, torch.float32, "sumsq")
    assert state.numel() == LOSS_SCALE_STATE_WORDS and state.is_contiguous() and sumsq.numel() == 1
    _check(_lib.load().mm_loss_scale_update(state.data_ptr(), sumsq.data_ptr(), float(max_norm or 0.0), int(dynamic),
                                            int(window), int(hysteresis), float(min_scale), _stream()),
           "mm_loss_scale_update")


def cast_bf16(x: torch.Tensor) -> torch.Tensor:
    _cuda(x, _F16, "x")
    assert x.is_contiguous()
    cols = x.shape[-1]
    rows = x.numel() // cols
    y = torch.empty(x.shape, device=x.device, dtype=torch.bfloat16)
    _check(_lib.load().mm_cast_f16_bf16(x.data_ptr(), cols, y.data_ptr(), cols, rows, cols, _stream()), "mm_cast_f16_bf16")
    return y


def align_dropout_fwd(P_unnorm: torch.Tensor, inv_l: torch.Tensor, pe: torch.Tensor, V: int, dropout):
    _cuda(P_unnorm, _F16, "P")
    R, ldp = P_unnorm.shape
    dev = P_unnorm.device
    Pm = torch.empty_like(P_unnorm)
    rs, psum_d, pext_d = (torch.empty((R,), device=dev, dtype=torch.float32) for _ in range(3))
    pd, seed, sid = _drop_args(dropout)
    _check(_lib.load().mm_align_dropout_fwd(P_unnorm.data_ptr(), Pm.data_ptr(), ldp, inv_l.data_ptr(), pe.data_ptr(),
                                            rs.data_ptr(), psum_d.data_ptr(), pext_d.data_ptr(), R, V, pd, seed, sid,
                                            _stream()), "mm_align_dropout_fwd")
    return Pm, rs, psum_d, pext_d


def align_softmax_bwd(G: torch.Tensor, P_unnorm: torch.Tensor, inv_l: torch.Tensor, dpsr: torch.Tensor, pe: torch.Tensor,
                      dpe: torch.Tensor, gscale: float, V: int, dropout=None):
    _cuda(G, torch.float32, "G"); _cuda(P_unnorm, _F16, "P")
    R, ldp = P_unnorm.shape
    assert G.shape[0] == R and G.stride(1) == 1 and P_unnorm.stride(1) == 1
    for t in (inv_l, dpsr, pe, dpe):
        assert t.dtype == torch.float32 and t.is_contiguous() and t.numel() == R
    P = torch.empty((R, ldp), device=G.device, dtype=ACT())
    dS = torch.empty((R, ldp), device=G.device, dtype=ACT())
    dstats = torch.empty((2, R), device=G.device, dtype=torch.float32)
    pd, seed, sid = _drop_args(dropout)
    _check(_lib.load().mm_align_softmax_bwd(G.data_ptr(), G.stride(0), P_unnorm.data_ptr(), ldp, inv_l.data_ptr(), dpsr.data_ptr(),
                                            pe.data_ptr(), dpe.data_ptr(), float(gscale), P.data_ptr(), dS.data_ptr(), ldp,
                                            dstats.data_ptr(), R, V, pd, seed, sid, _stream()), "mm_align_softmax_bwd")
    return P, dS, dstats


def head_weighted_colsum(x: torch.Tensor, w: torch.Tensor, head_dim: int, out: torch.Tensor) -> torch.Tensor:
    _cuda(x, None, "x"); _cuda(w, torch.float32, "w"); _cuda(out, torch.float32, "out")
    assert x.dtype in _16BIT and x.stride(1) == 1 and w.is_contiguous()
    Nq, E = x.shape
    assert w.numel() == (E // head_dim) * Nq and out.numel() == E
    _check(_lib.load().mm_head_weighted_colsum(x.data_ptr(), x.stride(0), int(x.dtype == _F16), w.data_ptr(), 1, Nq, E,
                                               head_dim, out.data_ptr(), _stream()), "mm_head_weighted_colsum")
    return out


def window_gather_add(dwin: torch.Tensor, B: int, N: int, C: int, Lq: int, kk: int, ss: int) -> torch.Tensor:
    _cuda(dwin, ACT(), "dwin")
    assert dwin.is_contiguous() and dwin.shape == (B * Lq, kk * C)
    out = torch.empty((B, N, C), device=dwin.device, dtype=ACT())
    _check(_lib.load().mm_window_gather_add(dwin.data_ptr(), B, N, C, Lq, kk, ss, out.data_ptr(), _stream()),
           "mm_window_gather_add")
    return out


def _lora_args(M: int, K: int, N: int, r: int, n: int, scaling: float = 1.0, dropout=None) -> "_lib.LoraArgs":
    assert 1 <= n <= _lib.LORA_MAX
    a = _lib.LoraArgs()
    a.n, a.M, a.K, a.N, a.r, a.scaling = n, M, K, N, r, float(scaling)
    if dropout is not None and float(dropout[0]) > 0.0:
        p, seed, sids = dropout
        _cuda(seed, torch.int64, "seed")
        assert seed.numel() == 1 and len(sids) == n
        a.p_drop, a.seed_dev = float(p), seed.data_ptr()
        for j, s in enumerate(sids):
            a.sid[j] = int(s)
    return a


def _lora_weights(As, Bs):
    for A in As:
        _cuda(A, ACT(), "lora_A")
        assert A.is_contiguous()
    for Bw in Bs:
        _cuda(Bw, ACT(), "lora_B")
        assert Bw.is_contiguous()


def lora_down(x: torch.Tensor, As, dropout=None):
    _cuda(x, ACT(), "x")
    _lora_weights(As, ())
    assert x.dim() == 2 and x.stride(1) == 1
    M, K = x.shape
    r = As[0].shape[0]
    assert all(A.shape == (r, K) for A in As)
    a = _lora_args(M, K, 1, r, len(As), dropout=dropout)
    a.x, a.ldx = x.data_ptr(), x.stride(0)
    us = [torch.empty((M, r), device=x.device, dtype=torch.float32) for _ in As]
    for j, (A, u) in enumerate(zip(As, us)):
        a.A[j], a.u[j] = A.data_ptr(), u.data_ptr()
    _check(_lib.load().mm_lora_down(C.byref(a), _stream()), "mm_lora_down")
    return us


def lora_up(ys, us, Bs, scaling: float, rope=None) -> None:
    _lora_weights((), Bs)
    M, N = ys[0].shape
    r = Bs[0].shape[1]
    for y, u, Bw in zip(ys, us, Bs):
        _cuda(y, ACT(), "y"); _cuda(u, torch.float32, "u")
        assert y.shape == (M, N) and y.stride(1) == 1 and y.stride(0) == ys[0].stride(0)
        assert u.shape == (M, r) and u.is_contiguous() and Bw.shape == (N, r)
    a = _lora_args(M, 8, N, r, len(ys), scaling)
    a.ldy = ys[0].stride(0)
    for j, (y, u, Bw) in enumerate(zip(ys, us, Bs)):
        a.y[j], a.u[j], a.B[j] = y.data_ptr(), u.data_ptr(), Bw.data_ptr()
    if rope is not None:
        cos, sin, T = rope
        a.rope_cos, a.rope_sin, a.rope_T = cos.data_ptr(), sin.data_ptr(), int(T)
    _check(_lib.load().mm_lora_up(C.byref(a), _stream()), "mm_lora_up")


def lora_bwd_dy(dys, us, Bs, dBs, scaling: float, accumulate):
    _lora_weights((), Bs)
    M, N = dys[0].shape
    r = Bs[0].shape[1]
    for dy, u, Bw, dB in zip(dys, us, Bs, dBs):
        _cuda(dy, ACT(), "dy"); _cuda(u, torch.float32, "u"); _cuda(dB, ACT(), "dB")
        assert dy.shape == (M, N) and dy.stride(1) == 1 and dy.stride(0) == dys[0].stride(0)
        assert u.shape == (M, r) and u.is_contiguous() and Bw.shape == (N, r) and dB.shape == (N, r) and dB.is_contiguous()
    a = _lora_args(M, 8, N, r, len(dys), scaling)
    a.ldy = dys[0].stride(0)
    gs = [torch.empty((M, r), device=dys[0].device, dtype=torch.float32) for _ in dys]
    for j, (dy, u, Bw, dB, g) in enumerate(zip(dys, us, Bs, dBs, gs)):
        a.y[j], a.u[j], a.B[j], a.dB[j], a.g[j] = dy.data_ptr(), u.data_ptr(), Bw.data_ptr(), dB.data_ptr(), g.data_ptr()
        a.accumulate[j] = int(bool(accumulate[j]))
    lib = _lib.load()
    ws = torch.empty(((int(lib.mm_lora_workspace_bytes(C.byref(a), 2)) + 15) // 16 * 4,), device=dys[0].device,
                     dtype=torch.float32)
    a.workspace, a.workspace_bytes = ws.data_ptr(), ws.numel() * 4
    _check(lib.mm_lora_bwd_dy(C.byref(a), _stream()), "mm_lora_bwd_dy")
    return gs


def lora_bwd_x(x: torch.Tensor, gs, As, dAs, dx: torch.Tensor, accumulate, dropout=None) -> None:
    _cuda(x, ACT(), "x"); _cuda(dx, ACT(), "dx")
    _lora_weights(As, ())
    M, K = x.shape
    r = As[0].shape[0]
    assert x.stride(1) == 1 and dx.shape == (M, K) and dx.stride(1) == 1
    for g, A, dA in zip(gs, As, dAs):
        _cuda(g, torch.float32, "g"); _cuda(dA, ACT(), "dA")
        assert g.shape == (M, r) and g.is_contiguous() and A.shape == (r, K) and dA.shape == (r, K) and dA.is_contiguous()
    a = _lora_args(M, K, 1, r, len(As), dropout=dropout)
    a.x, a.ldx, a.dx, a.lddx = x.data_ptr(), x.stride(0), dx.data_ptr(), dx.stride(0)
    for j, (g, A, dA) in enumerate(zip(gs, As, dAs)):
        a.g[j], a.A[j], a.dA[j] = g.data_ptr(), A.data_ptr(), dA.data_ptr()
        a.accumulate[j] = int(bool(accumulate[j]))
    lib = _lib.load()
    ws = torch.empty(((int(lib.mm_lora_workspace_bytes(C.byref(a), 3)) + 15) // 16 * 4,), device=x.device,
                     dtype=torch.float32)
    a.workspace, a.workspace_bytes = ws.data_ptr(), ws.numel() * 4
    _check(lib.mm_lora_bwd_x(C.byref(a), _stream()), "mm_lora_bwd_x")


def jpeg_decode(data: torch.Tensor, desc: torch.Tensor, layout: dict):
    _cuda(data, torch.uint8, "data"); _cuda(desc, torch.uint8, "desc")
    dev = data.device
    coef = torch.empty(layout["coef"], dtype=torch.int16, device=dev)
    planes = torch.empty(layout["planes"], dtype=torch.uint8, device=dev)
    out = torch.empty(layout["out"], dtype=torch.uint8, device=dev)
    status = torch.empty(layout["n_images"], dtype=torch.int32, device=dev)
    base, off = desc.data_ptr(), layout["off"]
    a = _lib.JpegArgs(layout["n_images"], layout["n_segments"], layout["n_huff"], layout["n_quant"], data.data_ptr(),
                      layout["data_bytes"], base + off["images"], base + off["segments"], base + off["huff"],
                      base + off["quant"], coef.data_ptr(), coef.numel(), planes.data_ptr(), planes.numel(),
                      out.data_ptr(), out.numel(), status.data_ptr(), layout["max_blocks"], layout["max_pixels"])
    _check(_lib.load().mm_jpeg_decode(C.byref(a), _stream()), "mm_jpeg_decode")
    return out, status
```

Baseline: 38070.

## Store GEMM epilogue output via swizzled smem boxes and TMA bulk stores

Replaces per-thread row stores of the GEMM output with a path that packs each 128x32 chunk into a 64B-swizzled shared-memory box and issues a TMA tensor store from a leader thread. It also swizzles the fp32 staging layout to reduce bank conflicts, and prefetches residual rows before the staging load. The aim is to cut scattered, poorly coalesced global writes from the epilogue. The cost is extra named-barrier syncs per chunk and bulk-group waits before the staging buffer is reused. The path is used only when the output is 16-bit, not transposed, and aligned.

```diff
diff --git a/include/macaw_b200.h b/include/macaw_b200.h
--- a/include/macaw_b200.h
+++ b/include/macaw_b200.h
@@ -71,6 +71,10 @@
   MM_GEMM_KERNEL_EPILOGUE_WARPGROUP = 1,
   MM_GEMM_KERNEL_TILE_PAIRS = 2
 };
+enum {
+  MM_GEMM_EPI_IO_ROWS = 0,
+  MM_GEMM_EPI_IO_TMA_BOXES = 1
+};
 typedef struct mm_gemm_schedule {
   int32_t block_n;
   int32_t kernel;
@@ -84,6 +88,7 @@
   int32_t streamk_tiles;
   int32_t smem_bytes;
   int32_t vectorised_epilogue;
+  int32_t epilogue_io;
 } mm_gemm_schedule;
 int32_t mm_gemm_plan(const mm_gemm_args* args, mm_gemm_schedule* plan);
 int32_t mm_gemm_streamk_mode(int32_t mode);
diff --git a/macaw-llm_b200/_lib.py b/macaw-llm_b200/_lib.py
--- a/macaw-llm_b200/_lib.py
+++ b/macaw-llm_b200/_lib.py
@@ -32,7 +32,8 @@
 
     _fields_ = [("block_n", c_i32), ("kernel", c_i32), ("m_tiles", c_i32), ("n_tiles", c_i32), ("k_blocks", c_i32),
                 ("units", c_i64), ("workers", c_i32), ("grid", c_i32), ("threads", c_i32), ("waves", c_i32),
-                ("group_m", c_i32), ("streamk_tiles", c_i32), ("smem_bytes", c_i32), ("vectorised_epilogue", c_i32)]
+                ("group_m", c_i32), ("streamk_tiles", c_i32), ("smem_bytes", c_i32), ("vectorised_epilogue", c_i32),
+                ("epilogue_io", c_i32)]
 
 
 class ThinArgs(C.Structure):
diff --git a/macaw-llm_b200/csrc/gemm_wgmma.cu b/macaw-llm_b200/csrc/gemm_wgmma.cu
--- a/macaw-llm_b200/csrc/gemm_wgmma.cu
+++ b/macaw-llm_b200/csrc/gemm_wgmma.cu
@@ -35,6 +35,7 @@
   int sumsq_parts, rs_parts;
   float rs_eps;
   int vec_ok;
+  int c_box;
   int group_m;
   int sk_tiles, sk_first;
   float* sk_ws;
@@ -59,6 +60,60 @@
   return 1024  + (size_t)stages * (kABytes + b_bytes) + (size_t)kBlockM * gemm_stage_ld(BN) * 4 +
          256 ;
 }
+
+__device__ __forceinline__ int stage_sw(int r) { return ((r & 3) << 1) | ((r >> 2) & 1); }
+__device__ __forceinline__ int stage_idx(int r, int col) {
+  return (((col >> 5) * kBlockM + r) << 5) + ((((col & 31) >> 2) ^ stage_sw(r)) << 2) + (col & 3);
+}
+__device__ __forceinline__ void stage_ld_chunk(const float* sC, int c, int r, uint32_t (&v)[32]) {
+  const float4* s = reinterpret_cast<const float4*>(sC + ((c * kBlockM + r) << 5));
+  const int x = stage_sw(r);
+#pragma unroll
+  for (int i = 0; i < 8; ++i) {
+    const float4 f = s[i ^ x];
+    v[4 * i] = __float_as_uint(f.x);
+    v[4 * i + 1] = __float_as_uint(f.y);
+    v[4 * i + 2] = __float_as_uint(f.z);
+    v[4 * i + 3] = __float_as_uint(f.w);
+  }
+}
+
+constexpr uint32_t kBoxBytes = kBlockM * 32 * 2;
+__device__ __forceinline__ void box_put_row(uint8_t* box, int r, const float (&v)[32], int f16) {
+  uint4* row = reinterpret_cast<uint4*>(box + r * 64);
+  const int x = (r >> 1) & 3;
+#pragma unroll
+  for (int k = 0; k < 4; ++k) {
+    uint4 u;
+    if (f16) {
+      u.x = pack_f16x2(v[8 * k + 0], v[8 * k + 1]);
+      u.y = pack_f16x2(v[8 * k + 2], v[8 * k + 3]);
+      u.z = pack_f16x2(v[8 * k + 4], v[8 * k + 5]);
+      u.w = pack_f16x2(v[8 * k + 6], v[8 * k + 7]);
+    } else {
+      u.x = pack_bf16x2(v[8 * k + 0], v[8 * k + 1]);
+      u.y = pack_bf16x2(v[8 * k + 2], v[8 * k + 3]);
+      u.z = pack_bf16x2(v[8 * k + 4], v[8 * k + 5]);
+      u.w = pack_bf16x2(v[8 * k + 6], v[8 * k + 7]);
+    }
+    row[k ^ x] = u;
+  }
+}
+__device__ __forceinline__ void tma_store_4d(const CUtensorMap* m, const void* smem_src, int c0, int c1, int c2, int c3) {
+  asm volatile("cp.async.bulk.tensor.4d.global.shared::cta.bulk_group [%0, {%2, %3, %4, %5}], [%1];"
+               ::"l"(reinterpret_cast<uint64_t>(m)), "r"(smem_u32(smem_src)), "r"(c0), "r"(c1), "r"(c2), "r"(c3)
+               : "memory");
+}
+__device__ __forceinline__ void bulk_commit() { asm volatile("cp.async.bulk.commit_group;" ::: "memory"); }
+__device__ __forceinline__ void bulk_wait_read() { asm volatile("cp.async.bulk.wait_group.read 0;" ::: "memory"); }
+__device__ __forceinline__ void bulk_wait_all() { asm volatile("cp.async.bulk.wait_group 0;" ::: "memory"); }
+__device__ __forceinline__ void group_sync(int id) { asm volatile("bar.sync %0, 128;" ::"r"(id) : "memory"); }
+
+struct EpiIO {
+  const CUtensorMap* tmC;
+  int bar;
+  bool leader;
+};
 
 struct GemmSmem {
   uint8_t *sA, *sB;
@@ -329,11 +384,21 @@
 }
 
 template <int BN, int EPI>
-__device__ __forceinline__ void gemm_epilogue(const GemmKParams& p, const TileCoord& t, const GemmWork& wk, const float* srow,
-                                              float rs, int q, int lane, int half, int wi, int worker, int n_workers) {
+__device__ __forceinline__ void gemm_epilogue(const GemmKParams& p, const TileCoord& t, const GemmWork& wk, float* sC,
+                                              float rs, int q, int lane, int half, int wi, int worker, int n_workers,
+                                              const EpiIO& io) {
   const int n_out_total = (EPI == MM_EPI_SWIGLU) ? p.N / 2 : p.N;
-  const int row = t.m_blk * kBlockM + q * 32 + lane;
+  const int rl = q * 32 + lane;
+  const int row = t.m_blk * kBlockM + rl;
   const bool row_ok = row < p.M;
+  auto box_write = [&](int c, const float (&v)[32]) { box_put_row(reinterpret_cast<uint8_t*>(sC + c * kBlockM * 32), rl, v, p.c_fp16); };
+  auto box_store = [&](int c, int col) {
+    if (io.leader) tma_store_4d(io.tmC, sC + c * kBlockM * 32, col, t.m_blk * kBlockM, t.b_lo, t.b_hi);
+  };
+  auto box_publish = [&]() {
+    fence_proxy_async_smem();
+    group_sync(io.bar);
+  };
   if (wk.role == 1) {
     float* slot = p.sk_ws + static_cast<long long>(worker) * (kBlockM * BN);
 #pragma unroll 1
@@ -341,7 +406,7 @@
       const int c = epi_chunk<BN, EPI>(half, j);
       if (c < 0) continue;
       uint32_t r[32];
-      stage_ld32(srow + c * 32, r);
+      stage_ld_chunk(sC, c, rl, r);
       float4* dst = reinterpret_cast<float4*>(slot) + static_cast<long long>(c) * 8 * kBlockM + q * 32 + lane;
 #pragma unroll
       for (int i = 0; i < 8; ++i)
@@ -400,7 +465,7 @@
         const int c = epi_chunk<BN, EPI>(half, j);
         if (c < 0) continue;
         uint32_t r[32];
-        stage_ld32(srow + c * 32, r);
+        stage_ld_chunk(sC, c, rl, r);
         sk_add(r, c * 32);
         const int col0 = t.n_blk * BN + c * 32;
         if (col0 >= p.N || !row_ok) continue;
@@ -440,15 +505,20 @@
     for (int j = 0; j < epi_chunk_count<BN, EPI>(); ++j) {
       const int c = epi_chunk<BN, EPI>(half, j);
       if (c < 0) continue;
+      const int col0 = t.n_blk * BN + c * 32;
+      const bool full = p.vec_ok && (col0 + 32 <= p.N);
+      uint4 res[4];
+      if (rrow != nullptr && full) {
+#pragma unroll
+        for (int i = 0; i < 4; ++i) res[i] = *(reinterpret_cast<const uint4*>(rrow + col0) + i);
+      }
       uint32_t r[32];
-      stage_ld32(srow + c * 32, r);
+      stage_ld_chunk(sC, c, rl, r);
       sk_add(r, c * 32);
-      const int col0 = t.n_blk * BN + c * 32;
       if (col0 >= p.N) continue;
       float v[32];
 #pragma unroll
       for (int i = 0; i < 32; ++i) v[i] = __uint_as_float(r[i]) * rs;
-      const bool full = p.vec_ok && (col0 + 32 <= p.N);
       if (p.bias_rs != nullptr || p.bias2 != nullptr) {
         const long long ri = static_cast<long long>(t.b) * p.M + row;
         const float s1 = (p.bias_rs != nullptr && row_ok) ? p.bias_rs[ri] : 1.0f;
@@ -475,14 +545,22 @@
       if (rrow != nullptr) {
         if (full) {
 #pragma unroll
-          for (int i = 0; i < 4; ++i) aux_add8(v + 8 * i, *(reinterpret_cast<const uint4*>(rrow + col0) + i), p.aux_f16);
+          for (int i = 0; i < 4; ++i) aux_add8(v + 8 * i, res[i], p.aux_f16);
         } else {
 #pragma unroll
           for (int i = 0; i < 32; ++i)
             if (col0 + i < p.N) v[i] += aux_ld(rrow, col0 + i, p.aux_f16);
         }
       }
-      if (row_ok) store_row32(p, crow, col0, n_out_total, v);
+      if (p.c_box) {
+        group_sync(io.bar);
+        box_write(c, v);
+        box_publish();
+        box_store(c, col0);
+        if (io.leader) bulk_commit();
+      } else if (row_ok) {
+        store_row32(p, crow, col0, n_out_total, v);
+      }
       if (p.sumsq_out != nullptr && row_ok) {
         float ss = 0.f;
 #pragma unroll
@@ -499,8 +577,8 @@
     for (int j = 0; j < epi_chunk_count<BN, EPI>(); j += 2) {
       const int cg = epi_chunk<BN, EPI>(half, j), cu = epi_chunk<BN, EPI>(half, j + 1);
       uint32_t g[32], u[32];
-      stage_ld32(srow + cg * 32, g);
-      stage_ld32(srow + cu * 32, u);
+      stage_ld_chunk(sC, cg, rl, g);
+      stage_ld_chunk(sC, cu, rl, u);
       sk_add(g, cg * 32);
       sk_add(u, cu * 32);
       const int col_in = t.n_blk * BN + cg * 32;
@@ -512,7 +590,15 @@
         const float uu = __uint_as_float(u[i]) * rs;
         v[i] = gg * sigmoid_fast(gg) * uu;
       }
-      if (row_ok) store_row32(p, crow, col_in / 2, n_out_total, v);
+      if (p.c_box) {
+        group_sync(io.bar);
+        box_write(cg, v);
+        box_publish();
+        box_store(cg, col_in / 2);
+        if (io.leader) bulk_commit();
+      } else if (row_ok) {
+        store_row32(p, crow, col_in / 2, n_out_total, v);
+      }
     }
   } else {
     const int pos = (row_ok ? (row % p.rope_T) : 0) + (p.rope_pos != nullptr ? __ldg(p.rope_pos) : 0);
@@ -524,8 +610,8 @@
         const int c1 = epi_chunk<BN, EPI>(half, j), c2 = epi_chunk<BN, EPI>(half, j + 1);
         const int hc = c1 & 1;
         uint32_t x1[32], x2[32];
-        stage_ld32(srow + c1 * 32, x1);
-        stage_ld32(srow + c2 * 32, x2);
+        stage_ld_chunk(sC, c1, rl, x1);
+        stage_ld_chunk(sC, c2, rl, x2);
         sk_add(x1, c1 * 32);
         sk_add(x2, c2 * 32);
         const int col1 = t.n_blk * BN + c1 * 32;
@@ -553,7 +639,15 @@
             o2[i] = __uint_as_float(x2[i]) * rs;
           }
         }
-        if (row_ok) {
+        if (p.c_box) {
+          group_sync(io.bar);
+          box_write(c1, o1);
+          box_write(c2, o2);
+          box_publish();
+          box_store(c1, col1);
+          box_store(c2, col1 + 64);
+          if (io.leader) bulk_commit();
+        } else if (row_ok) {
           store_row32(p, crow, col1, n_out_total, o1);
           store_row32(p, crow, col1 + 64, n_out_total, o2);
         }
@@ -570,36 +664,36 @@
 
 template <int BN, int N>
 __device__ __forceinline__ void stage_acc(float* sC, const float (&acc)[N], int off, int wg, int q, int lane) {
-  constexpr int LDS = gemm_stage_ld(BN);
   const int r0 = wg * 64 + q * 16 + (lane >> 2);
   const int c0 = 2 * (lane & 3);
 #pragma unroll
   for (int j = 0; j < BN / 8; ++j) {
     const int i = off + 4 * j;
-    *reinterpret_cast<float2*>(sC + r0 * LDS + 8 * j + c0) = make_float2(acc[i], acc[i + 1]);
-    *reinterpret_cast<float2*>(sC + (r0 + 8) * LDS + 8 * j + c0) = make_float2(acc[i + 2], acc[i + 3]);
+    const int s = stage_idx(r0, 8 * j + c0);
+    *reinterpret_cast<float2*>(sC + s) = make_float2(acc[i], acc[i + 1]);
+    *reinterpret_cast<float2*>(sC + s + 8 * 32) = make_float2(acc[i + 2], acc[i + 3]);
   }
 }
 
 template <int BN, int EPI>
 __device__ __forceinline__ void ewg_tile(const GemmKParams& p, const GemmSmem& s, const TileCoord& t, const GemmWork& wk,
-                                         const float* srow, float rs, uint32_t parity, int q, int lane, int worker,
-                                         int n_workers) {
+                                         float rs, uint32_t parity, int q, int lane, int worker, int n_workers,
+                                         const EpiIO& io) {
   mbar_wait(s.staging_full, parity);
   for (int half = 0; half < 2; ++half)
-    gemm_epilogue<BN, EPI>(p, t, wk, srow, rs, q, lane, half, q + 4 * half, worker, n_workers);
+    gemm_epilogue<BN, EPI>(p, t, wk, s.sC, rs, q, lane, half, q + 4 * half, worker, n_workers, io);
+  if (p.c_box && io.leader) bulk_wait_read();
   mbar_arrive(s.staging_empty);
 }
 
 template <int BN, int EPI, bool B_MN, bool A_MN, bool F16, bool EWG>
 __global__ void __launch_bounds__(EWG ? kGemmThreadsEwg : kGemmThreads, 1)
 gemm_bf16_kernel(const __grid_constant__ CUtensorMap tmA, const __grid_constant__ CUtensorMap tmB,
-                 const GemmKParams p) {
+                 const __grid_constant__ CUtensorMap tmC, const GemmKParams p) {
   static_assert(BN == 32 || BN == 64 || BN == 128, "wgmma tile width");
   static_assert(epi_chunks_partition_tile<BN, EPI>(), "epilogue chunk ownership must partition the tile");
   constexpr int STAGES = gemm_stages(BN);
   constexpr uint32_t B_BYTES = BN * kBlockK * 2;
-  constexpr int LDS = gemm_stage_ld(BN);
 
   extern __shared__ uint8_t smem_raw[];
   const GemmSmem sm = gemm_smem<STAGES, B_BYTES, BN>(smem_raw);
@@ -658,15 +752,16 @@
   }
 
   const int q = warp & 3;
-  const float* srow = sm.sC + (q * 32 + lane) * LDS;
+  const EpiIO io = {&tmC, EWG ? 2 : 2 + (warp >> 2), q == 0 && lane == 0};
   if (EWG && warp >= 8) {
     if constexpr (EWG) setmaxnreg_inc<168>();
     GemmWork wk;
     for (int it = 0; gemm_work(p, worker, n_workers, total_tiles, it, wk); ++it) {
       const TileCoord t = tile_coord(wk.tile, p, m_units);
       const float rs = epi_row_scale(p, t, t.m_blk * kBlockM + q * 32 + lane);
-      ewg_tile<BN, EPI>(p, sm, t, wk, srow, rs, it & 1, q, lane, worker, n_workers);
-    }
+      ewg_tile<BN, EPI>(p, sm, t, wk, rs, it & 1, q, lane, worker, n_workers, io);
+    }
+    if (p.c_box && io.leader) bulk_wait_all();
     return;
   }
 
@@ -720,8 +815,10 @@
     }
     const int half = warp >> 2;
     const float rs = wk.role == 1 ? 1.0f : epi_row_scale(p, t, t.m_blk * kBlockM + q * 32 + lane);
-    gemm_epilogue<BN, EPI>(p, t, wk, srow, rs, q, lane, half, warp, worker, n_workers);
-  }
+    gemm_epilogue<BN, EPI>(p, t, wk, sm.sC, rs, q, lane, half, warp, worker, n_workers, io);
+    if (p.c_box && io.leader) bulk_wait_read();
+  }
+  if (p.c_box && io.leader) bulk_wait_all();
 }
 
 constexpr int kWideThreads = 384;
@@ -748,7 +845,8 @@
 
 template <int EPI, bool F16>
 __global__ void __launch_bounds__(kWideThreads, 1)
-gemm_wide_kernel(const __grid_constant__ CUtensorMap tmA, const __grid_constant__ CUtensorMap tmB, const GemmKParams p) {
+gemm_wide_kernel(const __grid_constant__ CUtensorMap tmA, const __grid_constant__ CUtensorMap tmB,
+                 const __grid_constant__ CUtensorMap tmC, const GemmKParams p) {
   constexpr int BN = kMaxBN;
   extern __shared__ uint8_t smem_raw[];
   const GemmSmem sm = gemm_smem<kWideStages, kWideBBytes, BN>(smem_raw);
@@ -767,7 +865,7 @@
   const int q = warp & 3;
   if (warp >= 8) {
     setmaxnreg_dec<kWideRegsEpilogue>();
-    const float* srow = sm.sC + (q * 32 + lane) * gemm_stage_ld(BN);
+    const EpiIO io = {&tmC, 2, q == 0 && lane == 0};
     GemmWork wk;
     wk.tile = 0; wk.kb0 = 0; wk.kb1 = p.num_k; wk.role = 0; wk.c0 = 0; wk.nc = 0;
     for (int u = worker; u < total_pairs; u += n_workers) {
@@ -775,10 +873,11 @@
       const float rs = epi_row_scale(p, t, t.m_blk * kBlockM + q * 32 + lane);
 #pragma unroll 1
       for (int side = 0; side < 2; ++side) {
-        ewg_tile<BN, EPI>(p, sm, t, wk, srow, rs, side, q, lane, worker, n_workers);
+        ewg_tile<BN, EPI>(p, sm, t, wk, rs, side, q, lane, worker, n_workers, io);
         ++t.n_blk;
       }
     }
+    if (p.c_box && io.leader) bulk_wait_all();
     return;
   }
 
@@ -879,13 +978,12 @@
 template <int EPI, bool PROMOTE>
 __global__ void __launch_bounds__(kGemmThreads, 1)
 gemm_e4m3_kernel(const __grid_constant__ CUtensorMap tmA, const __grid_constant__ CUtensorMap tmB0,
-                 const __grid_constant__ CUtensorMap tmB1, const __grid_constant__ CUtensorMap tmB2, const GemmKParams p,
-                 const E4m3P e) {
+                 const __grid_constant__ CUtensorMap tmB1, const __grid_constant__ CUtensorMap tmB2,
+                 const __grid_constant__ CUtensorMap tmC, const GemmKParams p, const E4m3P e) {
   constexpr int BN = kMaxBN;
   constexpr int STAGES = gemm_stages(BN);
   constexpr uint32_t B_BYTES = BN * kE4m3BlockK;
   static_assert(B_BYTES == BN * kBlockK * 2 && kABytes == kBlockM * kE4m3BlockK, "e4m3 stage = the 16-bit stage");
-  constexpr int LDS = gemm_stage_ld(BN);
   extern __shared__ uint8_t smem_raw[];
   const GemmSmem sm = gemm_smem<STAGES, B_BYTES, BN>(smem_raw);
 
@@ -939,7 +1037,7 @@
   }
 
   const int q = warp & 3;
-  const float* srow = sm.sC + (q * 32 + lane) * LDS;
+  const EpiIO io = {&tmC, 2 + (warp >> 2), q == 0 && lane == 0};
   const int wg = warp >> 2;
   int stage = 0;
   uint32_t phase = 0;
@@ -1011,8 +1109,10 @@
     }
     const int half = warp >> 2;
     const float rs = epi_row_scale(p, t, t.m_blk * kBlockM + q * 32 + lane);
-    gemm_epilogue<BN, EPI>(p, t, wk, srow, rs, q, lane, half, warp, worker, n_workers);
-  }
+    gemm_epilogue<BN, EPI>(p, t, wk, sm.sC, rs, q, lane, half, warp, worker, n_workers, io);
+    if (p.c_box && io.leader) bulk_wait_read();
+  }
+  if (p.c_box && io.leader) bulk_wait_all();
 }
 
 typedef CUresult (*EncodeTiledFn)(CUtensorMap*, CUtensorMapDataType, cuuint32_t, void*, const cuuint64_t*,
@@ -1031,8 +1131,9 @@
   return fn;
 }
 
-int make_map(CUtensorMap* m, const void* ptr, uint64_t inner, uint64_t rows, uint64_t batch, uint64_t batch2,
-             int64_t ld, int64_t bs, int64_t bs2, uint32_t box_rows) {
+static int make_map_box(CUtensorMap* m, const void* ptr, uint64_t inner, uint64_t rows, uint64_t batch, uint64_t batch2,
+                        int64_t ld, int64_t bs, int64_t bs2, uint32_t box_rows, uint32_t box_inner,
+                        CUtensorMapSwizzle swizzle) {
   EncodeTiledFn fn = get_encode_fn();
   if (fn == nullptr) {
     set_error("cuTensorMapEncodeTiled entry point unavailable (no CUDA driver?)");
@@ -1043,10 +1144,10 @@
   if (bs2 <= 0) bs2 = static_cast<int64_t>(batch) * bs;
   cuuint64_t strides[3] = {static_cast<cuuint64_t>(ld) * 2, static_cast<cuuint64_t>(bs) * 2,
                            static_cast<cuuint64_t>(bs2) * 2};
-  cuuint32_t box[4] = {64, box_rows, 1, 1};
+  cuuint32_t box[4] = {box_inner, box_rows, 1, 1};
   cuuint32_t estr[4] = {1, 1, 1, 1};
   CUresult r = fn(m, CU_TENSOR_MAP_DATA_TYPE_BFLOAT16, 4, const_cast<void*>(ptr), dims, strides, box, estr,
-                  CU_TENSOR_MAP_INTERLEAVE_NONE, CU_TENSOR_MAP_SWIZZLE_128B, CU_TENSOR_MAP_L2_PROMOTION_L2_256B,
+                  CU_TENSOR_MAP_INTERLEAVE_NONE, swizzle, CU_TENSOR_MAP_L2_PROMOTION_L2_256B,
                   CU_TENSOR_MAP_FLOAT_OOB_FILL_NONE);
   if (r != CUDA_SUCCESS) {
     set_error("cuTensorMapEncodeTiled failed (%d): ptr=%p dims={%llu,%llu,%llu,%llu} ld=%lld bs=%lld bs2=%lld box_rows=%u",
@@ -1056,6 +1157,10 @@
     return 1;
   }
   return 0;
+}
+int make_map(CUtensorMap* m, const void* ptr, uint64_t inner, uint64_t rows, uint64_t batch, uint64_t batch2,
+             int64_t ld, int64_t bs, int64_t bs2, uint32_t box_rows) {
+  return make_map_box(m, ptr, inner, rows, batch, batch2, ld, bs, bs2, box_rows, 64, CU_TENSOR_MAP_SWIZZLE_128B);
 }
 
 
@@ -1136,6 +1241,9 @@
   p.sumsq_out = a->sumsq_out; p.sumsq_parts = (a->N + 31) / 32;
   p.rs_sumsq = a->rs_sumsq; p.rs_parts = a->rs_parts; p.rs_eps = a->rs_eps;
   p.vec_ok = vec ? 1 : 0;
+  p.c_box = (!a->c_fp32 && !a->c_trans && reinterpret_cast<uintptr_t>(a->C) % 16 == 0 && a->ldc % 8 == 0 &&
+             (a->batch == 1 || (a->c_bs > 0 && a->c_bs % 8 == 0)) && (batch2 == 1 || (a->c_bs2 > 0 && a->c_bs2 % 8 == 0)))
+                ? 1 : 0;
 
   const int sms = num_sms();
   int BN = kMaxBN;
@@ -1190,6 +1298,7 @@
   s.block_n = BN; s.m_tiles = p.m_tiles; s.n_tiles = p.n_tiles; s.k_blocks = p.num_k; s.group_m = p.group_m;
   s.units = tiles; s.workers = sms; s.waves = static_cast<int>((tiles + sms - 1) / sms);
   s.streamk_tiles = p.sk_tiles; s.vectorised_epilogue = p.vec_ok;
+  s.epilogue_io = p.c_box ? MM_GEMM_EPI_IO_TMA_BOXES : MM_GEMM_EPI_IO_ROWS;
   s.kernel = wide ? MM_GEMM_KERNEL_TILE_PAIRS : ewg ? MM_GEMM_KERNEL_EPILOGUE_WARPGROUP : MM_GEMM_KERNEL_CONSUMER_EPILOGUE;
   s.threads = wide ? kWideThreads : ewg ? kGemmThreadsEwg : kGemmThreads;
   s.smem_bytes = static_cast<int32_t>(wide ? kWideSmemBytes : gemm_smem_bytes(gemm_stages(BN), BN * kBlockK * 2, BN));
@@ -1201,10 +1310,11 @@
 }
 
 template <auto kern>
-static int launch_gemm(const GemmLaunch& L, const CUtensorMap& ta, const CUtensorMap& tb, cudaStream_t st) {
+static int launch_gemm(const GemmLaunch& L, const CUtensorMap& ta, const CUtensorMap& tb, const CUtensorMap& tc,
+                       cudaStream_t st) {
   static bool attr_set[kMaxDevices] = {};
   if (int rc = ensure_smem_attr(kern, L.s.smem_bytes, attr_set, "mm_gemm_fwd")) return rc;
-  cudaError_t e = launch_kernel(kern, dim3(L.s.grid), dim3(L.s.threads), L.s.smem_bytes, st, 1, ta, tb, L.p);
+  cudaError_t e = launch_kernel(kern, dim3(L.s.grid), dim3(L.s.threads), L.s.smem_bytes, st, 1, ta, tb, tc, L.p);
   if (e != cudaSuccess) {
     set_error("mm_gemm_fwd: launch failed: %s", cudaGetErrorString(e));
     return 2;
@@ -1213,16 +1323,27 @@
 }
 
 template <int BN, int EPI, bool B_MN = false, bool A_MN = false>
-static int launch_variant(const GemmLaunch& L, const CUtensorMap& ta, const CUtensorMap& tb, cudaStream_t st) {
+static int launch_variant(const GemmLaunch& L, const CUtensorMap& ta, const CUtensorMap& tb, const CUtensorMap& tc,
+                          cudaStream_t st) {
   if constexpr (BN == kMaxBN && !B_MN && !A_MN)
     if (L.s.kernel == MM_GEMM_KERNEL_TILE_PAIRS)
-      return L.f16 ? launch_gemm<&gemm_wide_kernel<EPI, true>>(L, ta, tb, st)
-                   : launch_gemm<&gemm_wide_kernel<EPI, false>>(L, ta, tb, st);
+      return L.f16 ? launch_gemm<&gemm_wide_kernel<EPI, true>>(L, ta, tb, tc, st)
+                   : launch_gemm<&gemm_wide_kernel<EPI, false>>(L, ta, tb, tc, st);
   if (L.s.kernel == MM_GEMM_KERNEL_EPILOGUE_WARPGROUP)
-    return L.f16 ? launch_gemm<&gemm_bf16_kernel<BN, EPI, B_MN, A_MN, true, true>>(L, ta, tb, st)
-                 : launch_gemm<&gemm_bf16_kernel<BN, EPI, B_MN, A_MN, false, true>>(L, ta, tb, st);
-  return L.f16 ? launch_gemm<&gemm_bf16_kernel<BN, EPI, B_MN, A_MN, true, false>>(L, ta, tb, st)
-               : launch_gemm<&gemm_bf16_kernel<BN, EPI, B_MN, A_MN, false, false>>(L, ta, tb, st);
+    return L.f16 ? launch_gemm<&gemm_bf16_kernel<BN, EPI, B_MN, A_MN, true, true>>(L, ta, tb, tc, st)
+                 : launch_gemm<&gemm_bf16_kernel<BN, EPI, B_MN, A_MN, false, true>>(L, ta, tb, tc, st);
+  return L.f16 ? launch_gemm<&gemm_bf16_kernel<BN, EPI, B_MN, A_MN, true, false>>(L, ta, tb, tc, st)
+               : launch_gemm<&gemm_bf16_kernel<BN, EPI, B_MN, A_MN, false, false>>(L, ta, tb, tc, st);
+}
+
+static int make_c_map(CUtensorMap* tc, const mm_gemm_args* a, const GemmLaunch& L, const CUtensorMap& ta) {
+  if (!L.p.c_box) {
+    *tc = ta;
+    return 0;
+  }
+  const uint64_t n_out = a->epi == MM_EPI_SWIGLU ? a->N / 2 : a->N;
+  return make_map_box(tc, a->C, n_out, a->M, a->batch, L.p.batch2, a->ldc, a->c_bs, a->c_bs2, kBlockM, 32,
+                  CU_TENSOR_MAP_SWIZZLE_64B);
 }
 
 }
@@ -1247,8 +1368,10 @@
   } else {
     if (make_map(&tb, a->B, a->N, a->K, b_batch, b_batch2, a->ldb, a->b_bs, a->b_bs2, 64)) return 1;
   }
+  CUtensorMap tc;
+  if (make_c_map(&tc, a, L, ta)) return 1;
   cudaStream_t st = reinterpret_cast<cudaStream_t>(stream);
-#define MM_LAUNCH(...) return launch_variant<__VA_ARGS__>(L, ta, tb, st)
+#define MM_LAUNCH(...) return launch_variant<__VA_ARGS__>(L, ta, tb, tc, st)
   if (a->epi == MM_EPI_ROPE) MM_LAUNCH(128, MM_EPI_ROPE);
   if (a->epi == MM_EPI_SWIGLU) MM_LAUNCH(128, MM_EPI_SWIGLU);
   if (a->a_mn_major) {
@@ -1357,6 +1480,7 @@
   s.block_n = kMaxBN; s.m_tiles = p.m_tiles; s.n_tiles = p.n_tiles; s.k_blocks = p.num_k; s.group_m = p.group_m;
   s.units = tiles; s.workers = sms; s.waves = static_cast<int>((tiles + sms - 1) / sms);
   s.streamk_tiles = 0; s.vectorised_epilogue = p.vec_ok;
+  s.epilogue_io = p.c_box ? MM_GEMM_EPI_IO_TMA_BOXES : MM_GEMM_EPI_IO_ROWS;
   s.kernel = MM_GEMM_KERNEL_CONSUMER_EPILOGUE;
   s.threads = kGemmThreads;
   s.smem_bytes = static_cast<int32_t>(gemm_smem_bytes(gemm_stages(kMaxBN), kMaxBN * kE4m3BlockK, kMaxBN));
@@ -1365,12 +1489,12 @@
 }
 
 template <int EPI, bool PROMOTE>
-static int launch_e4m3(const GemmLaunch& L, const CUtensorMap (&tm)[4], const E4m3P& e, cudaStream_t st) {
+static int launch_e4m3(const GemmLaunch& L, const CUtensorMap (&tm)[5], const E4m3P& e, cudaStream_t st) {
   auto kern = &gemm_e4m3_kernel<EPI, PROMOTE>;
   static bool attr_set[kMaxDevices] = {};
   if (int rc = ensure_smem_attr(kern, L.s.smem_bytes, attr_set, "mm_gemm_e4m3_fwd")) return rc;
   cudaError_t err = launch_kernel(kern, dim3(L.s.grid), dim3(L.s.threads), L.s.smem_bytes, st, 1, tm[0], tm[1], tm[2], tm[3],
-                                  L.p, e);
+                                  tm[4], L.p, e);
   if (err != cudaSuccess) {
     set_error("mm_gemm_e4m3_fwd: launch failed: %s", cudaGetErrorString(err));
     return 2;
@@ -1390,8 +1514,9 @@
 extern "C" int32_t mm_gemm_e4m3_fwd(const mm_gemm_args* a, const mm_gemm_e4m3_args* e, void* stream) {
   GemmLaunch L;
   if (int rc = plan_gemm_e4m3(a, e, L)) return rc;
-  CUtensorMap tm[4];
+  CUtensorMap tm[5];
   if (make_map_e4m3(&tm[0], a->A, a->K, a->M, a->lda, kBlockM)) return 1;
+  if (make_c_map(&tm[4], a, L, tm[0])) return 1;
   const mm_w8_matrix& w = e->w;
   for (int j = 0; j < MM_W8_MAX_SRC; ++j) {
     const int src = w.q[j] != nullptr ? j : 0;
diff --git a/macaw-llm_b200/ops.py b/macaw-llm_b200/ops.py
--- a/macaw-llm_b200/ops.py
+++ b/macaw-llm_b200/ops.py
@@ -11,6 +11,7 @@
 ACT_NONE, ACT_GELU, ACT_QUICK_GELU, ACT_SILU = 0, 1, 2, 3
 EPI_STD, EPI_SWIGLU, EPI_ROPE = 0, 1, 2
 GEMM_CONSUMER_EPILOGUE, GEMM_EPILOGUE_WARPGROUP, GEMM_TILE_PAIRS = 0, 1, 2
+GEMM_EPI_IO_ROWS, GEMM_EPI_IO_TMA_BOXES = 0, 1
 
 _BF16 = torch.bfloat16
 _F16 = torch.float16
```

Measured after the change: 39000, median of 6. +2.4%, better.
